# YangHai-1218/RADet

Measured on AMD Instinct MI355X. Metric: images/sec train-step, r50_ycbv_pbr 640x480 bs=4/GPU, higher is better.
Workload: dtype f32

## Files before the change

include/radet_hip.h:

```cpp
#ifndef RADET_HIP_H
#define RADET_HIP_H
#include <stdint.h>

#ifdef __cplusplus
extern "C" {
#endif


typedef struct RadetConvDesc {
    const float* w;
    const float* bias;
    const float* bn_gamma;
    const float* bn_beta;
    const float* bn_mean;
    const float* bn_var;
    float* wf;
    float* wft;
    float* bias_f;
    const float* dwf_slabs;
    const float* dbias_partials;
    float* dw;
    float* dbias;
    float* dgamma;
    float* dbeta;
    int cout, cin, kh, kw;
    int nsplit;
    float eps;
    int wft_ld;
    int wft_off;
    int w16;
    float* w_amax;
    float* wfq;
    float* w_l1;
    float* bias_amax;
    float* w_l1t;
} RadetConvDesc;

#define RADET_AMAX_WORDS 64
typedef struct RadetScales {
    const void* x_amax;
    const void* w_amax;
    void* y_amax;
    const void* x1_amax;
    const void* w1_amax;
    void* y1_amax;
    void* yq;
    void* yq_amax;
    const void* x_true_amax;
    const void* w_l1;
    const void* bias_amax;
    const void* addend_amax;
} RadetScales;

int radet_gather_table_rows(int M);
int radet_build_gather_table(int* table, int B, int KH, int KW, int so, int sr, int off, int div, const int* seg_desc,
                             int nseg, void* stream);
enum {
    RADET_TILE_ID_MASK = 0xFF,
    RADET_TILE_SYMBOL = 0x100,
    RADET_TILE_BK32 = 0x200,
    RADET_TILE_MATH_BF16 = 0x400,
    RADET_TILE_STORE_BF16 = 0x800,
    RADET_TILE_SPLITK = 0x1000,
    RADET_TILE_SPLITK_MASK = 0xF000,
    RADET_TILE_OUT_F32 = 0x10000,
    RADET_TILE_STAGES3 = 0x20000,
    RADET_TILE_STAGES4 = 0x40000,
    RADET_TILE_ROWPAIRS = 0x80000,
    RADET_TILE_STREAMK = 0x100000,
    RADET_TILE_STREAMK_MASK = 0x700000,
    RADET_TILE_X3 = 0x1000000,
    RADET_TILE_P3 = 0x2000000,
    RADET_TILE_H2 = 0x8000000,
    RADET_TILE_MASKQ = 0x10000000
};
int radet_conv2d_igemm(const float* x, const float* w, const float* bias, const float* addend, const float* mask,
                       float* y, const int* gather_table, int M, int Cin, int Cout, int KH, int KW, int relu,
                       int tile_override, float* splitk_ws, size_t splitk_ws_floats, void* stream);
int radet_conv2d_igemm_s(const float* x, const float* w, const float* bias, const float* addend, const float* mask,
                         float* y, const int* gather_table, int M, int Cin, int Cout, int KH, int KW, int relu,
                         int tile_override, float* splitk_ws, size_t splitk_ws_floats, void* stream, const RadetScales* sc);
int radet_conv2d_igemm_pair_s(const float* x0, const float* w0, const float* bias0, const float* addend0,
                              const float* mask0, float* y0, const float* x1, const float* w1, const float* bias1,
                              const float* addend1, const float* mask1, float* y1, const int* gather_table, int M,
                              int Cin, int Cout, int KH, int KW, int relu, int tile_override, float* splitk_ws,
                              size_t splitk_ws_floats, void* stream, const RadetScales* sc);
int radet_conv2d_igemm_taps_s(const float* x, const float* w, const float* addend, const float* mask, float* y,
                              const int* gather_table, const int* out_rows, const int* tap_ids_host, int ntaps, int kt_w,
                              int M, int Cin, int Cout, int tile_override, float* splitk_ws, size_t splitk_ws_floats,
                              void* stream, const RadetScales* sc);
int radet_conv2d_igemm_classes_s(const float* x, const float* w, const float* addend, const float* mask, float* y,
                                 const int* gather_table, const int* out_rows, const int* tap_ids_host,
                                 const int* cls_ntaps, const int* cls_start, int ncls, int kt_w, int M, int Cin, int Cout,
                                 int tile_override, float* splitk_ws, size_t splitk_ws_floats, void* stream,
                                 const RadetScales* sc);
int radet_conv2d_igemm_pair(const float* x0, const float* w0, const float* bias0, const float* addend0,
                            const float* mask0, float* y0, const float* x1, const float* w1, const float* bias1,
                            const float* addend1, const float* mask1, float* y1, const int* gather_table, int M, int Cin,
                            int Cout, int KH, int KW, int relu, int tile_override, float* splitk_ws,
                            size_t splitk_ws_floats, void* stream);
int radet_conv2d_igemm_taps(const float* x, const float* w, const float* addend, const float* mask, float* y,
                            const int* gather_table, const int* out_rows, const int* tap_ids_host, int ntaps, int kt_w,
                            int M, int Cin, int Cout, int tile_override, float* splitk_ws, size_t splitk_ws_floats,
                            void* stream);
int radet_conv2d_igemm_classes(const float* x, const float* w, const float* addend, const float* mask, float* y,
                               const int* gather_table, const int* out_rows, const int* tap_ids_host, const int* cls_ntaps,
                               const int* cls_start, int ncls, int kt_w, int M, int Cin, int Cout, int tile_override,
                               float* splitk_ws, size_t splitk_ws_floats, void* stream);
int radet_pred3x3_patch(const float* x, int Cin, const int* tiles_dev, int ntiles, const float* w0, const float* bias0,
                        float* y0, int c0, const float* w1, const float* bias1, float* y1, int c1, void* stream);
enum {
    RADET_WGRAD_MATH_BF16 = 0x1,
    RADET_WGRAD_STORE_BF16 = 0x2,
    RADET_WGRAD_TILE = 0x10,
    RADET_WGRAD_TILE_MASK = 0x30,
    RADET_WGRAD_ONE_TAP = 0x40,
    RADET_WGRAD_PX32 = 0x80,
    RADET_WGRAD_X3 = 0x100,
    RADET_WGRAD_P3 = 0x200,
    RADET_WGRAD_KDIV4 = 0x400,
    RADET_WGRAD_KDIV2 = 0x800,
    RADET_WGRAD_H2 = 0x1000,
    RADET_WGRAD_DEEP = 0x2000,
    RADET_WGRAD_WINDOWS = 0x4000
};
int radet_conv2d_wgrad_splits(int M, int Cin, int Cout, int KH, int KW);
int radet_conv2d_wgrad(const float* dy, const float* x, float* slabs, float* dbias_partials, const int* gather_table,
                       int M, int Cin, int Cout, int ld_dy, int KH, int KW, int S, int flags, void* stream);
int radet_conv2d_wgrad_s(const float* dy, const float* x, float* slabs, float* dbias_partials, const int* gather_table,
                         int M, int Cin, int Cout, int ld_dy, int KH, int KW, int S, int flags, void* stream,
                         const RadetScales* sc);
typedef struct RadetWgradJob {
    const float* dy;
    const float* x;
    float* slabs;
    float* dbias_partials;
    const int* gather_table;
    int M, Cin, Cout, ld_dy, KH, KW, S;
} RadetWgradJob;
int radet_conv2d_wgrad_group(const RadetWgradJob* jobs, int njobs, int flags, void* stream);
int radet_fold_weights(const RadetConvDesc* table_dev, int nconv, void* stream);
int radet_unfold_grads(const RadetConvDesc* table_dev, int nconv, int max_cout, void* stream);
int radet_stem_conv_bn_relu(const float* img_nchw, const float* wf_ohwi, const float* bias, float* y_nhwc, int B,
                            int H, int W, void* stream);
int radet_maxpool3x3s2(const float* x, float* y, int B, int H, int W, int C, void* stream);
int radet_maxpool3x3s2_bwd_relu(const float* s, const float* dpool, float* ds, int B, int H, int W, int C, void* stream);
int radet_stem_wgrad_splits(int B, int H, int W);
int radet_stem_wgrad(const float* img_nchw, const float* ds, float* slabs, float* dbias_partials, int B, int H, int W, int S,
                     void* stream);

int radet_gn_workspace_floats(int B, const int* seg_desc, int nseg);
int radet_gn_relu_fwd(const float* z, const float* gamma, const float* beta, float* y, float* stats ,
                      float* partial_ws, int B, int C, int groups, float eps, int relu, const int* seg_desc, int nseg,
                      void* stream);
int radet_gn_relu_bwd(const float* dy, const float* z, const float* stats, const float* gamma, const float* beta,
                      float* dz, float* dgamma, float* dbeta, float* partial_ws, int B, int C, int groups, int relu,
                      const int* seg_desc, int nseg, void* stream);

int radet_upsample_add(float* dst, const float* src, int B, int Ho, int Wo, int Hi, int Wi, int C, void* stream);
int radet_upsample_add_bwd(float* dsrc, const float* ddst, int B, int Ho, int Wo, int Hi, int Wi, int C, void* stream);
int radet_relu_bwd(const float* dy, const float* addend, const float* act, float* dx, size_t n, void* stream);
int radet_stem_conv_bn_relu_h(const float* img_nchw, const float* wf_ohwi, const float* bias, void* y_nhwc, int B, int H,
                              int W, void* stream);
int radet_maxpool3x3s2_h(const void* x, void* y, int B, int H, int W, int C, void* stream);
int radet_gn_relu_fwd_pair(const float* z0, const float* gamma0, const float* beta0, float* y0, float* stats0,
                           float* partial_ws0, const float* z1, const float* gamma1, const float* beta1, float* y1,
                           float* stats1, float* partial_ws1, int B, int C, int groups, float eps, int relu,
                           const int* seg_desc, int nseg, void* stream);
int radet_gn_relu_fwd_pair_h(const void* z0, const float* gamma0, const float* beta0, void* y0, float* stats0,
                             float* partial_ws0, const void* z1, const float* gamma1, const float* beta1, void* y1,
                             float* stats1, float* partial_ws1, int B, int C, int groups, float eps, int relu,
                             const int* seg_desc, int nseg, void* stream);
int radet_gn_relu_fwd_h(const void* z, const float* gamma, const float* beta, void* y, float* stats, float* partial_ws,
                        int B, int C, int groups, float eps, int relu, const int* seg_desc, int nseg, void* stream);
int radet_gn_relu_bwd_h(const void* dy, const void* z, const float* stats, const float* gamma, const float* beta, void* dz,
                        float* dgamma, float* dbeta, float* partial_ws, int B, int C, int groups, int relu,
                        const int* seg_desc, int nseg, void* stream);
int radet_upsample_add_h(void* dst, const void* src, int B, int Ho, int Wo, int Hi, int Wi, int C, void* stream);
int radet_upsample_add_bwd_h(void* dsrc, const void* ddst, int B, int Ho, int Wo, int Hi, int Wi, int C, void* stream);
int radet_relu_bwd_h(const void* dy, const void* addend, const void* act, void* dx, size_t n, void* stream);
int radet_convert_rows(const void* src, void* dst, size_t rows, int ncols, int src_ld, int src_off, int dst_ld,
                       int dst_off, int to_bf16, void* stream);
int radet_split_planes(const float* src, void* dst_planes, size_t rows, int C, int src_ld, void* stream);
int radet_merge_planes(const void* src_planes, float* dst, size_t rows, int C, int dst_ld, void* stream);
int radet_split_pairs(const float* src, void* dst_pairs, size_t rows, int C, int src_ld, const void* src_amax, void* dst_amax,
                      void* stream);
int radet_merge_pairs(const void* src_pairs, float* dst, size_t rows, int C, int dst_ld, const void* amax, void* stream);
int radet_gn_relu_fwd_q(const float* z, const float* gamma, const float* beta, float* y, void* yq, float* stats,
                        float* partial_ws, int B, int C, int groups, float eps, int relu, const int* seg_desc, int nseg,
                        void* stream, void* y_amax, void* yq_amax, void* zhat_amax);
int radet_gn_relu_fwd_pair_q(const float* z0, const float* gamma0, const float* beta0, float* y0, void* yq0, float* stats0,
                             float* partial_ws0, void* y_amax0, void* yq_amax0, void* zhat_amax0, const float* z1,
                             const float* gamma1, const float* beta1, float* y1, void* yq1, float* stats1,
                             float* partial_ws1, void* y_amax1, void* yq_amax1, void* zhat_amax1, int B, int C, int groups,
                             float eps, int relu, const int* seg_desc, int nseg, void* stream);
int radet_gn_relu_bwd_q(const float* dy, const float* z, const float* stats, const float* gamma, const float* beta, float* dz,
                        void* dzq, float* dgamma, float* dbeta, float* partial_ws, int B, int C, int groups, int relu,
                        const int* seg_desc, int nseg, void* stream, const void* dy_amax, const void* zhat_amax,
                        void* dzq_amax);
int radet_maxpool3x3s2_a(const float* x, float* y, int B, int H, int W, int C, void* y_amax, void* stream);
int radet_maxpool3x3s2_q(const float* x, float* y, int B, int H, int W, int C, void* y_amax, void* yq, void* yq_amax,
                         const void* x_amax, void* stream);
int radet_stem_conv_bn_relu_a(const float* img_nchw, const float* wf_ohwi, const float* bias, float* y_nhwc, int B, int H, int W,
                              void* y_amax, void* stream);
int radet_upsample_add_a(float* dst, const float* src, int B, int Ho, int Wo, int Hi, int Wi, int C, void* dst_amax,
                         void* stream);
int radet_upsample_add_bwd_a(float* dsrc, const float* ddst, int B, int Ho, int Wo, int Hi, int Wi, int C, void* dsrc_amax,
                             void* stream);
int radet_relu_bwd_a(const float* dy, const float* addend, const float* act, float* dx, size_t n, void* dx_amax, void* stream);
int radet_absmax(const float* x, size_t n, void* amax, void* stream);
int radet_amax_slot_words(void);
int radet_gn_relu_fwd_p(const float* z, const float* gamma, const float* beta, float* y, void* yp, float* stats,
                        float* partial_ws, int B, int C, int groups, float eps, int relu, const int* seg_desc, int nseg,
                        void* stream);
int radet_gn_relu_fwd_pair_p(const float* z0, const float* gamma0, const float* beta0, float* y0, void* yp0, float* stats0,
                             float* partial_ws0, const float* z1, const float* gamma1, const float* beta1, float* y1,
                             void* yp1, float* stats1, float* partial_ws1, int B, int C, int groups, float eps, int relu,
                             const int* seg_desc, int nseg, void* stream);
int radet_gn_relu_bwd_p(const float* dy, const float* z, const float* stats, const float* gamma, const float* beta,
                        float* dz, void* dzp, float* dgamma, float* dbeta, float* partial_ws, int B, int C, int groups,
                        int relu, const int* seg_desc, int nseg, void* stream);
int radet_nchw_to_nhwc(const float* x, float* y, int B, int C, int H, int W, void* stream);
int radet_nhwc_to_nchw(const float* x, float* y, int B, int C, int H, int W, void* stream);

#define RADET_HEAD_LOSS_POSTACT 1
#define RADET_HEAD_LOSS_KIND_SHIFT 1
#define RADET_HEAD_LOSS_KIND_MASK (7 << RADET_HEAD_LOSS_KIND_SHIFT)
#define RADET_BOX_LOSS_GIOU 0
#define RADET_BOX_LOSS_IOU 1
#define RADET_BOX_LOSS_IOU_LINEAR 2
#define RADET_BOX_LOSS_DIOU 3
#define RADET_BOX_LOSS_CIOU 4
#define RADET_BOX_LOSS_KINDS 5
int radet_head_loss_ws_ints(int R);
int radet_head_loss(const float* cls, const float* reg_u, const float* iou, const float* scales,
                    const float* gt_boxes, const int64_t* gt_labels, const int* gt_off, const int64_t* p2g,
                    const float* pw, const int* level_desc, int nlvl, int B, int num_classes, float alpha,
                    float gamma, float loss_bbox_weight, float giou_eps, const float* grad_scale, float* losses,
                    float* dcls, int dcls_ld, float* dreg_u, int dreg_ld, float* diou, int diou_ld, float* dscales,
                    int64_t* labels_out, float* bbox_targets_out, int flags, int* ws, void* stream);
int radet_scale_relu(const float* reg_u, const float* scales, float* out, const int* level_desc, int nlvl, int B,
                     void* stream);

size_t radet_decode_ws_bytes(int B, int nlvl, int nms_pre);
int radet_decode_candidates(const float* cls, const float* reg_u, const float* iou, const float* scales,
                            const int* level_desc, int nlvl, int B, int num_classes, float score_thr, int nms_pre,
                            const float* img_hw , const float* scale_factor ,
                            float* cand_boxes, float* cand_scores, float* cand_ctr, int64_t* cand_labels,
                            int* cand_count, void* ws, void* stream);

size_t radet_nms_ws_bytes(int B, int cap);
int radet_nms(const float* boxes, const float* cluster_scores, const float* vote_scores, const int64_t* labels,
              const int* counts, int B, int cap, int mode, float iou_thr, int iou_enable, float sigma, int max_out,
              float* out_boxes, float* out_scores, int64_t* out_labels, int* out_count, int64_t* aux0, int64_t* aux1,
              void* ws, void* stream);

size_t radet_assign_ws_bytes(int B, int N);
int radet_assign_points(const float* gt_boxes, const int* gt_off, const uint8_t* masks, int H, int W,
                        const uint32_t* rng_words, int U, const int* level_desc, const float* regress_ranges ,
                        int nlvl, int B, int positive_num, int flags, float neg_threshold, int64_t* p2g, float* pw, int* used,
                        void* ws, void* stream);

int radet_assign_points_f(const float* gt_boxes, const int* gt_off, const float* distance_maps, int H, int W,
                          const uint32_t* rng_words, int U, const int* level_desc, const float* regress_ranges ,
                          int nlvl, int B, int positive_num, int flags, float neg_threshold, int64_t* p2g, float* pw, int* used,
                          void* ws, void* stream);

size_t radet_mbd_ws_bytes(size_t total_px);
int radet_mbd(const uint8_t* images, const int* img_desc_dev, int nimg, const int* seeds_x, const int* seeds_y, float alpha,
              int niter, int base_size, double* dmap, size_t total_px, void* ws, void* stream);
int radet_gdt(const float* cost, const int* img_desc_dev, int nimg, const int* seeds_x, const int* seeds_y, float* dist,
              void* ws_labels , void* stream);

int radet_resize_linear_u8(const uint8_t* src, const int* src_desc, uint8_t* dst, const int* dst_desc, const int* view_desc,
                           int ncrop, int max_dst_px, int channels, void* stream);
int radet_resize_linear_f(const void* src, const int* src_desc, void* dst, const int* dst_desc, int ncrop, int max_dst_px,
                          int is_f64, void* stream);
#define RADET_VIEW_INTS 12
int radet_gaussian_blur9_u8(const uint8_t* src, const int* desc, uint8_t* dst, float* tmp, const float* kernel5, int ncrop,
                            int max_px, void* stream);
int radet_sobel_edge(const uint8_t* src, const int* desc, float* edge, uint8_t* gray_ws, uint32_t* max_ws, int ncrop,
                     int max_px, void* stream);

int radet_mask_max(const uint8_t* masks, uint32_t* maxes , int G, size_t hw, void* stream);
int radet_mask_transform(const uint8_t* src, uint8_t* dst, const uint32_t* norm_max, const int* view_desc, int G, int Hs, int Ws,
                         int Hr, int Wr, int Hd, int Wd, int flip, int pad_val, void* stream);

#define RLE_MASK_INTS 5
#define RLE_PART_INTS 2
int radet_rle_masks(const uint32_t* run_ends, int n_ends, const int* part_desc, int n_parts, const int* mask_desc,
                    const int* view_desc, int G, uint8_t* dst, uint8_t* dst_plain, int Hr, int Wr, int Hd, int Wd, int pad_val,
                    void* stream);

#define JPEG_ROW_INTS 8
#define JPEG_DESC_INTS 20
#define JPEG_HUFF_BYTES 1424
int radet_jpeg_index(const uint8_t* file, int scan_lo, int scan_hi, int ncomp, const int* comp_blocks, const void* huff,
                     int n_mcus, int restart_interval, int seg_mcus, int* rows, int max_rows);
int radet_jpeg_decode(const uint8_t* files, const int* desc, int nimg, const int* wgs, int n_wg, const void* huff,
                      const uint16_t* quant, const int* rows, int n_rows, int16_t* coef, uint8_t* planes, uint8_t* dst,
                      int* err, int max_blocks, int max_px, int stages, void* stream);

#define AUG_PARAM_INTS 16
#define AUG_MAX_W 8192
int radet_augment_merge_hblur(const uint8_t* src, const uint8_t* bg, const int* params, uint8_t* dst, int nimg, int max_h,
                              int max_w, void* stream);
int radet_augment_vblur(const uint8_t* src, const int* params, uint8_t* dst, int nimg, int max_h, int max_w, void* stream);
int radet_augment_sharp(const uint8_t* src, const int* params, uint8_t* dst, unsigned long long* lsum, int nimg, int max_px,
                        void* stream);
int radet_augment_finish(const uint8_t* src, const unsigned long long* lsum, const int* params, float* out, int nimg, int Hp,
                         int Wp, float m0, float m1, float m2, float s0, float s1, float s2, void* stream);

#define AUG2_PARAM_INTS 16
int radet_augment_hsv_noise(const uint8_t* src, const int* params2, uint8_t* dst, int nimg, int max_px, void* stream);
int radet_augment_box(const uint8_t* src, const int* params2, uint8_t* dst, size_t nbytes, int nimg, int max_h, int max_w,
                      void* stream);

#define CROP_DESC_INTS 12
#define PASTE_DESC_INTS 10
int radet_crop_canvases(const uint8_t* src, size_t src_bytes, const unsigned long long* lsum, const int* params, int nimg,
                        const int* desc, int ncanvas, int max_px, uint8_t* dst, size_t total_px, void* stream);
int radet_paste_maps(const void* maps, size_t map_px, int is_f64, const int* desc, int nbox, int H, int W, float* out,
                     void* stream);

#define WARP_DESC_INTS 20
#define WARP_DESC_SRC 0
#define WARP_DESC_DST 1
#define WARP_DESC_H 2
#define WARP_DESC_W 3
#define WARP_DESC_CHANNELS 4
#define WARP_DESC_FILL 5
#define WARP_DESC_FLAGS 6
#define WARP_DESC_MATRIX 8
#define WARP_SKIP 1
int radet_warp_affine_u8(const uint8_t* src, size_t src_px, uint8_t* dst, size_t dst_px, const int* desc, int nimg, int max_px,
                         int channels, void* stream);

#define CUTOUT_DESC_INTS 8
#define CUTOUT_DESC_OFF 0
#define CUTOUT_DESC_H 1
#define CUTOUT_DESC_W 2
#define CUTOUT_DESC_FILL 3
#define CUTOUT_DESC_FIRST 4
#define CUTOUT_DESC_COUNT 5
#define CUTOUT_DESC_FLAGS 6
#define CUTOUT_SKIP 1
#define CUTOUT_FLIP 2
#define CUTOUT_TO_RGB 4
int radet_cutout_u8(uint8_t* img, size_t img_px, const int* desc, int nimg, const int* holes, int nholes, int max_holes,
                    int max_area, int channels, void* stream);
int radet_cutout_f32(float* out, int nbatch, int Hp, int Wp, const int* desc, int nimg, const int* holes, int nholes, int max_holes,
                     int max_area, float m0, float m1, float m2, float s0, float s1, float s2, void* stream);

#define PREP_DESC_INTS 8
#define PREP_TO_RGB 1
int radet_preprocess_frames(const int* desc, int nimg, int Hp, int Wp, float m0, float m1, float m2, float s0, float s1,
                            float s2, float* out, void* stream);

int radet_bbox_overlaps(const float* bboxes1, const float* bboxes2, float* out, int batch, int M, int N, int mode,
                        int aligned, float eps, void* stream);
int radet_tblr_encode(const float* priors, const float* gts, float* out, int n, const float* normalizer4,
                      int normalize_by_wh, void* stream);
int radet_tblr_decode(const float* priors, const float* tblr, float* out, int n, const float* normalizer4,
                      int normalize_by_wh, float max_h, float max_w, int clip, void* stream);
int radet_loss_partials(size_t n_elem);
int radet_loss_finalize(const float* partials, int npartials, const float* avg_factor, float scale, float* out,
                        void* stream);
int radet_sigmoid_focal_loss(const float* logits, const int64_t* target, const float* weight, int weight_cols, size_t N,
                             int C, float gamma, float alpha, float* loss_elem, float elem_scale, float* partials,
                             void* stream);
int radet_sigmoid_focal_loss_bwd(const float* logits, const int64_t* target, const float* weight, int weight_cols, size_t N,
                                 int C, float gamma, float alpha, const float* grad_elem, const float* grad_scalar,
                                 const float* avg_factor, float scale, float* dlogits, void* stream);
int radet_bce_logits_loss(const float* logits, const float* target, const float* weight, int weight_cols, size_t N, int C,
                          float* loss_elem, float elem_scale, float* partials, void* stream);
int radet_bce_logits_loss_bwd(const float* logits, const float* target, const float* weight, int weight_cols, size_t N,
                              int C, const float* grad_elem, const float* grad_scalar, const float* avg_factor, float scale,
                              float* dlogits, void* stream);
int radet_giou_loss(const float* pred, const float* target, const float* weight, size_t N, float eps, float* loss_elem,
                    float elem_scale, float* partials, void* stream);
int radet_giou_loss_bwd(const float* pred, const float* target, const float* weight, size_t N, float eps,
                        const float* grad_elem, const float* grad_scalar, const float* avg_factor, float scale, float* dpred,
                        void* stream);
int radet_box_loss(int kind, const float* pred, const float* target, const float* weight, size_t N, float eps, float hp1,
                   float* loss_elem, float elem_scale, float* partials, void* stream);
int radet_box_loss_bwd(int kind, const float* pred, const float* target, const float* weight, size_t N, float eps, float hp1,
                       const float* grad_elem, const float* grad_scalar, const float* avg_factor, float scale, float* dpred,
                       void* stream);
int radet_threshold_compact(const float* scores, size_t n, float thr, int64_t* idx, int* count, void* stream);

int radet_grid_anchors(float* out, const int* level_desc, int nlvl, int octave_base_scale, void* stream);

int radet_sqnorm_partials(const float* g, size_t n, float* partials, int npartials, void* stream);
int radet_adamw_step(float* p, const float* g, float* m, float* v, size_t n, float lr, float beta1, float beta2,
                     float eps, float weight_decay, int step, float max_norm, float grad_div,
                     const float* partials, int npartials, float* grad_norm_out, void* stream);
#define RADET_OPT_MAX_RUNS 1024
typedef struct { uint32_t begin, end; float lr_mult, decay_mult; } RadetOptRun;
// ... 42 lines not shown
```

radet_amd/_lib.py:

```python
import ctypes as C
import os

_HERE = os.path.dirname(os.path.abspath(__file__))
LIB_PATH = os.path.join(_HERE, os.environ.get("RADET_LIB", "libradet_hip.so"))

_p = C.c_void_p
_i = C.c_int
_f = C.c_float
_sz = C.c_size_t


class RadetConvDesc(C.Structure):
    _fields_ = [("w", _p), ("bias", _p), ("bn_gamma", _p), ("bn_beta", _p), ("bn_mean", _p), ("bn_var", _p),
                ("wf", _p), ("wft", _p), ("bias_f", _p), ("dwf_slabs", _p), ("dbias_partials", _p),
                ("dw", _p), ("dbias", _p), ("dgamma", _p), ("dbeta", _p),
                ("cout", _i), ("cin", _i), ("kh", _i), ("kw", _i), ("nsplit", _i), ("eps", _f),
                ("wft_ld", _i), ("wft_off", _i), ("w16", _i), ("w_amax", _p), ("wfq", _p), ("w_l1", _p), ("bias_amax", _p),
                ("w_l1t", _p)]


class RadetScales(C.Structure):
    _fields_ = [("x_amax", _p), ("w_amax", _p), ("y_amax", _p), ("x1_amax", _p), ("w1_amax", _p), ("y1_amax", _p),
                ("yq", _p), ("yq_amax", _p), ("x_true_amax", _p), ("w_l1", _p), ("bias_amax", _p), ("addend_amax", _p)]


class RadetWgradJob(C.Structure):
    _fields_ = [("dy", _p), ("x", _p), ("slabs", _p), ("dbias_partials", _p), ("gather_table", _p),
                ("M", _i), ("Cin", _i), ("Cout", _i), ("ld_dy", _i), ("KH", _i), ("KW", _i), ("S", _i)]


class RadetTapeOp(C.Structure):
    _fields_ = [("kind", C.c_int32), ("fn", C.c_int32), ("stream", _p), ("event", _p), ("args", C.c_uint64 * 32)]


SIGNATURES = {
    "radet_gather_table_rows": (_i, [_i]),
    "radet_build_gather_table": (_i, [_p, _i, _i, _i, _i, _i, _i, _i, _p, _i, _p]),
    "radet_conv2d_igemm": (_i, [_p, _p, _p, _p, _p, _p, _p, _i, _i, _i, _i, _i, _i, _i, _p, _sz, _p]),
    "radet_conv2d_igemm_pair": (_i, [_p] * 13 + [_i, _i, _i, _i, _i, _i, _i, _p, _sz, _p]),
    "radet_conv2d_igemm_taps": (_i, [_p, _p, _p, _p, _p, _p, _p, _p, _i, _i, _i, _i, _i, _i, _p, _sz, _p]),
    "radet_conv2d_igemm_classes": (_i, [_p, _p, _p, _p, _p, _p, _p, _p, _p, _p, _i, _i, _i, _i, _i, _i, _p, _sz, _p]),
    "radet_conv2d_igemm_s": (_i, [_p, _p, _p, _p, _p, _p, _p, _i, _i, _i, _i, _i, _i, _i, _p, _sz, _p, _p]),
    "radet_conv2d_igemm_pair_s": (_i, [_p] * 13 + [_i, _i, _i, _i, _i, _i, _i, _p, _sz, _p, _p]),
    "radet_conv2d_igemm_taps_s": (_i, [_p, _p, _p, _p, _p, _p, _p, _p, _i, _i, _i, _i, _i, _i, _p, _sz, _p, _p]),
    "radet_conv2d_igemm_classes_s": (_i, [_p, _p, _p, _p, _p, _p, _p, _p, _p, _p, _i, _i, _i, _i, _i, _i, _p, _sz, _p, _p]),
    "radet_conv2d_wgrad_s": (_i, [_p, _p, _p, _p, _p, _i, _i, _i, _i, _i, _i, _i, _i, _p, _p]),
    "radet_split_pairs": (_i, [_p, _p, _sz, _i, _i, _p, _p, _p]),
    "radet_merge_pairs": (_i, [_p, _p, _sz, _i, _i, _p, _p]),
    "radet_gn_relu_fwd_q": (_i, [_p, _p, _p, _p, _p, _p, _p, _i, _i, _i, _f, _i, _p, _i, _p, _p, _p, _p]),
    "radet_gn_relu_fwd_pair_q": (_i, [_p] * 20 + [_i, _i, _i, _f, _i, _p, _i, _p]),
    "radet_gn_relu_bwd_q": (_i, [_p, _p, _p, _p, _p, _p, _p, _p, _p, _p, _i, _i, _i, _i, _p, _i, _p, _p, _p, _p]),
    "radet_maxpool3x3s2_a": (_i, [_p, _p, _i, _i, _i, _i, _p, _p]),
    "radet_maxpool3x3s2_q": (_i, [_p, _p, _i, _i, _i, _i, _p, _p, _p, _p, _p]),
    "radet_stem_conv_bn_relu_a": (_i, [_p, _p, _p, _p, _i, _i, _i, _p, _p]),
    "radet_upsample_add_a": (_i, [_p, _p, _i, _i, _i, _i, _i, _i, _p, _p]),
    "radet_upsample_add_bwd_a": (_i, [_p, _p, _i, _i, _i, _i, _i, _i, _p, _p]),
    "radet_relu_bwd_a": (_i, [_p, _p, _p, _p, _sz, _p, _p]),
    "radet_absmax": (_i, [_p, _sz, _p, _p]),
    "radet_amax_slot_words": (_i, []),
    "radet_pred3x3_patch": (_i, [_p, _i, _p, _i, _p, _p, _p, _i, _p, _p, _p, _i, _p]),
    "radet_conv2d_wgrad_splits": (_i, [_i, _i, _i, _i, _i]),
    "radet_conv2d_wgrad": (_i, [_p, _p, _p, _p, _p, _i, _i, _i, _i, _i, _i, _i, _i, _p]),
    "radet_conv2d_wgrad_group": (_i, [_p, _i, _i, _p]),
    "radet_fold_weights": (_i, [_p, _i, _p]),
    "radet_unfold_grads": (_i, [_p, _i, _i, _p]),
    "radet_stem_conv_bn_relu": (_i, [_p, _p, _p, _p, _i, _i, _i, _p]),
    "radet_maxpool3x3s2": (_i, [_p, _p, _i, _i, _i, _i, _p]),
    "radet_maxpool3x3s2_bwd_relu": (_i, [_p, _p, _p, _i, _i, _i, _i, _p]),
    "radet_stem_wgrad_splits": (_i, [_i, _i, _i]),
    "radet_stem_wgrad": (_i, [_p, _p, _p, _p, _i, _i, _i, _i, _p]),
    "radet_gn_workspace_floats": (_i, [_i, _p, _i]),
    "radet_gn_relu_fwd": (_i, [_p, _p, _p, _p, _p, _p, _i, _i, _i, _f, _i, _p, _i, _p]),
    "radet_gn_relu_fwd_pair": (_i, [_p] * 12 + [_i, _i, _i, _f, _i, _p, _i, _p]),
    "radet_gn_relu_fwd_pair_h": (_i, [_p] * 12 + [_i, _i, _i, _f, _i, _p, _i, _p]),
    "radet_gn_relu_bwd": (_i, [_p, _p, _p, _p, _p, _p, _p, _p, _p, _i, _i, _i, _i, _p, _i, _p]),
    "radet_upsample_add": (_i, [_p, _p, _i, _i, _i, _i, _i, _i, _p]),
    "radet_upsample_add_bwd": (_i, [_p, _p, _i, _i, _i, _i, _i, _i, _p]),
    "radet_relu_bwd": (_i, [_p, _p, _p, _p, _sz, _p]),
    "radet_nchw_to_nhwc": (_i, [_p, _p, _i, _i, _i, _i, _p]),
    "radet_nhwc_to_nchw": (_i, [_p, _p, _i, _i, _i, _i, _p]),
    "radet_head_loss_ws_ints": (_i, [_i]),
    "radet_head_loss": (_i, [_p, _p, _p, _p, _p, _p, _p, _p, _p, _p, _i, _i, _i, _f, _f, _f, _f, _p, _p, _p, _i, _p,
                             _i, _p, _i, _p, _p, _p, _i, _p, _p]),
    "radet_scale_relu": (_i, [_p, _p, _p, _p, _i, _i, _p]),
    "radet_decode_ws_bytes": (_sz, [_i, _i, _i]),
    "radet_decode_candidates": (_i, [_p, _p, _p, _p, _p, _i, _i, _i, _f, _i, _p, _p, _p, _p, _p, _p, _p, _p, _p]),
    "radet_nms_ws_bytes": (_sz, [_i, _i]),
    "radet_nms": (_i, [_p, _p, _p, _p, _p, _i, _i, _i, _f, _i, _f, _i, _p, _p, _p, _p, _p, _p, _p, _p]),
    "radet_assign_ws_bytes": (_sz, [_i, _i]),
    "radet_assign_points": (_i, [_p, _p, _p, _i, _i, _p, _i, _p, _p, _i, _i, _i, _i, _f, _p, _p, _p, _p, _p]),
    "radet_assign_points_f": (_i, [_p, _p, _p, _i, _i, _p, _i, _p, _p, _i, _i, _i, _i, _f, _p, _p, _p, _p, _p]),
    "radet_resize_linear_u8": (_i, [_p, _p, _p, _p, _p, _i, _i, _i, _p]),
    "radet_resize_linear_f": (_i, [_p, _p, _p, _p, _i, _i, _i, _p]),
    "radet_warp_affine_u8": (_i, [_p, _sz, _p, _sz, _p, _i, _i, _i, _p]),
    "radet_cutout_u8": (_i, [_p, _sz, _p, _i, _p, _i, _i, _i, _i, _p]),
    "radet_cutout_f32": (_i, [_p, _i, _i, _i, _p, _i, _p, _i, _i, _i, _f, _f, _f, _f, _f, _f, _p]),
    "radet_gaussian_blur9_u8": (_i, [_p, _p, _p, _p, _p, _i, _i, _p]),
    "radet_sobel_edge": (_i, [_p, _p, _p, _p, _p, _i, _i, _p]),
    "radet_stem_conv_bn_relu_h": (_i, [_p, _p, _p, _p, _i, _i, _i, _p]),
    "radet_maxpool3x3s2_h": (_i, [_p, _p, _i, _i, _i, _i, _p]),
    "radet_gn_relu_fwd_h": (_i, [_p, _p, _p, _p, _p, _p, _i, _i, _i, _f, _i, _p, _i, _p]),
    "radet_gn_relu_bwd_h": (_i, [_p, _p, _p, _p, _p, _p, _p, _p, _p, _i, _i, _i, _i, _p, _i, _p]),
    "radet_upsample_add_h": (_i, [_p, _p, _i, _i, _i, _i, _i, _i, _p]),
    "radet_upsample_add_bwd_h": (_i, [_p, _p, _i, _i, _i, _i, _i, _i, _p]),
    "radet_relu_bwd_h": (_i, [_p, _p, _p, _p, _sz, _p]),
    "radet_convert_rows": (_i, [_p, _p, _sz, _i, _i, _i, _i, _i, _i, _p]),
    "radet_split_planes": (_i, [_p, _p, _sz, _i, _i, _p]),
    "radet_merge_planes": (_i, [_p, _p, _sz, _i, _i, _p]),
    "radet_gn_relu_fwd_p": (_i, [_p, _p, _p, _p, _p, _p, _p, _i, _i, _i, _f, _i, _p, _i, _p]),
    "radet_gn_relu_fwd_pair_p": (_i, [_p] * 14 + [_i, _i, _i, _f, _i, _p, _i, _p]),
    "radet_gn_relu_bwd_p": (_i, [_p, _p, _p, _p, _p, _p, _p, _p, _p, _p, _i, _i, _i, _i, _p, _i, _p]),
    "radet_mbd_ws_bytes": (_sz, [_sz]),
    "radet_mbd": (_i, [_p, _p, _i, _p, _p, _f, _i, _i, _p, _sz, _p, _p]),
    "radet_gdt": (_i, [_p, _p, _i, _p, _p, _p, _p, _p]),
    "radet_mask_max": (_i, [_p, _p, _i, _sz, _p]),
    "radet_mask_transform": (_i, [_p, _p, _p, _p, _i, _i, _i, _i, _i, _i, _i, _i, _i, _p]),
    "radet_rle_masks": (_i, [_p, _i, _p, _i, _p, _p, _i, _p, _p, _i, _i, _i, _i, _i, _p]),
    "radet_jpeg_index": (_i, [_p, _i, _i, _i, _p, _p, _i, _i, _i, _p, _i]),
    "radet_jpeg_decode": (_i, [_p, _p, _i, _p, _i, _p, _p, _p, _i, _p, _p, _p, _p, _i, _i, _i, _p]),
    "radet_augment_merge_hblur": (_i, [_p, _p, _p, _p, _i, _i, _i, _p]),
    "radet_augment_vblur": (_i, [_p, _p, _p, _i, _i, _i, _p]),
    "radet_augment_sharp": (_i, [_p, _p, _p, _p, _i, _i, _p]),
    "radet_augment_finish": (_i, [_p, _p, _p, _p, _i, _i, _i, _f, _f, _f, _f, _f, _f, _p]),
    "radet_augment_hsv_noise": (_i, [_p, _p, _p, _i, _i, _p]),
    "radet_augment_box": (_i, [_p, _p, _p, _sz, _i, _i, _i, _p]),
    "radet_crop_canvases": (_i, [_p, _sz, _p, _p, _i, _p, _i, _i, _p, _sz, _p]),
    "radet_paste_maps": (_i, [_p, _sz, _i, _p, _i, _i, _i, _p, _p]),
    "radet_preprocess_frames": (_i, [_p, _i, _i, _i, _f, _f, _f, _f, _f, _f, _p, _p]),
    "radet_grid_anchors": (_i, [_p, _p, _i, _i, _p]),
    "radet_bbox_overlaps": (_i, [_p, _p, _p, _i, _i, _i, _i, _i, _f, _p]),
    "radet_tblr_encode": (_i, [_p, _p, _p, _i, _p, _i, _p]),
    "radet_tblr_decode": (_i, [_p, _p, _p, _i, _p, _i, _f, _f, _i, _p]),
    "radet_loss_partials": (_i, [_sz]),
    "radet_loss_finalize": (_i, [_p, _i, _p, _f, _p, _p]),
    "radet_sigmoid_focal_loss": (_i, [_p, _p, _p, _i, _sz, _i, _f, _f, _p, _f, _p, _p]),
    "radet_sigmoid_focal_loss_bwd": (_i, [_p, _p, _p, _i, _sz, _i, _f, _f, _p, _p, _p, _f, _p, _p]),
    "radet_bce_logits_loss": (_i, [_p, _p, _p, _i, _sz, _i, _p, _f, _p, _p]),
    "radet_bce_logits_loss_bwd": (_i, [_p, _p, _p, _i, _sz, _i, _p, _p, _p, _f, _p, _p]),
    "radet_giou_loss": (_i, [_p, _p, _p, _sz, _f, _p, _f, _p, _p]),
    "radet_giou_loss_bwd": (_i, [_p, _p, _p, _sz, _f, _p, _p, _p, _f, _p, _p]),
    "radet_box_loss": (_i, [_i, _p, _p, _p, _sz, _f, _f, _p, _f, _p, _p]),
    "radet_box_loss_bwd": (_i, [_i, _p, _p, _p, _sz, _f, _f, _p, _p, _p, _f, _p, _p]),
    "radet_threshold_compact": (_i, [_p, _sz, _f, _p, _p, _p]),
    "radet_sqnorm_partials": (_i, [_p, _sz, _p, _i, _p]),
    "radet_adamw_step": (_i, [_p, _p, _p, _p, _sz, _f, _f, _f, _f, _f, _i, _f, _f, _p, _i, _p, _p]),
    "radet_adamw_step_runs": (_i, [_p, _p, _p, _p, _sz, _f, _f, _f, _f, _f, _i, _f, _f, _p, _i, _p, _p, _i, _p]),
    "radet_sgd_step": (_i, [_p, _p, _p, _sz, _f, _f, _f, _f, _i, _i, _f, _f, _p, _i, _p, _p, _i, _p]),
    "radet_grad_accumulate": (_i, [_p, _p, _sz, _i, _p]),
    "radet_coco_match": (_i, [_p, _p, _p, _p, _p, _p, _i, _i, _p, _i, _p, _i, _p, _p, _p, _p, _p]),
    "radet_coco_accumulate": (_i, [_p, _p, _p, _p, _p, _p, _p, _p, _i, _i, _i, _i, _i, _p, _p, _p, _p]),
    "radet_tape_fn_index": (_i, [C.c_char_p]),
    "radet_tape_replay": (_i, [_p, _i, _i, _p]),
    "radet_fill_zero": (_i, [_p, _sz, _p]),
    "radet_copy_d2d": (_i, [_p, _p, _sz, _p]),
    "radet_stream_create_cumask": (_i, [_p, _i, _p]),
    "radet_copy_segments": (_i, [_p, _i, _i, _p]),
}

_lib = None


class RadetHipError(RuntimeError):
    pass


def load():
    global _lib
    if _lib is not None:
        return _lib
    if not os.path.exists(LIB_PATH):
        raise RadetHipError(
            f"{LIB_PATH} is missing: the HIP extension is not built. Run `make -C radet_amd/csrc` "
            "(or __graft_entry__.build()). radet_amd has no CPU / PyTorch fallback.")
    lib = C.CDLL(LIB_PATH)
    for name, (res, args) in SIGNATURES.items():
        try:
            fn = getattr(lib, name)
        except AttributeError as e:
            raise RadetHipError(f"libradet_hip.so does not export {name}") from e
        fn.restype = res
        fn.argtypes = args
    _lib = lib
    return lib


def check(rc, name):
    if rc != 0:
        raise RadetHipError(f"{name} failed with code {rc} (-1 bad argument, -2 launch failure)")


_FN = {}


def call(name, *args):
    fn = _FN.get(name)
    if fn is None:
        if name not in SIGNATURES:
            raise RadetHipError(f"{name} has no entry in radet_amd._lib.SIGNATURES")
        fn = _FN[name] = getattr(load(), name)
    rc = fn(*args)
    if rc != 0:
        raise RadetHipError(f"{name} failed with code {rc} (-1 bad argument, -2 launch failure)")
    if TAPE is not None:
        TAPE.record_call(name, args)


TAPE = None
```

radet_amd/csrc/tape_thunks.c:

```c
#include <stdint.h>
#include <stddef.h>
#include <string.h>
#include "radet_hip.h"

static float f32(uint64_t w) { uint32_t u = (uint32_t)w; float f; memcpy(&f, &u, 4); return f; }

static int t_radet_absmax(const uint64_t* a) { return radet_absmax((void*)(uintptr_t)a[0], (size_t)a[1], (void*)(uintptr_t)a[2], (void*)(uintptr_t)a[3]); }
static int t_radet_adamw_step(const uint64_t* a) { return radet_adamw_step((void*)(uintptr_t)a[0], (void*)(uintptr_t)a[1], (void*)(uintptr_t)a[2], (void*)(uintptr_t)a[3], (size_t)a[4], f32(a[5]), f32(a[6]), f32(a[7]), f32(a[8]), f32(a[9]), (int)(int64_t)a[10], f32(a[11]), f32(a[12]), (void*)(uintptr_t)a[13], (int)(int64_t)a[14], (void*)(uintptr_t)a[15], (void*)(uintptr_t)a[16]); }
static int t_radet_adamw_step_runs(const uint64_t* a) { return radet_adamw_step_runs((void*)(uintptr_t)a[0], (void*)(uintptr_t)a[1], (void*)(uintptr_t)a[2], (void*)(uintptr_t)a[3], (size_t)a[4], f32(a[5]), f32(a[6]), f32(a[7]), f32(a[8]), f32(a[9]), (int)(int64_t)a[10], f32(a[11]), f32(a[12]), (void*)(uintptr_t)a[13], (int)(int64_t)a[14], (void*)(uintptr_t)a[15], (void*)(uintptr_t)a[16], (int)(int64_t)a[17], (void*)(uintptr_t)a[18]); }
static int t_radet_amax_slot_words(const uint64_t* a) { (void)a; return radet_amax_slot_words(); }
static int t_radet_assign_points(const uint64_t* a) { return radet_assign_points((void*)(uintptr_t)a[0], (void*)(uintptr_t)a[1], (void*)(uintptr_t)a[2], (int)(int64_t)a[3], (int)(int64_t)a[4], (void*)(uintptr_t)a[5], (int)(int64_t)a[6], (void*)(uintptr_t)a[7], (void*)(uintptr_t)a[8], (int)(int64_t)a[9], (int)(int64_t)a[10], (int)(int64_t)a[11], (int)(int64_t)a[12], f32(a[13]), (void*)(uintptr_t)a[14], (void*)(uintptr_t)a[15], (void*)(uintptr_t)a[16], (void*)(uintptr_t)a[17], (void*)(uintptr_t)a[18]); }
static int t_radet_assign_points_f(const uint64_t* a) { return radet_assign_points_f((void*)(uintptr_t)a[0], (void*)(uintptr_t)a[1], (void*)(uintptr_t)a[2], (int)(int64_t)a[3], (int)(int64_t)a[4], (void*)(uintptr_t)a[5], (int)(int64_t)a[6], (void*)(uintptr_t)a[7], (void*)(uintptr_t)a[8], (int)(int64_t)a[9], (int)(int64_t)a[10], (int)(int64_t)a[11], (int)(int64_t)a[12], f32(a[13]), (void*)(uintptr_t)a[14], (void*)(uintptr_t)a[15], (void*)(uintptr_t)a[16], (void*)(uintptr_t)a[17], (void*)(uintptr_t)a[18]); }
static int t_radet_augment_box(const uint64_t* a) { return radet_augment_box((void*)(uintptr_t)a[0], (void*)(uintptr_t)a[1], (void*)(uintptr_t)a[2], (size_t)a[3], (int)(int64_t)a[4], (int)(int64_t)a[5], (int)(int64_t)a[6], (void*)(uintptr_t)a[7]); }
static int t_radet_augment_finish(const uint64_t* a) { return radet_augment_finish((void*)(uintptr_t)a[0], (void*)(uintptr_t)a[1], (void*)(uintptr_t)a[2], (void*)(uintptr_t)a[3], (int)(int64_t)a[4], (int)(int64_t)a[5], (int)(int64_t)a[6], f32(a[7]), f32(a[8]), f32(a[9]), f32(a[10]), f32(a[11]), f32(a[12]), (void*)(uintptr_t)a[13]); }
static int t_radet_augment_hsv_noise(const uint64_t* a) { return radet_augment_hsv_noise((void*)(uintptr_t)a[0], (void*)(uintptr_t)a[1], (void*)(uintptr_t)a[2], (int)(int64_t)a[3], (int)(int64_t)a[4], (void*)(uintptr_t)a[5]); }
static int t_radet_augment_merge_hblur(const uint64_t* a) { return radet_augment_merge_hblur((void*)(uintptr_t)a[0], (void*)(uintptr_t)a[1], (void*)(uintptr_t)a[2], (void*)(uintptr_t)a[3], (int)(int64_t)a[4], (int)(int64_t)a[5], (int)(int64_t)a[6], (void*)(uintptr_t)a[7]); }
static int t_radet_augment_sharp(const uint64_t* a) { return radet_augment_sharp((void*)(uintptr_t)a[0], (void*)(uintptr_t)a[1], (void*)(uintptr_t)a[2], (void*)(uintptr_t)a[3], (int)(int64_t)a[4], (int)(int64_t)a[5], (void*)(uintptr_t)a[6]); }
static int t_radet_augment_vblur(const uint64_t* a) { return radet_augment_vblur((void*)(uintptr_t)a[0], (void*)(uintptr_t)a[1], (void*)(uintptr_t)a[2], (int)(int64_t)a[3], (int)(int64_t)a[4], (int)(int64_t)a[5], (void*)(uintptr_t)a[6]); }
static int t_radet_bbox_overlaps(const uint64_t* a) { return radet_bbox_overlaps((void*)(uintptr_t)a[0], (void*)(uintptr_t)a[1], (void*)(uintptr_t)a[2], (int)(int64_t)a[3], (int)(int64_t)a[4], (int)(int64_t)a[5], (int)(int64_t)a[6], (int)(int64_t)a[7], f32(a[8]), (void*)(uintptr_t)a[9]); }
static int t_radet_bce_logits_loss(const uint64_t* a) { return radet_bce_logits_loss((void*)(uintptr_t)a[0], (void*)(uintptr_t)a[1], (void*)(uintptr_t)a[2], (int)(int64_t)a[3], (size_t)a[4], (int)(int64_t)a[5], (void*)(uintptr_t)a[6], f32(a[7]), (void*)(uintptr_t)a[8], (void*)(uintptr_t)a[9]); }
static int t_radet_bce_logits_loss_bwd(const uint64_t* a) { return radet_bce_logits_loss_bwd((void*)(uintptr_t)a[0], (void*)(uintptr_t)a[1], (void*)(uintptr_t)a[2], (int)(int64_t)a[3], (size_t)a[4], (int)(int64_t)a[5], (void*)(uintptr_t)a[6], (void*)(uintptr_t)a[7], (void*)(uintptr_t)a[8], f32(a[9]), (void*)(uintptr_t)a[10], (void*)(uintptr_t)a[11]); }
static int t_radet_box_loss(const uint64_t* a) { return radet_box_loss((int)(int64_t)a[0], (void*)(uintptr_t)a[1], (void*)(uintptr_t)a[2], (void*)(uintptr_t)a[3], (size_t)a[4], f32(a[5]), f32(a[6]), (void*)(uintptr_t)a[7], f32(a[8]), (void*)(uintptr_t)a[9], (void*)(uintptr_t)a[10]); }
static int t_radet_box_loss_bwd(const uint64_t* a) { return radet_box_loss_bwd((int)(int64_t)a[0], (void*)(uintptr_t)a[1], (void*)(uintptr_t)a[2], (void*)(uintptr_t)a[3], (size_t)a[4], f32(a[5]), f32(a[6]), (void*)(uintptr_t)a[7], (void*)(uintptr_t)a[8], (void*)(uintptr_t)a[9], f32(a[10]), (void*)(uintptr_t)a[11], (void*)(uintptr_t)a[12]); }
static int t_radet_build_gather_table(const uint64_t* a) { return radet_build_gather_table((void*)(uintptr_t)a[0], (int)(int64_t)a[1], (int)(int64_t)a[2], (int)(int64_t)a[3], (int)(int64_t)a[4], (int)(int64_t)a[5], (int)(int64_t)a[6], (int)(int64_t)a[7], (void*)(uintptr_t)a[8], (int)(int64_t)a[9], (void*)(uintptr_t)a[10]); }
static int t_radet_coco_accumulate(const uint64_t* a) { return radet_coco_accumulate((void*)(uintptr_t)a[0], (void*)(uintptr_t)a[1], (void*)(uintptr_t)a[2], (void*)(uintptr_t)a[3], (void*)(uintptr_t)a[4], (void*)(uintptr_t)a[5], (void*)(uintptr_t)a[6], (void*)(uintptr_t)a[7], (int)(int64_t)a[8], (int)(int64_t)a[9], (int)(int64_t)a[10], (int)(int64_t)a[11], (int)(int64_t)a[12], (void*)(uintptr_t)a[13], (void*)(uintptr_t)a[14], (void*)(uintptr_t)a[15], (void*)(uintptr_t)a[16]); }
static int t_radet_coco_match(const uint64_t* a) { return radet_coco_match((void*)(uintptr_t)a[0], (void*)(uintptr_t)a[1], (void*)(uintptr_t)a[2], (void*)(uintptr_t)a[3], (void*)(uintptr_t)a[4], (void*)(uintptr_t)a[5], (int)(int64_t)a[6], (int)(int64_t)a[7], (void*)(uintptr_t)a[8], (int)(int64_t)a[9], (void*)(uintptr_t)a[10], (int)(int64_t)a[11], (void*)(uintptr_t)a[12], (void*)(uintptr_t)a[13], (void*)(uintptr_t)a[14], (void*)(uintptr_t)a[15], (void*)(uintptr_t)a[16]); }
static int t_radet_conv2d_igemm(const uint64_t* a) { return radet_conv2d_igemm((void*)(uintptr_t)a[0], (void*)(uintptr_t)a[1], (void*)(uintptr_t)a[2], (void*)(uintptr_t)a[3], (void*)(uintptr_t)a[4], (void*)(uintptr_t)a[5], (void*)(uintptr_t)a[6], (int)(int64_t)a[7], (int)(int64_t)a[8], (int)(int64_t)a[9], (int)(int64_t)a[10], (int)(int64_t)a[11], (int)(int64_t)a[12], (int)(int64_t)a[13], (void*)(uintptr_t)a[14], (size_t)a[15], (void*)(uintptr_t)a[16]); }
static int t_radet_conv2d_igemm_classes(const uint64_t* a) { return radet_conv2d_igemm_classes((void*)(uintptr_t)a[0], (void*)(uintptr_t)a[1], (void*)(uintptr_t)a[2], (void*)(uintptr_t)a[3], (void*)(uintptr_t)a[4], (void*)(uintptr_t)a[5], (void*)(uintptr_t)a[6], (void*)(uintptr_t)a[7], (void*)(uintptr_t)a[8], (void*)(uintptr_t)a[9], (int)(int64_t)a[10], (int)(int64_t)a[11], (int)(int64_t)a[12], (int)(int64_t)a[13], (int)(int64_t)a[14], (int)(int64_t)a[15], (void*)(uintptr_t)a[16], (size_t)a[17], (void*)(uintptr_t)a[18]); }
static int t_radet_conv2d_igemm_classes_s(const uint64_t* a) { return radet_conv2d_igemm_classes_s((void*)(uintptr_t)a[0], (void*)(uintptr_t)a[1], (void*)(uintptr_t)a[2], (void*)(uintptr_t)a[3], (void*)(uintptr_t)a[4], (void*)(uintptr_t)a[5], (void*)(uintptr_t)a[6], (void*)(uintptr_t)a[7], (void*)(uintptr_t)a[8], (void*)(uintptr_t)a[9], (int)(int64_t)a[10], (int)(int64_t)a[11], (int)(int64_t)a[12], (int)(int64_t)a[13], (int)(int64_t)a[14], (int)(int64_t)a[15], (void*)(uintptr_t)a[16], (size_t)a[17], (void*)(uintptr_t)a[18], (void*)(uintptr_t)a[19]); }
static int t_radet_conv2d_igemm_pair(const uint64_t* a) { return radet_conv2d_igemm_pair((void*)(uintptr_t)a[0], (void*)(uintptr_t)a[1], (void*)(uintptr_t)a[2], (void*)(uintptr_t)a[3], (void*)(uintptr_t)a[4], (void*)(uintptr_t)a[5], (void*)(uintptr_t)a[6], (void*)(uintptr_t)a[7], (void*)(uintptr_t)a[8], (void*)(uintptr_t)a[9], (void*)(uintptr_t)a[10], (void*)(uintptr_t)a[11], (void*)(uintptr_t)a[12], (int)(int64_t)a[13], (int)(int64_t)a[14], (int)(int64_t)a[15], (int)(int64_t)a[16], (int)(int64_t)a[17], (int)(int64_t)a[18], (int)(int64_t)a[19], (void*)(uintptr_t)a[20], (size_t)a[21], (void*)(uintptr_t)a[22]); }
static int t_radet_conv2d_igemm_pair_s(const uint64_t* a) { return radet_conv2d_igemm_pair_s((void*)(uintptr_t)a[0], (void*)(uintptr_t)a[1], (void*)(uintptr_t)a[2], (void*)(uintptr_t)a[3], (void*)(uintptr_t)a[4], (void*)(uintptr_t)a[5], (void*)(uintptr_t)a[6], (void*)(uintptr_t)a[7], (void*)(uintptr_t)a[8], (void*)(uintptr_t)a[9], (void*)(uintptr_t)a[10], (void*)(uintptr_t)a[11], (void*)(uintptr_t)a[12], (int)(int64_t)a[13], (int)(int64_t)a[14], (int)(int64_t)a[15], (int)(int64_t)a[16], (int)(int64_t)a[17], (int)(int64_t)a[18], (int)(int64_t)a[19], (void*)(uintptr_t)a[20], (size_t)a[21], (void*)(uintptr_t)a[22], (void*)(uintptr_t)a[23]); }
static int t_radet_conv2d_igemm_s(const uint64_t* a) { return radet_conv2d_igemm_s((void*)(uintptr_t)a[0], (void*)(uintptr_t)a[1], (void*)(uintptr_t)a[2], (void*)(uintptr_t)a[3], (void*)(uintptr_t)a[4], (void*)(uintptr_t)a[5], (void*)(uintptr_t)a[6], (int)(int64_t)a[7], (int)(int64_t)a[8], (int)(int64_t)a[9], (int)(int64_t)a[10], (int)(int64_t)a[11], (int)(int64_t)a[12], (int)(int64_t)a[13], (void*)(uintptr_t)a[14], (size_t)a[15], (void*)(uintptr_t)a[16], (void*)(uintptr_t)a[17]); }
static int t_radet_conv2d_igemm_taps(const uint64_t* a) { return radet_conv2d_igemm_taps((void*)(uintptr_t)a[0], (void*)(uintptr_t)a[1], (void*)(uintptr_t)a[2], (void*)(uintptr_t)a[3], (void*)(uintptr_t)a[4], (void*)(uintptr_t)a[5], (void*)(uintptr_t)a[6], (void*)(uintptr_t)a[7], (int)(int64_t)a[8], (int)(int64_t)a[9], (int)(int64_t)a[10], (int)(int64_t)a[11], (int)(int64_t)a[12], (int)(int64_t)a[13], (void*)(uintptr_t)a[14], (size_t)a[15], (void*)(uintptr_t)a[16]); }
static int t_radet_conv2d_igemm_taps_s(const uint64_t* a) { return radet_conv2d_igemm_taps_s((void*)(uintptr_t)a[0], (void*)(uintptr_t)a[1], (void*)(uintptr_t)a[2], (void*)(uintptr_t)a[3], (void*)(uintptr_t)a[4], (void*)(uintptr_t)a[5], (void*)(uintptr_t)a[6], (void*)(uintptr_t)a[7], (int)(int64_t)a[8], (int)(int64_t)a[9], (int)(int64_t)a[10], (int)(int64_t)a[11], (int)(int64_t)a[12], (int)(int64_t)a[13], (void*)(uintptr_t)a[14], (size_t)a[15], (void*)(uintptr_t)a[16], (void*)(uintptr_t)a[17]); }
static int t_radet_conv2d_wgrad(const uint64_t* a) { return radet_conv2d_wgrad((void*)(uintptr_t)a[0], (void*)(uintptr_t)a[1], (void*)(uintptr_t)a[2], (void*)(uintptr_t)a[3], (void*)(uintptr_t)a[4], (int)(int64_t)a[5], (int)(int64_t)a[6], (int)(int64_t)a[7], (int)(int64_t)a[8], (int)(int64_t)a[9], (int)(int64_t)a[10], (int)(int64_t)a[11], (int)(int64_t)a[12], (void*)(uintptr_t)a[13]); }
static int t_radet_conv2d_wgrad_group(const uint64_t* a) { return radet_conv2d_wgrad_group((void*)(uintptr_t)a[0], (int)(int64_t)a[1], (int)(int64_t)a[2], (void*)(uintptr_t)a[3]); }
static int t_radet_conv2d_wgrad_s(const uint64_t* a) { return radet_conv2d_wgrad_s((void*)(uintptr_t)a[0], (void*)(uintptr_t)a[1], (void*)(uintptr_t)a[2], (void*)(uintptr_t)a[3], (void*)(uintptr_t)a[4], (int)(int64_t)a[5], (int)(int64_t)a[6], (int)(int64_t)a[7], (int)(int64_t)a[8], (int)(int64_t)a[9], (int)(int64_t)a[10], (int)(int64_t)a[11], (int)(int64_t)a[12], (void*)(uintptr_t)a[13], (void*)(uintptr_t)a[14]); }
static int t_radet_conv2d_wgrad_splits(const uint64_t* a) { return radet_conv2d_wgrad_splits((int)(int64_t)a[0], (int)(int64_t)a[1], (int)(int64_t)a[2], (int)(int64_t)a[3], (int)(int64_t)a[4]); }
static int t_radet_convert_rows(const uint64_t* a) { return radet_convert_rows((void*)(uintptr_t)a[0], (void*)(uintptr_t)a[1], (size_t)a[2], (int)(int64_t)a[3], (int)(int64_t)a[4], (int)(int64_t)a[5], (int)(int64_t)a[6], (int)(int64_t)a[7], (int)(int64_t)a[8], (void*)(uintptr_t)a[9]); }
static int t_radet_copy_d2d(const uint64_t* a) { return radet_copy_d2d((void*)(uintptr_t)a[0], (void*)(uintptr_t)a[1], (size_t)a[2], (void*)(uintptr_t)a[3]); }
static int t_radet_copy_segments(const uint64_t* a) { return radet_copy_segments((void*)(uintptr_t)a[0], (int)(int64_t)a[1], (int)(int64_t)a[2], (void*)(uintptr_t)a[3]); }
static int t_radet_crop_canvases(const uint64_t* a) { return radet_crop_canvases((void*)(uintptr_t)a[0], (size_t)a[1], (void*)(uintptr_t)a[2], (void*)(uintptr_t)a[3], (int)(int64_t)a[4], (void*)(uintptr_t)a[5], (int)(int64_t)a[6], (int)(int64_t)a[7], (void*)(uintptr_t)a[8], (size_t)a[9], (void*)(uintptr_t)a[10]); }
static int t_radet_cutout_f32(const uint64_t* a) { return radet_cutout_f32((void*)(uintptr_t)a[0], (int)(int64_t)a[1], (int)(int64_t)a[2], (int)(int64_t)a[3], (void*)(uintptr_t)a[4], (int)(int64_t)a[5], (void*)(uintptr_t)a[6], (int)(int64_t)a[7], (int)(int64_t)a[8], (int)(int64_t)a[9], f32(a[10]), f32(a[11]), f32(a[12]), f32(a[13]), f32(a[14]), f32(a[15]), (void*)(uintptr_t)a[16]); }
static int t_radet_cutout_u8(const uint64_t* a) { return radet_cutout_u8((void*)(uintptr_t)a[0], (size_t)a[1], (void*)(uintptr_t)a[2], (int)(int64_t)a[3], (void*)(uintptr_t)a[4], (int)(int64_t)a[5], (int)(int64_t)a[6], (int)(int64_t)a[7], (int)(int64_t)a[8], (void*)(uintptr_t)a[9]); }
static int t_radet_decode_candidates(const uint64_t* a) { return radet_decode_candidates((void*)(uintptr_t)a[0], (void*)(uintptr_t)a[1], (void*)(uintptr_t)a[2], (void*)(uintptr_t)a[3], (void*)(uintptr_t)a[4], (int)(int64_t)a[5], (int)(int64_t)a[6], (int)(int64_t)a[7], f32(a[8]), (int)(int64_t)a[9], (void*)(uintptr_t)a[10], (void*)(uintptr_t)a[11], (void*)(uintptr_t)a[12], (void*)(uintptr_t)a[13], (void*)(uintptr_t)a[14], (void*)(uintptr_t)a[15], (void*)(uintptr_t)a[16], (void*)(uintptr_t)a[17], (void*)(uintptr_t)a[18]); }
static int t_radet_fill_zero(const uint64_t* a) { return radet_fill_zero((void*)(uintptr_t)a[0], (size_t)a[1], (void*)(uintptr_t)a[2]); }
static int t_radet_fold_weights(const uint64_t* a) { return radet_fold_weights((void*)(uintptr_t)a[0], (int)(int64_t)a[1], (void*)(uintptr_t)a[2]); }
static int t_radet_gather_table_rows(const uint64_t* a) { return radet_gather_table_rows((int)(int64_t)a[0]); }
static int t_radet_gaussian_blur9_u8(const uint64_t* a) { return radet_gaussian_blur9_u8((void*)(uintptr_t)a[0], (void*)(uintptr_t)a[1], (void*)(uintptr_t)a[2], (void*)(uintptr_t)a[3], (void*)(uintptr_t)a[4], (int)(int64_t)a[5], (int)(int64_t)a[6], (void*)(uintptr_t)a[7]); }
static int t_radet_gdt(const uint64_t* a) { return radet_gdt((void*)(uintptr_t)a[0], (void*)(uintptr_t)a[1], (int)(int64_t)a[2], (void*)(uintptr_t)a[3], (void*)(uintptr_t)a[4], (void*)(uintptr_t)a[5], (void*)(uintptr_t)a[6], (void*)(uintptr_t)a[7]); }
static int t_radet_giou_loss(const uint64_t* a) { return radet_giou_loss((void*)(uintptr_t)a[0], (void*)(uintptr_t)a[1], (void*)(uintptr_t)a[2], (size_t)a[3], f32(a[4]), (void*)(uintptr_t)a[5], f32(a[6]), (void*)(uintptr_t)a[7], (void*)(uintptr_t)a[8]); }
static int t_radet_giou_loss_bwd(const uint64_t* a) { return radet_giou_loss_bwd((void*)(uintptr_t)a[0], (void*)(uintptr_t)a[1], (void*)(uintptr_t)a[2], (size_t)a[3], f32(a[4]), (void*)(uintptr_t)a[5], (void*)(uintptr_t)a[6], (void*)(uintptr_t)a[7], f32(a[8]), (void*)(uintptr_t)a[9], (void*)(uintptr_t)a[10]); }
static int t_radet_gn_relu_bwd(const uint64_t* a) { return radet_gn_relu_bwd((void*)(uintptr_t)a[0], (void*)(uintptr_t)a[1], (void*)(uintptr_t)a[2], (void*)(uintptr_t)a[3], (void*)(uintptr_t)a[4], (void*)(uintptr_t)a[5], (void*)(uintptr_t)a[6], (void*)(uintptr_t)a[7], (void*)(uintptr_t)a[8], (int)(int64_t)a[9], (int)(int64_t)a[10], (int)(int64_t)a[11], (int)(int64_t)a[12], (void*)(uintptr_t)a[13], (int)(int64_t)a[14], (void*)(uintptr_t)a[15]); }
static int t_radet_gn_relu_bwd_h(const uint64_t* a) { return radet_gn_relu_bwd_h((void*)(uintptr_t)a[0], (void*)(uintptr_t)a[1], (void*)(uintptr_t)a[2], (void*)(uintptr_t)a[3], (void*)(uintptr_t)a[4], (void*)(uintptr_t)a[5], (void*)(uintptr_t)a[6], (void*)(uintptr_t)a[7], (void*)(uintptr_t)a[8], (int)(int64_t)a[9], (int)(int64_t)a[10], (int)(int64_t)a[11], (int)(int64_t)a[12], (void*)(uintptr_t)a[13], (int)(int64_t)a[14], (void*)(uintptr_t)a[15]); }
static int t_radet_gn_relu_bwd_p(const uint64_t* a) { return radet_gn_relu_bwd_p((void*)(uintptr_t)a[0], (void*)(uintptr_t)a[1], (void*)(uintptr_t)a[2], (void*)(uintptr_t)a[3], (void*)(uintptr_t)a[4], (void*)(uintptr_t)a[5], (void*)(uintptr_t)a[6], (void*)(uintptr_t)a[7], (void*)(uintptr_t)a[8], (void*)(uintptr_t)a[9], (int)(int64_t)a[10], (int)(int64_t)a[11], (int)(int64_t)a[12], (int)(int64_t)a[13], (void*)(uintptr_t)a[14], (int)(int64_t)a[15], (void*)(uintptr_t)a[16]); }
static int t_radet_gn_relu_bwd_q(const uint64_t* a) { return radet_gn_relu_bwd_q((void*)(uintptr_t)a[0], (void*)(uintptr_t)a[1], (void*)(uintptr_t)a[2], (void*)(uintptr_t)a[3], (void*)(uintptr_t)a[4], (void*)(uintptr_t)a[5], (void*)(uintptr_t)a[6], (void*)(uintptr_t)a[7], (void*)(uintptr_t)a[8], (void*)(uintptr_t)a[9], (int)(int64_t)a[10], (int)(int64_t)a[11], (int)(int64_t)a[12], (int)(int64_t)a[13], (void*)(uintptr_t)a[14], (int)(int64_t)a[15], (void*)(uintptr_t)a[16], (void*)(uintptr_t)a[17], (void*)(uintptr_t)a[18], (void*)(uintptr_t)a[19]); }
static int t_radet_gn_relu_fwd(const uint64_t* a) { return radet_gn_relu_fwd((void*)(uintptr_t)a[0], (void*)(uintptr_t)a[1], (void*)(uintptr_t)a[2], (void*)(uintptr_t)a[3], (void*)(uintptr_t)a[4], (void*)(uintptr_t)a[5], (int)(int64_t)a[6], (int)(int64_t)a[7], (int)(int64_t)a[8], f32(a[9]), (int)(int64_t)a[10], (void*)(uintptr_t)a[11], (int)(int64_t)a[12], (void*)(uintptr_t)a[13]); }
static int t_radet_gn_relu_fwd_h(const uint64_t* a) { return radet_gn_relu_fwd_h((void*)(uintptr_t)a[0], (void*)(uintptr_t)a[1], (void*)(uintptr_t)a[2], (void*)(uintptr_t)a[3], (void*)(uintptr_t)a[4], (void*)(uintptr_t)a[5], (int)(int64_t)a[6], (int)(int64_t)a[7], (int)(int64_t)a[8], f32(a[9]), (int)(int64_t)a[10], (void*)(uintptr_t)a[11], (int)(int64_t)a[12], (void*)(uintptr_t)a[13]); }
static int t_radet_gn_relu_fwd_p(const uint64_t* a) { return radet_gn_relu_fwd_p((void*)(uintptr_t)a[0], (void*)(uintptr_t)a[1], (void*)(uintptr_t)a[2], (void*)(uintptr_t)a[3], (void*)(uintptr_t)a[4], (void*)(uintptr_t)a[5], (void*)(uintptr_t)a[6], (int)(int64_t)a[7], (int)(int64_t)a[8], (int)(int64_t)a[9], f32(a[10]), (int)(int64_t)a[11], (void*)(uintptr_t)a[12], (int)(int64_t)a[13], (void*)(uintptr_t)a[14]); }
static int t_radet_gn_relu_fwd_pair(const uint64_t* a) { return radet_gn_relu_fwd_pair((void*)(uintptr_t)a[0], (void*)(uintptr_t)a[1], (void*)(uintptr_t)a[2], (void*)(uintptr_t)a[3], (void*)(uintptr_t)a[4], (void*)(uintptr_t)a[5], (void*)(uintptr_t)a[6], (void*)(uintptr_t)a[7], (void*)(uintptr_t)a[8], (void*)(uintptr_t)a[9], (void*)(uintptr_t)a[10], (void*)(uintptr_t)a[11], (int)(int64_t)a[12], (int)(int64_t)a[13], (int)(int64_t)a[14], f32(a[15]), (int)(int64_t)a[16], (void*)(uintptr_t)a[17], (int)(int64_t)a[18], (void*)(uintptr_t)a[19]); }
static int t_radet_gn_relu_fwd_pair_h(const uint64_t* a) { return radet_gn_relu_fwd_pair_h((void*)(uintptr_t)a[0], (void*)(uintptr_t)a[1], (void*)(uintptr_t)a[2], (void*)(uintptr_t)a[3], (void*)(uintptr_t)a[4], (void*)(uintptr_t)a[5], (void*)(uintptr_t)a[6], (void*)(uintptr_t)a[7], (void*)(uintptr_t)a[8], (void*)(uintptr_t)a[9], (void*)(uintptr_t)a[10], (void*)(uintptr_t)a[11], (int)(int64_t)a[12], (int)(int64_t)a[13], (int)(int64_t)a[14], f32(a[15]), (int)(int64_t)a[16], (void*)(uintptr_t)a[17], (int)(int64_t)a[18], (void*)(uintptr_t)a[19]); }
static int t_radet_gn_relu_fwd_pair_p(const uint64_t* a) { return radet_gn_relu_fwd_pair_p((void*)(uintptr_t)a[0], (void*)(uintptr_t)a[1], (void*)(uintptr_t)a[2], (void*)(uintptr_t)a[3], (void*)(uintptr_t)a[4], (void*)(uintptr_t)a[5], (void*)(uintptr_t)a[6], (void*)(uintptr_t)a[7], (void*)(uintptr_t)a[8], (void*)(uintptr_t)a[9], (void*)(uintptr_t)a[10], (void*)(uintptr_t)a[11], (void*)(uintptr_t)a[12], (void*)(uintptr_t)a[13], (int)(int64_t)a[14], (int)(int64_t)a[15], (int)(int64_t)a[16], f32(a[17]), (int)(int64_t)a[18], (void*)(uintptr_t)a[19], (int)(int64_t)a[20], (void*)(uintptr_t)a[21]); }
static int t_radet_gn_relu_fwd_pair_q(const uint64_t* a) { return radet_gn_relu_fwd_pair_q((void*)(uintptr_t)a[0], (void*)(uintptr_t)a[1], (void*)(uintptr_t)a[2], (void*)(uintptr_t)a[3], (void*)(uintptr_t)a[4], (void*)(uintptr_t)a[5], (void*)(uintptr_t)a[6], (void*)(uintptr_t)a[7], (void*)(uintptr_t)a[8], (void*)(uintptr_t)a[9], (void*)(uintptr_t)a[10], (void*)(uintptr_t)a[11], (void*)(uintptr_t)a[12], (void*)(uintptr_t)a[13], (void*)(uintptr_t)a[14], (void*)(uintptr_t)a[15], (void*)(uintptr_t)a[16], (void*)(uintptr_t)a[17], (void*)(uintptr_t)a[18], (void*)(uintptr_t)a[19], (int)(int64_t)a[20], (int)(int64_t)a[21], (int)(int64_t)a[22], f32(a[23]), (int)(int64_t)a[24], (void*)(uintptr_t)a[25], (int)(int64_t)a[26], (void*)(uintptr_t)a[27]); }
static int t_radet_gn_relu_fwd_q(const uint64_t* a) { return radet_gn_relu_fwd_q((void*)(uintptr_t)a[0], (void*)(uintptr_t)a[1], (void*)(uintptr_t)a[2], (void*)(uintptr_t)a[3], (void*)(uintptr_t)a[4], (void*)(uintptr_t)a[5], (void*)(uintptr_t)a[6], (int)(int64_t)a[7], (int)(int64_t)a[8], (int)(int64_t)a[9], f32(a[10]), (int)(int64_t)a[11], (void*)(uintptr_t)a[12], (int)(int64_t)a[13], (void*)(uintptr_t)a[14], (void*)(uintptr_t)a[15], (void*)(uintptr_t)a[16], (void*)(uintptr_t)a[17]); }
static int t_radet_gn_workspace_floats(const uint64_t* a) { return radet_gn_workspace_floats((int)(int64_t)a[0], (void*)(uintptr_t)a[1], (int)(int64_t)a[2]); }
static int t_radet_grad_accumulate(const uint64_t* a) { return radet_grad_accumulate((void*)(uintptr_t)a[0], (void*)(uintptr_t)a[1], (size_t)a[2], (int)(int64_t)a[3], (void*)(uintptr_t)a[4]); }
static int t_radet_grid_anchors(const uint64_t* a) { return radet_grid_anchors((void*)(uintptr_t)a[0], (void*)(uintptr_t)a[1], (int)(int64_t)a[2], (int)(int64_t)a[3], (void*)(uintptr_t)a[4]); }
static int t_radet_head_loss(const uint64_t* a) { return radet_head_loss((void*)(uintptr_t)a[0], (void*)(uintptr_t)a[1], (void*)(uintptr_t)a[2], (void*)(uintptr_t)a[3], (void*)(uintptr_t)a[4], (void*)(uintptr_t)a[5], (void*)(uintptr_t)a[6], (void*)(uintptr_t)a[7], (void*)(uintptr_t)a[8], (void*)(uintptr_t)a[9], (int)(int64_t)a[10], (int)(int64_t)a[11], (int)(int64_t)a[12], f32(a[13]), f32(a[14]), f32(a[15]), f32(a[16]), (void*)(uintptr_t)a[17], (void*)(uintptr_t)a[18], (void*)(uintptr_t)a[19], (int)(int64_t)a[20], (void*)(uintptr_t)a[21], (int)(int64_t)a[22], (void*)(uintptr_t)a[23], (int)(int64_t)a[24], (void*)(uintptr_t)a[25], (void*)(uintptr_t)a[26], (void*)(uintptr_t)a[27], (int)(int64_t)a[28], (void*)(uintptr_t)a[29], (void*)(uintptr_t)a[30]); }
static int t_radet_head_loss_ws_ints(const uint64_t* a) { return radet_head_loss_ws_ints((int)(int64_t)a[0]); }
static int t_radet_jpeg_decode(const uint64_t* a) { return radet_jpeg_decode((void*)(uintptr_t)a[0], (void*)(uintptr_t)a[1], (int)(int64_t)a[2], (void*)(uintptr_t)a[3], (int)(int64_t)a[4], (void*)(uintptr_t)a[5], (void*)(uintptr_t)a[6], (void*)(uintptr_t)a[7], (int)(int64_t)a[8], (void*)(uintptr_t)a[9], (void*)(uintptr_t)a[10], (void*)(uintptr_t)a[11], (void*)(uintptr_t)a[12], (int)(int64_t)a[13], (int)(int64_t)a[14], (int)(int64_t)a[15], (void*)(uintptr_t)a[16]); }
static int t_radet_jpeg_index(const uint64_t* a) { return radet_jpeg_index((void*)(uintptr_t)a[0], (int)(int64_t)a[1], (int)(int64_t)a[2], (int)(int64_t)a[3], (void*)(uintptr_t)a[4], (void*)(uintptr_t)a[5], (int)(int64_t)a[6], (int)(int64_t)a[7], (int)(int64_t)a[8], (void*)(uintptr_t)a[9], (int)(int64_t)a[10]); }
static int t_radet_loss_finalize(const uint64_t* a) { return radet_loss_finalize((void*)(uintptr_t)a[0], (int)(int64_t)a[1], (void*)(uintptr_t)a[2], f32(a[3]), (void*)(uintptr_t)a[4], (void*)(uintptr_t)a[5]); }
static int t_radet_loss_partials(const uint64_t* a) { return radet_loss_partials((size_t)a[0]); }
static int t_radet_mask_max(const uint64_t* a) { return radet_mask_max((void*)(uintptr_t)a[0], (void*)(uintptr_t)a[1], (int)(int64_t)a[2], (size_t)a[3], (void*)(uintptr_t)a[4]); }
static int t_radet_mask_transform(const uint64_t* a) { return radet_mask_transform((void*)(uintptr_t)a[0], (void*)(uintptr_t)a[1], (void*)(uintptr_t)a[2], (void*)(uintptr_t)a[3], (int)(int64_t)a[4], (int)(int64_t)a[5], (int)(int64_t)a[6], (int)(int64_t)a[7], (int)(int64_t)a[8], (int)(int64_t)a[9], (int)(int64_t)a[10], (int)(int64_t)a[11], (int)(int64_t)a[12], (void*)(uintptr_t)a[13]); }
static int t_radet_maxpool3x3s2(const uint64_t* a) { return radet_maxpool3x3s2((void*)(uintptr_t)a[0], (void*)(uintptr_t)a[1], (int)(int64_t)a[2], (int)(int64_t)a[3], (int)(int64_t)a[4], (int)(int64_t)a[5], (void*)(uintptr_t)a[6]); }
static int t_radet_maxpool3x3s2_a(const uint64_t* a) { return radet_maxpool3x3s2_a((void*)(uintptr_t)a[0], (void*)(uintptr_t)a[1], (int)(int64_t)a[2], (int)(int64_t)a[3], (int)(int64_t)a[4], (int)(int64_t)a[5], (void*)(uintptr_t)a[6], (void*)(uintptr_t)a[7]); }
static int t_radet_maxpool3x3s2_bwd_relu(const uint64_t* a) { return radet_maxpool3x3s2_bwd_relu((void*)(uintptr_t)a[0], (void*)(uintptr_t)a[1], (void*)(uintptr_t)a[2], (int)(int64_t)a[3], (int)(int64_t)a[4], (int)(int64_t)a[5], (int)(int64_t)a[6], (void*)(uintptr_t)a[7]); }
static int t_radet_maxpool3x3s2_h(const uint64_t* a) { return radet_maxpool3x3s2_h((void*)(uintptr_t)a[0], (void*)(uintptr_t)a[1], (int)(int64_t)a[2], (int)(int64_t)a[3], (int)(int64_t)a[4], (int)(int64_t)a[5], (void*)(uintptr_t)a[6]); }
static int t_radet_maxpool3x3s2_q(const uint64_t* a) { return radet_maxpool3x3s2_q((void*)(uintptr_t)a[0], (void*)(uintptr_t)a[1], (int)(int64_t)a[2], (int)(int64_t)a[3], (int)(int64_t)a[4], (int)(int64_t)a[5], (void*)(uintptr_t)a[6], (void*)(uintptr_t)a[7], (void*)(uintptr_t)a[8], (void*)(uintptr_t)a[9], (void*)(uintptr_t)a[10]); }
static int t_radet_mbd(const uint64_t* a) { return radet_mbd((void*)(uintptr_t)a[0], (void*)(uintptr_t)a[1], (int)(int64_t)a[2], (void*)(uintptr_t)a[3], (void*)(uintptr_t)a[4], f32(a[5]), (int)(int64_t)a[6], (int)(int64_t)a[7], (void*)(uintptr_t)a[8], (size_t)a[9], (void*)(uintptr_t)a[10], (void*)(uintptr_t)a[11]); }
static int t_radet_merge_pairs(const uint64_t* a) { return radet_merge_pairs((void*)(uintptr_t)a[0], (void*)(uintptr_t)a[1], (size_t)a[2], (int)(int64_t)a[3], (int)(int64_t)a[4], (void*)(uintptr_t)a[5], (void*)(uintptr_t)a[6]); }
static int t_radet_merge_planes(const uint64_t* a) { return radet_merge_planes((void*)(uintptr_t)a[0], (void*)(uintptr_t)a[1], (size_t)a[2], (int)(int64_t)a[3], (int)(int64_t)a[4], (void*)(uintptr_t)a[5]); }
static int t_radet_nchw_to_nhwc(const uint64_t* a) { return radet_nchw_to_nhwc((void*)(uintptr_t)a[0], (void*)(uintptr_t)a[1], (int)(int64_t)a[2], (int)(int64_t)a[3], (int)(int64_t)a[4], (int)(int64_t)a[5], (void*)(uintptr_t)a[6]); }
static int t_radet_nhwc_to_nchw(const uint64_t* a) { return radet_nhwc_to_nchw((void*)(uintptr_t)a[0], (void*)(uintptr_t)a[1], (int)(int64_t)a[2], (int)(int64_t)a[3], (int)(int64_t)a[4], (int)(int64_t)a[5], (void*)(uintptr_t)a[6]); }
static int t_radet_nms(const uint64_t* a) { return radet_nms((void*)(uintptr_t)a[0], (void*)(uintptr_t)a[1], (void*)(uintptr_t)a[2], (void*)(uintptr_t)a[3], (void*)(uintptr_t)a[4], (int)(int64_t)a[5], (int)(int64_t)a[6], (int)(int64_t)a[7], f32(a[8]), (int)(int64_t)a[9], f32(a[10]), (int)(int64_t)a[11], (void*)(uintptr_t)a[12], (void*)(uintptr_t)a[13], (void*)(uintptr_t)a[14], (void*)(uintptr_t)a[15], (void*)(uintptr_t)a[16], (void*)(uintptr_t)a[17], (void*)(uintptr_t)a[18], (void*)(uintptr_t)a[19]); }
static int t_radet_paste_maps(const uint64_t* a) { return radet_paste_maps((void*)(uintptr_t)a[0], (size_t)a[1], (int)(int64_t)a[2], (void*)(uintptr_t)a[3], (int)(int64_t)a[4], (int)(int64_t)a[5], (int)(int64_t)a[6], (void*)(uintptr_t)a[7], (void*)(uintptr_t)a[8]); }
static int t_radet_pred3x3_patch(const uint64_t* a) { return radet_pred3x3_patch((void*)(uintptr_t)a[0], (int)(int64_t)a[1], (void*)(uintptr_t)a[2], (int)(int64_t)a[3], (void*)(uintptr_t)a[4], (void*)(uintptr_t)a[5], (void*)(uintptr_t)a[6], (int)(int64_t)a[7], (void*)(uintptr_t)a[8], (void*)(uintptr_t)a[9], (void*)(uintptr_t)a[10], (int)(int64_t)a[11], (void*)(uintptr_t)a[12]); }
static int t_radet_preprocess_frames(const uint64_t* a) { return radet_preprocess_frames((void*)(uintptr_t)a[0], (int)(int64_t)a[1], (int)(int64_t)a[2], (int)(int64_t)a[3], f32(a[4]), f32(a[5]), f32(a[6]), f32(a[7]), f32(a[8]), f32(a[9]), (void*)(uintptr_t)a[10], (void*)(uintptr_t)a[11]); }
static int t_radet_relu_bwd(const uint64_t* a) { return radet_relu_bwd((void*)(uintptr_t)a[0], (void*)(uintptr_t)a[1], (void*)(uintptr_t)a[2], (void*)(uintptr_t)a[3], (size_t)a[4], (void*)(uintptr_t)a[5]); }
static int t_radet_relu_bwd_a(const uint64_t* a) { return radet_relu_bwd_a((void*)(uintptr_t)a[0], (void*)(uintptr_t)a[1], (void*)(uintptr_t)a[2], (void*)(uintptr_t)a[3], (size_t)a[4], (void*)(uintptr_t)a[5], (void*)(uintptr_t)a[6]); }
static int t_radet_relu_bwd_h(const uint64_t* a) { return radet_relu_bwd_h((void*)(uintptr_t)a[0], (void*)(uintptr_t)a[1], (void*)(uintptr_t)a[2], (void*)(uintptr_t)a[3], (size_t)a[4], (void*)(uintptr_t)a[5]); }
static int t_radet_resize_linear_f(const uint64_t* a) { return radet_resize_linear_f((void*)(uintptr_t)a[0], (void*)(uintptr_t)a[1], (void*)(uintptr_t)a[2], (void*)(uintptr_t)a[3], (int)(int64_t)a[4], (int)(int64_t)a[5], (int)(int64_t)a[6], (void*)(uintptr_t)a[7]); }
static int t_radet_resize_linear_u8(const uint64_t* a) { return radet_resize_linear_u8((void*)(uintptr_t)a[0], (void*)(uintptr_t)a[1], (void*)(uintptr_t)a[2], (void*)(uintptr_t)a[3], (void*)(uintptr_t)a[4], (int)(int64_t)a[5], (int)(int64_t)a[6], (int)(int64_t)a[7], (void*)(uintptr_t)a[8]); }
static int t_radet_rle_masks(const uint64_t* a) { return radet_rle_masks((void*)(uintptr_t)a[0], (int)(int64_t)a[1], (void*)(uintptr_t)a[2], (int)(int64_t)a[3], (void*)(uintptr_t)a[4], (void*)(uintptr_t)a[5], (int)(int64_t)a[6], (void*)(uintptr_t)a[7], (void*)(uintptr_t)a[8], (int)(int64_t)a[9], (int)(int64_t)a[10], (int)(int64_t)a[11], (int)(int64_t)a[12], (int)(int64_t)a[13], (void*)(uintptr_t)a[14]); }
static int t_radet_scale_relu(const uint64_t* a) { return radet_scale_relu((void*)(uintptr_t)a[0], (void*)(uintptr_t)a[1], (void*)(uintptr_t)a[2], (void*)(uintptr_t)a[3], (int)(int64_t)a[4], (int)(int64_t)a[5], (void*)(uintptr_t)a[6]); }
static int t_radet_sgd_step(const uint64_t* a) { return radet_sgd_step((void*)(uintptr_t)a[0], (void*)(uintptr_t)a[1], (void*)(uintptr_t)a[2], (size_t)a[3], f32(a[4]), f32(a[5]), f32(a[6]), f32(a[7]), (int)(int64_t)a[8], (int)(int64_t)a[9], f32(a[10]), f32(a[11]), (void*)(uintptr_t)a[12], (int)(int64_t)a[13], (void*)(uintptr_t)a[14], (void*)(uintptr_t)a[15], (int)(int64_t)a[16], (void*)(uintptr_t)a[17]); }
static int t_radet_sigmoid_focal_loss(const uint64_t* a) { return radet_sigmoid_focal_loss((void*)(uintptr_t)a[0], (void*)(uintptr_t)a[1], (void*)(uintptr_t)a[2], (int)(int64_t)a[3], (size_t)a[4], (int)(int64_t)a[5], f32(a[6]), f32(a[7]), (void*)(uintptr_t)a[8], f32(a[9]), (void*)(uintptr_t)a[10], (void*)(uintptr_t)a[11]); }
static int t_radet_sigmoid_focal_loss_bwd(const uint64_t* a) { return radet_sigmoid_focal_loss_bwd((void*)(uintptr_t)a[0], (void*)(uintptr_t)a[1], (void*)(uintptr_t)a[2], (int)(int64_t)a[3], (size_t)a[4], (int)(int64_t)a[5], f32(a[6]), f32(a[7]), (void*)(uintptr_t)a[8], (void*)(uintptr_t)a[9], (void*)(uintptr_t)a[10], f32(a[11]), (void*)(uintptr_t)a[12], (void*)(uintptr_t)a[13]); }
static int t_radet_sobel_edge(const uint64_t* a) { return radet_sobel_edge((void*)(uintptr_t)a[0], (void*)(uintptr_t)a[1], (void*)(uintptr_t)a[2], (void*)(uintptr_t)a[3], (void*)(uintptr_t)a[4], (int)(int64_t)a[5], (int)(int64_t)a[6], (void*)(uintptr_t)a[7]); }
static int t_radet_split_pairs(const uint64_t* a) { return radet_split_pairs((void*)(uintptr_t)a[0], (void*)(uintptr_t)a[1], (size_t)a[2], (int)(int64_t)a[3], (int)(int64_t)a[4], (void*)(uintptr_t)a[5], (void*)(uintptr_t)a[6], (void*)(uintptr_t)a[7]); }
static int t_radet_split_planes(const uint64_t* a) { return radet_split_planes((void*)(uintptr_t)a[0], (void*)(uintptr_t)a[1], (size_t)a[2], (int)(int64_t)a[3], (int)(int64_t)a[4], (void*)(uintptr_t)a[5]); }
static int t_radet_sqnorm_partials(const uint64_t* a) { return radet_sqnorm_partials((void*)(uintptr_t)a[0], (size_t)a[1], (void*)(uintptr_t)a[2], (int)(int64_t)a[3], (void*)(uintptr_t)a[4]); }
static int t_radet_stem_conv_bn_relu(const uint64_t* a) { return radet_stem_conv_bn_relu((void*)(uintptr_t)a[0], (void*)(uintptr_t)a[1], (void*)(uintptr_t)a[2], (void*)(uintptr_t)a[3], (int)(int64_t)a[4], (int)(int64_t)a[5], (int)(int64_t)a[6], (void*)(uintptr_t)a[7]); }
static int t_radet_stem_conv_bn_relu_a(const uint64_t* a) { return radet_stem_conv_bn_relu_a((void*)(uintptr_t)a[0], (void*)(uintptr_t)a[1], (void*)(uintptr_t)a[2], (void*)(uintptr_t)a[3], (int)(int64_t)a[4], (int)(int64_t)a[5], (int)(int64_t)a[6], (void*)(uintptr_t)a[7], (void*)(uintptr_t)a[8]); }
static int t_radet_stem_conv_bn_relu_h(const uint64_t* a) { return radet_stem_conv_bn_relu_h((void*)(uintptr_t)a[0], (void*)(uintptr_t)a[1], (void*)(uintptr_t)a[2], (void*)(uintptr_t)a[3], (int)(int64_t)a[4], (int)(int64_t)a[5], (int)(int64_t)a[6], (void*)(uintptr_t)a[7]); }
static int t_radet_stem_wgrad(const uint64_t* a) { return radet_stem_wgrad((void*)(uintptr_t)a[0], (void*)(uintptr_t)a[1], (void*)(uintptr_t)a[2], (void*)(uintptr_t)a[3], (int)(int64_t)a[4], (int)(int64_t)a[5], (int)(int64_t)a[6], (int)(int64_t)a[7], (void*)(uintptr_t)a[8]); }
static int t_radet_stem_wgrad_splits(const uint64_t* a) { return radet_stem_wgrad_splits((int)(int64_t)a[0], (int)(int64_t)a[1], (int)(int64_t)a[2]); }
static int t_radet_stream_create_cumask(const uint64_t* a) { return radet_stream_create_cumask((void*)(uintptr_t)a[0], (int)(int64_t)a[1], (void*)(uintptr_t)a[2]); }
static int t_radet_tblr_decode(const uint64_t* a) { return radet_tblr_decode((void*)(uintptr_t)a[0], (void*)(uintptr_t)a[1], (void*)(uintptr_t)a[2], (int)(int64_t)a[3], (void*)(uintptr_t)a[4], (int)(int64_t)a[5], f32(a[6]), f32(a[7]), (int)(int64_t)a[8], (void*)(uintptr_t)a[9]); }
static int t_radet_tblr_encode(const uint64_t* a) { return radet_tblr_encode((void*)(uintptr_t)a[0], (void*)(uintptr_t)a[1], (void*)(uintptr_t)a[2], (int)(int64_t)a[3], (void*)(uintptr_t)a[4], (int)(int64_t)a[5], (void*)(uintptr_t)a[6]); }
static int t_radet_threshold_compact(const uint64_t* a) { return radet_threshold_compact((void*)(uintptr_t)a[0], (size_t)a[1], f32(a[2]), (void*)(uintptr_t)a[3], (void*)(uintptr_t)a[4], (void*)(uintptr_t)a[5]); }
static int t_radet_unfold_grads(const uint64_t* a) { return radet_unfold_grads((void*)(uintptr_t)a[0], (int)(int64_t)a[1], (int)(int64_t)a[2], (void*)(uintptr_t)a[3]); }
static int t_radet_upsample_add(const uint64_t* a) { return radet_upsample_add((void*)(uintptr_t)a[0], (void*)(uintptr_t)a[1], (int)(int64_t)a[2], (int)(int64_t)a[3], (int)(int64_t)a[4], (int)(int64_t)a[5], (int)(int64_t)a[6], (int)(int64_t)a[7], (void*)(uintptr_t)a[8]); }
static int t_radet_upsample_add_a(const uint64_t* a) { return radet_upsample_add_a((void*)(uintptr_t)a[0], (void*)(uintptr_t)a[1], (int)(int64_t)a[2], (int)(int64_t)a[3], (int)(int64_t)a[4], (int)(int64_t)a[5], (int)(int64_t)a[6], (int)(int64_t)a[7], (void*)(uintptr_t)a[8], (void*)(uintptr_t)a[9]); }
static int t_radet_upsample_add_bwd(const uint64_t* a) { return radet_upsample_add_bwd((void*)(uintptr_t)a[0], (void*)(uintptr_t)a[1], (int)(int64_t)a[2], (int)(int64_t)a[3], (int)(int64_t)a[4], (int)(int64_t)a[5], (int)(int64_t)a[6], (int)(int64_t)a[7], (void*)(uintptr_t)a[8]); }
static int t_radet_upsample_add_bwd_a(const uint64_t* a) { return radet_upsample_add_bwd_a((void*)(uintptr_t)a[0], (void*)(uintptr_t)a[1], (int)(int64_t)a[2], (int)(int64_t)a[3], (int)(int64_t)a[4], (int)(int64_t)a[5], (int)(int64_t)a[6], (int)(int64_t)a[7], (void*)(uintptr_t)a[8], (void*)(uintptr_t)a[9]); }
static int t_radet_upsample_add_bwd_h(const uint64_t* a) { return radet_upsample_add_bwd_h((void*)(uintptr_t)a[0], (void*)(uintptr_t)a[1], (int)(int64_t)a[2], (int)(int64_t)a[3], (int)(int64_t)a[4], (int)(int64_t)a[5], (int)(int64_t)a[6], (int)(int64_t)a[7], (void*)(uintptr_t)a[8]); }
static int t_radet_upsample_add_h(const uint64_t* a) { return radet_upsample_add_h((void*)(uintptr_t)a[0], (void*)(uintptr_t)a[1], (int)(int64_t)a[2], (int)(int64_t)a[3], (int)(int64_t)a[4], (int)(int64_t)a[5], (int)(int64_t)a[6], (int)(int64_t)a[7], (void*)(uintptr_t)a[8]); }
static int t_radet_warp_affine_u8(const uint64_t* a) { return radet_warp_affine_u8((void*)(uintptr_t)a[0], (size_t)a[1], (void*)(uintptr_t)a[2], (size_t)a[3], (void*)(uintptr_t)a[4], (int)(int64_t)a[5], (int)(int64_t)a[6], (int)(int64_t)a[7], (void*)(uintptr_t)a[8]); }

typedef int (*radet_thunk_fn)(const uint64_t*);
const struct RadetTapeThunk { const char* name; radet_thunk_fn fn; int nargs; } radet_tape_thunks[] = {
    {"radet_absmax", t_radet_absmax, 4},
    {"radet_adamw_step", t_radet_adamw_step, 17},
    {"radet_adamw_step_runs", t_radet_adamw_step_runs, 19},
    {"radet_amax_slot_words", t_radet_amax_slot_words, 0},
    {"radet_assign_points", t_radet_assign_points, 19},
    {"radet_assign_points_f", t_radet_assign_points_f, 19},
    {"radet_augment_box", t_radet_augment_box, 8},
    {"radet_augment_finish", t_radet_augment_finish, 14},
    {"radet_augment_hsv_noise", t_radet_augment_hsv_noise, 6},
    {"radet_augment_merge_hblur", t_radet_augment_merge_hblur, 8},
    {"radet_augment_sharp", t_radet_augment_sharp, 7},
    {"radet_augment_vblur", t_radet_augment_vblur, 7},
    {"radet_bbox_overlaps", t_radet_bbox_overlaps, 10},
    {"radet_bce_logits_loss", t_radet_bce_logits_loss, 10},
    {"radet_bce_logits_loss_bwd", t_radet_bce_logits_loss_bwd, 12},
    {"radet_box_loss", t_radet_box_loss, 11},
    {"radet_box_loss_bwd", t_radet_box_loss_bwd, 13},
    {"radet_build_gather_table", t_radet_build_gather_table, 11},
    {"radet_coco_accumulate", t_radet_coco_accumulate, 17},
    {"radet_coco_match", t_radet_coco_match, 17},
    {"radet_conv2d_igemm", t_radet_conv2d_igemm, 17},
    {"radet_conv2d_igemm_classes", t_radet_conv2d_igemm_classes, 19},
    {"radet_conv2d_igemm_classes_s", t_radet_conv2d_igemm_classes_s, 20},
    {"radet_conv2d_igemm_pair", t_radet_conv2d_igemm_pair, 23},
    {"radet_conv2d_igemm_pair_s", t_radet_conv2d_igemm_pair_s, 24},
    {"radet_conv2d_igemm_s", t_radet_conv2d_igemm_s, 18},
    {"radet_conv2d_igemm_taps", t_radet_conv2d_igemm_taps, 17},
    {"radet_conv2d_igemm_taps_s", t_radet_conv2d_igemm_taps_s, 18},
    {"radet_conv2d_wgrad", t_radet_conv2d_wgrad, 14},
    {"radet_conv2d_wgrad_group", t_radet_conv2d_wgrad_group, 4},
    {"radet_conv2d_wgrad_s", t_radet_conv2d_wgrad_s, 15},
    {"radet_conv2d_wgrad_splits", t_radet_conv2d_wgrad_splits, 5},
    {"radet_convert_rows", t_radet_convert_rows, 10},
    {"radet_copy_d2d", t_radet_copy_d2d, 4},
    {"radet_copy_segments", t_radet_copy_segments, 4},
    {"radet_crop_canvases", t_radet_crop_canvases, 11},
    {"radet_cutout_f32", t_radet_cutout_f32, 17},
    {"radet_cutout_u8", t_radet_cutout_u8, 10},
    {"radet_decode_candidates", t_radet_decode_candidates, 19},
    {"radet_fill_zero", t_radet_fill_zero, 3},
    {"radet_fold_weights", t_radet_fold_weights, 3},
    {"radet_gather_table_rows", t_radet_gather_table_rows, 1},
    {"radet_gaussian_blur9_u8", t_radet_gaussian_blur9_u8, 8},
    {"radet_gdt", t_radet_gdt, 8},
    {"radet_giou_loss", t_radet_giou_loss, 9},
    {"radet_giou_loss_bwd", t_radet_giou_loss_bwd, 11},
    {"radet_gn_relu_bwd", t_radet_gn_relu_bwd, 16},
    {"radet_gn_relu_bwd_h", t_radet_gn_relu_bwd_h, 16},
    {"radet_gn_relu_bwd_p", t_radet_gn_relu_bwd_p, 17},
    {"radet_gn_relu_bwd_q", t_radet_gn_relu_bwd_q, 20},
    {"radet_gn_relu_fwd", t_radet_gn_relu_fwd, 14},
    {"radet_gn_relu_fwd_h", t_radet_gn_relu_fwd_h, 14},
    {"radet_gn_relu_fwd_p", t_radet_gn_relu_fwd_p, 15},
    {"radet_gn_relu_fwd_pair", t_radet_gn_relu_fwd_pair, 20},
    {"radet_gn_relu_fwd_pair_h", t_radet_gn_relu_fwd_pair_h, 20},
    {"radet_gn_relu_fwd_pair_p", t_radet_gn_relu_fwd_pair_p, 22},
    {"radet_gn_relu_fwd_pair_q", t_radet_gn_relu_fwd_pair_q, 28},
    {"radet_gn_relu_fwd_q", t_radet_gn_relu_fwd_q, 18},
    {"radet_gn_workspace_floats", t_radet_gn_workspace_floats, 3},
    {"radet_grad_accumulate", t_radet_grad_accumulate, 5},
    {"radet_grid_anchors", t_radet_grid_anchors, 5},
    {"radet_head_loss", t_radet_head_loss, 31},
    {"radet_head_loss_ws_ints", t_radet_head_loss_ws_ints, 1},
    {"radet_jpeg_decode", t_radet_jpeg_decode, 17},
    {"radet_jpeg_index", t_radet_jpeg_index, 11},
    {"radet_loss_finalize", t_radet_loss_finalize, 6},
    {"radet_loss_partials", t_radet_loss_partials, 1},
    {"radet_mask_max", t_radet_mask_max, 5},
    {"radet_mask_transform", t_radet_mask_transform, 14},
    {"radet_maxpool3x3s2", t_radet_maxpool3x3s2, 7},
    {"radet_maxpool3x3s2_a", t_radet_maxpool3x3s2_a, 8},
    {"radet_maxpool3x3s2_bwd_relu", t_radet_maxpool3x3s2_bwd_relu, 8},
    {"radet_maxpool3x3s2_h", t_radet_maxpool3x3s2_h, 7},
    {"radet_maxpool3x3s2_q", t_radet_maxpool3x3s2_q, 11},
    {"radet_mbd", t_radet_mbd, 12},
    {"radet_merge_pairs", t_radet_merge_pairs, 7},
    {"radet_merge_planes", t_radet_merge_planes, 6},
    {"radet_nchw_to_nhwc", t_radet_nchw_to_nhwc, 7},
    {"radet_nhwc_to_nchw", t_radet_nhwc_to_nchw, 7},
    {"radet_nms", t_radet_nms, 20},
    {"radet_paste_maps", t_radet_paste_maps, 9},
    {"radet_pred3x3_patch", t_radet_pred3x3_patch, 13},
    {"radet_preprocess_frames", t_radet_preprocess_frames, 12},
    {"radet_relu_bwd", t_radet_relu_bwd, 6},
    {"radet_relu_bwd_a", t_radet_relu_bwd_a, 7},
    {"radet_relu_bwd_h", t_radet_relu_bwd_h, 6},
    {"radet_resize_linear_f", t_radet_resize_linear_f, 8},
    {"radet_resize_linear_u8", t_radet_resize_linear_u8, 9},
    {"radet_rle_masks", t_radet_rle_masks, 15},
    {"radet_scale_relu", t_radet_scale_relu, 7},
    {"radet_sgd_step", t_radet_sgd_step, 18},
    {"radet_sigmoid_focal_loss", t_radet_sigmoid_focal_loss, 12},
    {"radet_sigmoid_focal_loss_bwd", t_radet_sigmoid_focal_loss_bwd, 14},
    {"radet_sobel_edge", t_radet_sobel_edge, 8},
    {"radet_split_pairs", t_radet_split_pairs, 8},
    {"radet_split_planes", t_radet_split_planes, 6},
    {"radet_sqnorm_partials", t_radet_sqnorm_partials, 5},
    {"radet_stem_conv_bn_relu", t_radet_stem_conv_bn_relu, 8},
    {"radet_stem_conv_bn_relu_a", t_radet_stem_conv_bn_relu_a, 9},
    {"radet_stem_conv_bn_relu_h", t_radet_stem_conv_bn_relu_h, 8},
    {"radet_stem_wgrad", t_radet_stem_wgrad, 9},
    {"radet_stem_wgrad_splits", t_radet_stem_wgrad_splits, 3},
    {"radet_stream_create_cumask", t_radet_stream_create_cumask, 3},
    {"radet_tblr_decode", t_radet_tblr_decode, 10},
    {"radet_tblr_encode", t_radet_tblr_encode, 7},
    {"radet_threshold_compact", t_radet_threshold_compact, 6},
    {"radet_unfold_grads", t_radet_unfold_grads, 4},
    {"radet_upsample_add", t_radet_upsample_add, 9},
    {"radet_upsample_add_a", t_radet_upsample_add_a, 10},
    {"radet_upsample_add_bwd", t_radet_upsample_add_bwd, 9},
    {"radet_upsample_add_bwd_a", t_radet_upsample_add_bwd_a, 10},
    {"radet_upsample_add_bwd_h", t_radet_upsample_add_bwd_h, 9},
    {"radet_upsample_add_h", t_radet_upsample_add_h, 9},
    {"radet_warp_affine_u8", t_radet_warp_affine_u8, 9},
};
const int radet_tape_nthunks = 114;
```

radet_amd/engine.py:

```python
import contextlib
import ctypes as C
import os

import torch

from . import _lib
from . import kernels as K
from .kernels import ConvGeom, Levels

ARCH = {50: (3, 4, 6, 3), 101: (3, 4, 23, 3)}


def conv_out_hw(h, w, k, s, p):
    return (h + 2 * p - k) // s + 1, (w + 2 * p - k) // s + 1


class _StemSplits:

    def __init__(self, nsplit):
        self.nsplit = nsplit


class Conv:

    def __init__(self, name, cin, cout, k, stride, pad, bn=None, bias=False, trainable=True, dgrad=True):
        self.name, self.cin, self.cout, self.k, self.stride, self.pad = name, cin, cout, k, stride, pad
        self.bn, self.bias, self.trainable, self.need_dgrad = bn, bias, trainable, dgrad
        self.wft_ld, self.wft_off, self.wft_shared = 0, 0, None
        self.grouped = False
        self.geom = None
        self.wf = self.wft = self.bias_f = self.slabs = self.dbias_partials = None

    @property
    def wsize(self):
        return self.cout * self.cin * self.k * self.k


class Engine:
    def __init__(self, params, grads, depth=50, num_classes=21, frozen_stages=1, strides=(8, 16, 32, 64, 128),
                 stacked_convs=4, feat=256, math=None, watch=None):
        math = math or os.environ.get("RADET_MATH", "fp32")
        assert math in ("fp32", "fp32-mfma", "bf16", "bf16-storage"), math
        self.watch = watch or {}
        self._watched = {}
        self.math = 1 if math == "bf16" else 0
        self.h16 = math == "bf16-storage"
        x3mode = os.environ.get("RADET_X3", "h2")
        self.x3 = math == "fp32" and x3mode != "0"
        self.h2 = self.x3 and x3mode not in ("bf16", "b3")
        self.pairs = self.h2 and os.environ.get("RADET_PAIRS", "0") == "1"
        self.po = self.h2 and not self.pairs and os.environ.get("RADET_PAIRS_ONLY", "0") == "1"
        self.po_max_planes = int(os.environ.get("RADET_PAIRS_ONLY_MAX", "512"))
        self.pairs_from = int(os.environ.get("RADET_PAIRS_FROM", "2"))
        if self.x3 and "RADET_TOWER_MODE" not in os.environ:
            self.tower_mode = "pairbwd"
        self.p3 = self.x3 and self.tower_mode == "pairbwd" and feat % 32 == 0 and os.environ.get("RADET_P3", "1") != "0"
        self.math_name = math
        self.act_dtype = torch.bfloat16 if self.h16 else torch.float32
        self.p, self.g = params, grads
        self.depth, self.num_classes, self.frozen_stages = depth, num_classes, frozen_stages
        self.strides, self.stacked_convs, self.feat = tuple(strides), stacked_convs, feat
        self.dev = next(iter(params.values())).device
        self.convs = []
        self._build_layers()
        self._alloc_folded()
        self.geo_key = None
        self.table = None

    TOWER_TAG = K.SYMBOL | K.BK32 | 3
    TOWER_TAG_FWD = K.SYMBOL | K.BK32 | 2

    tower_stages = K.STAGES3 if os.environ.get("RADET_TOWER_STAGES3", "0") == "1" else 0
    tower_tile = int(os.environ.get("RADET_TOWER_TILE", "6"))
    if os.environ.get("RADET_TOWER_ROWPAIRS", "0") == "1":
        tower_tile |= K.ROWPAIRS

    def _ttile(self, c, bwd=False, tag=True, pair=True):
        fp32 = not self.math and not self.h16
        if self.p3:
            return (6 if pair else 5) | (K.SYMBOL if tag else 0) | self.tower_stages
        if fp32 and self.x3:
            t = K.BK32 | 1
        elif bwd:
            t = (self.TOWER_TAG & ~K.SYMBOL) if fp32 else (self.tower_bwd_tile_h16 or c.geom.bwd_tile)
        else:
            t = (self.TOWER_TAG_FWD & ~K.SYMBOL) | (K.STAGES3 if fp32 else 0)
            if not fp32 and self.tower_fwd_tile_h16:
                t = self.tower_fwd_tile_h16
        return t | (K.SYMBOL if tag else 0)
    tower_fwd_tile_h16 = int(os.environ.get("RADET_TOWER_FWD_TILE", "0"), 0)
    tower_bwd_tile_h16 = int(os.environ.get("RADET_TOWER_BWD_TILE", str(K.BK32 | 1)), 0)
    tower_events = None
    _pfx_ready = None

    def _tower_launch(self, fn, *args, **kw):
        ev = self.tower_events
        if ev is None:
            return fn(*args, **kw)
        s, e = torch.cuda.Event(enable_timing=True), torch.cuda.Event(enable_timing=True)
        s.record()
        fn(*args, **kw)
        e.record()
        ev.append((s, e))

    def tower_gemm_flops(self):
        return 2.0 * self.R * self.feat * 9 * self.feat

    def _add(self, conv):
        self.convs.append(conv)
        return conv

    def _build_layers(self):
        fs = self.frozen_stages
        if fs < 0 and self.h16:
            raise NotImplementedError("ResNet(frozen_stages=-1) (trainable stem) with bf16 storage is not implemented on MI355X: "
                                      "every RADet config freezes the stem (frozen_stages >= 0; the BOP configs use 1)")
        self.stem = self._add(Conv("backbone.conv1", 3, 64, 7, 2, 3, bn="backbone.bn1", trainable=fs < 0, dgrad=False))
        self.stages = []
        inpl = 64
        for li, nb in enumerate(ARCH[self.depth]):
            planes = 64 * 2 ** li
            train = (li + 1) > fs
            blocks = []
            for b in range(nb):
                pfx = f"backbone.layer{li + 1}.{b}"
                stride = 2 if (b == 0 and li > 0) else 1
                in_dgrad = train and not (b == 0 and li <= fs)
                blk = dict(
                    c1=self._add(Conv(pfx + ".conv1", inpl, planes, 1, 1, 0, bn=pfx + ".bn1", trainable=train, dgrad=in_dgrad)),
                    c2=self._add(Conv(pfx + ".conv2", planes, planes, 3, stride, 1, bn=pfx + ".bn2", trainable=train, dgrad=train)),
                    c3=self._add(Conv(pfx + ".conv3", planes, planes * 4, 1, 1, 0, bn=pfx + ".bn3", trainable=train, dgrad=train)),
                    ds=None, stride=stride, train=train,
                    po=self.po and stride == 1 and planes % 32 == 0 and planes <= self.po_max_planes)
                if b == 0:
                    blk["ds"] = self._add(Conv(pfx + ".downsample.0", inpl, planes * 4, 1, stride, 0, bn=pfx + ".downsample.1",
                                               trainable=train, dgrad=in_dgrad))
                inpl = planes * 4
                blocks.append(blk)
            self.stages.append(blocks)
        f = self.feat
        self.lat = [self._add(Conv(f"neck.lateral_convs.{i}.conv", c, f, 1, 1, 0, bias=True)) for i, c in enumerate((512, 1024, 2048))]
        self.fpn = [self._add(Conv(f"neck.fpn_convs.{i}.conv", f, f, 3, 1 if i < 3 else 2, 1, bias=True)) for i in range(5)]
        self.cls_tower = [self._add(Conv(f"bbox_head.cls_convs.{i}.conv", f, f, 3, 1, 1)) for i in range(self.stacked_convs)]
        self.reg_tower = [self._add(Conv(f"bbox_head.reg_convs.{i}.conv", f, f, 3, 1, 1)) for i in range(self.stacked_convs)]
        self.pred_cls = self._add(Conv("bbox_head.atss_cls", f, self.num_classes, 3, 1, 1, bias=True))
        self.pred_reg = self._add(Conv("bbox_head.atss_reg", f, 4, 3, 1, 1, bias=True))
        self.pred_iou = self._add(Conv("bbox_head.atss_centerness", f, 1, 3, 1, 1, bias=True))
        kq = 32 if self.h16 else 16
        self.cls_pad = ((self.num_classes + kq - 1) // kq) * kq
        self.ri_pad = kq
        self.iou_col = 8 if self.h16 else 4
        self.pred_cls.wft_ld, self.pred_cls.wft_off = self.cls_pad, 0
        self.pred_reg.wft_ld, self.pred_reg.wft_off = self.ri_pad, 0
        self.pred_iou.wft_ld, self.pred_iou.wft_off = self.ri_pad, self.iou_col
        self.pred_iou.wft_shared = self.pred_reg

    def _alloc_folded(self):
        dev = self.dev
        n_wf = sum(c.wsize for c in self.convs)
        n_b = sum(c.cout for c in self.convs)
        self.wf_arena = torch.zeros(n_wf, device=dev, dtype=self.act_dtype)
        self.stem_wf = torch.zeros(self.convs[0].wsize, device=dev)
        self.bias_arena = torch.zeros(n_b, device=dev)
        n_wft = 0
        for c in self.convs:
            if c.need_dgrad and c.wft_shared is None:
                ld = c.wft_ld or c.cout
                n_wft += c.cin * c.k * c.k * ld
        self.wft_arena = torch.zeros(n_wft, device=dev, dtype=self.act_dtype)
        self.w_amax = K.new_amax(dev, len(self.convs))
        self.w_l1 = K.new_amax(dev, len(self.convs)) if (self.pairs or self.po) else None
        self.b_amax = K.new_amax(dev, len(self.convs)) if (self.pairs or self.po) else None
        self.w_l1t = K.new_amax(dev, len(self.convs)) if self.po else None
        self._w_amax_keys = []
        o_w = o_b = o_t = 0
        towers = (self.cls_tower + self.reg_tower) if self.p3 else []
        po_c1 = [blk["c1"] for st in self.stages for blk in st if blk["po"]]
        po_c2 = [blk["c2"] for st in self.stages for blk in st if blk["po"]]
        po_c3 = [blk["c3"] for st in self.stages for blk in st if blk["po"] and blk["train"]]
        towers = towers + po_c2
        pkind = "h2" if self.h2 else "b3"
        for ci, c in enumerate(self.convs):
            c.w_amax = self.w_amax[ci]
            c.wfq = None
            c.wmeta = (self.w_l1[ci], self.b_amax[ci] if (c.bn or c.bias) else None) if (self.pairs or c in po_c1) else None
            c.wmeta_t = (self.w_l1t[ci], None) if c in po_c3 else None
            c.w16 = (3 if self.h2 else 2) if c in towers else (1 if (self.h16 and c is not self.convs[0]) else 0)
            c.wf = self.wf_arena[o_w:o_w + c.wsize] if c is not self.convs[0] else self.stem_wf
            o_w += c.wsize
            c.bias_f = self.bias_arena[o_b:o_b + c.cout]
            o_b += c.cout
            if c.need_dgrad:
                if c.wft_shared is not None:
                    c.wft = c.wft_shared.wft
                else:
                    n = c.cin * c.k * c.k * (c.wft_ld or c.cout)
                    c.wft = self.wft_arena[o_t:o_t + n]
                    o_t += n
            if c.w16 >= 2:
                c.wf = K.Planes(c.cout * c.k * c.k, c.cin, device=dev, kind=pkind, amax=c.w_amax)
                c.wft = K.Planes(c.cin * c.k * c.k, c.cout, device=dev, kind=pkind, amax=c.w_amax) if c.need_dgrad else None
            elif self.h2 and c is not self.convs[0]:
                if self.pairs and c.name.startswith(("backbone.layer", "neck.lateral")) and c.cin % 32 == 0 and \
                        (not c.name.startswith("backbone.layer") or int(c.name[14]) >= self.pairs_from):
                    c.wfq = K.Planes(c.cout * c.k * c.k, c.cin, device=dev, kind="h2", amax=c.w_amax)
                self._w_amax_keys.append(K.register_amax(c.wf, c.w_amax))
                if c.need_dgrad and c.wft_shared is None:
                    self._w_amax_keys.append(K.register_amax(c.wft, c.w_amax))

    max_plans = int(os.environ.get("RADET_MAX_PLANS", "4"))
    _PLAN_ATTRS = ("B", "H", "W", "stem_hw", "pool_hw", "buf", "plv", "R", "gn_ws", "gn_ws2", "ldesc", "nlvl", "loss_ws",
                   "losses", "dscales", "slab_arena", "bp_arena", "table", "_table_keepalive", "max_cout", "_pending_wgrad",
                   "amax_act", "amax_aux", "_amax_keys", "amax_pfx", "_pfx_shapes", "_pfx_sets", "_pfx_active", "_pfx_ready",
                   "plan_id")

    def _snapshot(self):
        return dict(attrs={k: getattr(self, k) for k in self._PLAN_ATTRS},
                    convs=[(c.geom, c.slabs, c.dbias_partials, c.grouped) for c in self.convs],
                    blocks=[[(blk.get("lin"), blk.get("lout")) for blk in blocks] for blocks in self.stages])

    def _restore(self, plan):
        for k, v in plan["attrs"].items():
            setattr(self, k, v)
        for c, (g, sl, bp, gr) in zip(self.convs, plan["convs"]):
            c.geom, c.slabs, c.dbias_partials, c.grouped = g, sl, bp, gr
        for blocks, saved in zip(self.stages, plan["blocks"]):
            for blk, (lin, lout) in zip(blocks, saved):
                blk["lin"], blk["lout"] = lin, lout

    def prepare(self, B, H, W):
        key = (B, H, W)
        if self.geo_key == key:
            return
        if not hasattr(self, "_plans"):
            import collections
            self._plans = collections.OrderedDict()
        if self.geo_key is not None:
            self._plans[self.geo_key] = self._snapshot()
            requested = self._plans.pop(key, None)
            while len(self._plans) >= max(self.max_plans, 1):
                torch.cuda.synchronize()
                _, old = self._plans.popitem(last=False)
                K.unregister_amax(old["attrs"].get("_amax_keys") or [])
            if requested is not None:
                self._plans[key] = requested
        self.geo_key = key
        if key in self._plans:
            self._restore(self._plans.pop(key))
            return
        self.plans_built = getattr(self, "plans_built", 0) + 1
        self.plan_id = self.plans_built
        dev = self.dev
        self.B, self.H, self.W = B, H, W
        h1, w1 = conv_out_hw(H, W, 7, 2, 3)
        h2, w2 = conv_out_hw(h1, w1, 3, 2, 1)
        self.stem_hw, self.pool_hw = (h1, w1), (h2, w2)
        self.buf = {}
        self.amax_act = K.new_amax(dev, 768)
        self.amax_aux = K.new_amax(dev, 32)
        self._amax_keys = []
        n_slot = [0, 0]

        def slot(aux=False):
            i = n_slot[aux]
            n_slot[aux] += 1
            return (self.amax_aux if aux else self.amax_act)[i]

        self.amax_pfx = [K.new_amax(dev, 128), None]
        self._pfx_shapes = {}
        self._pfx_sets = [{}, None]
        self._pfx_active, self._pfx_ready = 0, None
        n_pfx = [0]

        def new(name, rows, ch, dtype=None, prefix=False, twin=False, only=False):
            if only:
                q = K.Planes(rows, ch, device=dev, kind="h2")
                if prefix:
                    assert n_pfx[0] < self.amax_pfx[0].shape[0], "frozen prefix: more buffers than amax slots"
                    q.true_amax = self.amax_pfx[0][n_pfx[0]]
                    n_pfx[0] += 1
                    self._pfx_shapes[name] = (rows, ch, "pairs-only", False)
                    self._pfx_sets[0][name] = q
                else:
                    q.true_amax = slot()
                self.buf[name] = q
                return q
            t = torch.empty(rows, ch, device=dev, dtype=dtype or self.act_dtype)
            self.buf[name] = t
            if prefix:
                self._pfx_shapes[name] = (rows, ch, t.dtype, twin and self.pairs)
                self._pfx_sets[0][name] = t
            sl_ = None
            if self.h2 and t.dtype == torch.float32:
                if prefix:
                    assert n_pfx[0] < self.amax_pfx[0].shape[0], "frozen prefix: more buffers than amax slots"
                    sl_ = self.amax_pfx[0][n_pfx[0]]
                    n_pfx[0] += 1
                else:
                    sl_ = slot()
                self._amax_keys.append(K.register_amax(t, sl_, by_storage=True))
            if twin and self.pairs and ch % 32 == 0:
                q = K.Planes(rows, ch, device=dev, kind="h2")
                q.true_amax = sl_
                self.buf[name + "@q"] = q
                if prefix:
                    self._pfx_sets[0][name + "@q"] = q
            return t

        frozen_prefix = not self.stem.trainable
        new("stem", B * h1 * w1, 64, prefix=frozen_prefix)
        new("pool", B * h2 * w2, 64, prefix=frozen_prefix, twin=self.pairs_from <= 1)
        if self.stem.trainable:
            new("d_pool", B * h2 * w2, 64)
            new("d_stem", B * h1 * w1, 64)
            self.stem.geom = _StemSplits(K.stem_wgrad_splits(B, H, W))
        lv = Levels([(h2, w2)], B)
        for li, blocks in enumerate(self.stages):
            for b, blk in enumerate(blocks):
                pfx = f"l{li + 1}.{b}"
                blk["lin"] = lv
                fz = frozen_prefix and not blk["train"] and all(not bb["train"] for st in self.stages[:li] for bb in st)
                blk["c1"].geom = ConvGeom(lv, blk["c1"].cin, blk["c1"].cout, 1, 1, 0)
                blk["c2"].geom = ConvGeom(lv, blk["c2"].cin, blk["c2"].cout, 3, blk["stride"], 1)
                lo = blk["c2"].geom.lout
                blk["c3"].geom = ConvGeom(lo, blk["c3"].cin, blk["c3"].cout, 1, 1, 0)
                if blk["ds"] is not None:
                    blk["ds"].geom = ConvGeom(lv, blk["ds"].cin, blk["ds"].cout, 1, blk["stride"], 0)
                    new(pfx + ".idt", lo.rows, blk["ds"].cout, prefix=fz)
                blk["lout"] = lo
                tw = li + 1 >= self.pairs_from
                new(pfx + ".o1", lv.rows, blk["c1"].cout, prefix=fz, twin=tw, only=blk["po"])
                new(pfx + ".o2", lo.rows, blk["c2"].cout, prefix=fz, twin=tw)
                new(pfx + ".out", lo.rows, blk["c3"].cout, prefix=fz, twin=tw or (li + 2 == self.pairs_from and b == len(blocks) - 1))
                if blk["train"]:
                    new(pfx + ".d_o1", lv.rows, blk["c1"].cout)
                    new(pfx + ".d_o2", lo.rows, blk["c2"].cout, only=blk["po"])
                    new(pfx + ".d_pre", lo.rows, blk["c3"].cout)
                lv = lo
        c_lv = [self.stages[i][-1]["lout"] for i in (1, 2, 3)]
        f = self.feat
        for i in range(3):
            self.lat[i].geom = ConvGeom(c_lv[i], self.lat[i].cin, f, 1, 1, 0)
            new(f"lat{i}", c_lv[i].rows, f)
            new(f"d_lat{i}", c_lv[i].rows, f)
            new(f"d_c{i}", c_lv[i].rows, self.lat[i].cin)
        hw = [c_lv[i].hw[0] for i in range(3)]
        hw.append(conv_out_hw(*hw[-1], 3, 2, 1))
        hw.append(conv_out_hw(*hw[-1], 3, 2, 1))
        self.plv = Levels(hw, B)
        if self.x3:
            K._pred_tiles(self.plv)
        for i in range(3):
            self.fpn[i].geom = ConvGeom(c_lv[i], f, f, 3, 1, 1)
        self.fpn[3].geom = ConvGeom(self.plv.sub(2), f, f, 3, 2, 1)
        self.fpn[4].geom = ConvGeom(self.plv.sub(3), f, f, 3, 2, 1)
        R = self.plv.rows
        self.R = R
        new("P", R, f)
        new("dP", R, f)
        for lvl in (2, 3):
            r0, r1 = self.plv.level_rows(lvl)
            new(f"dP_tmp{lvl}", r1 - r0, f)
        pkind = "h2" if self.h2 else "b3"
        if self.p3:
            self.buf["Pp"] = K.Planes(R, f, device=dev, kind=pkind)
        for t in ("cls", "reg"):
            for i in range(self.stacked_convs):
                new(f"{t}.z{i}", R, f)
                if self.p3 and i < self.stacked_convs - 1:
                    self.buf[f"{t}.y{i}"] = K.Planes(R, f, device=dev, kind=pkind)
                else:
                    new(f"{t}.y{i}", R, f)
                if self.h2:
                    self.buf[f"{t}.zhat{i}"] = slot(aux=True)
                self.buf[f"{t}.stats{i}"] = torch.empty(len(hw) * B * 64, device=dev)
            new(f"{t}.dy", R, f)
            for nm in (f"{t}.dz0", f"{t}.dz1"):
                if self.p3:
                    self.buf[nm] = K.Planes(R, f, device=dev, kind=pkind)
                else:
                    new(nm, R, f)
            self.buf[f"{t}.dz"] = self.buf[f"{t}.dz0"]
        for c in self.cls_tower + self.reg_tower:
            c.geom = ConvGeom(self.plv, f, f, 3, 1, 1)
            if self.p3 and self.h2:
                c.geom.nsplit = max(1, min(64, 256 // (-(-f // 128) * (f // 32)), (R + 127) // 128))
        for c in (self.pred_cls, self.pred_reg, self.pred_iou):
            c.geom = ConvGeom(self.plv, f, c.cout, 3, 1, 1)
        new("cls", R, self.num_classes, torch.float32)
        new("reg_u", R, 4, torch.float32)
        new("iou", R, 1, torch.float32)
        self.buf["dcls"] = torch.zeros(R, self.cls_pad, device=dev)
        self.buf["dregiou"] = torch.zeros(R, 16, device=dev)
        if self.h2:
            for nm in ("dcls", "dregiou"):
                self._amax_keys.append(K.register_amax(self.buf[nm], slot(), by_storage=True))
        if self.h16:
            self.buf["dcls16"] = torch.zeros(R, self.cls_pad, device=dev, dtype=torch.bfloat16)
            self.buf["dregiou16"] = torch.zeros(R, self.ri_pad, device=dev, dtype=torch.bfloat16)
        self.gn_ws = torch.empty(K.gn_ws_floats(self.plv), device=dev)
        self.gn_ws2 = torch.empty(K.gn_ws_floats(self.plv), device=dev)
        self.ldesc, self.nlvl = K.level_desc(self.plv, self.strides)
        self.loss_ws = torch.zeros(K.head_loss_ws_ints(R), dtype=torch.int32, device=dev)
        self.losses = torch.zeros(3, device=dev)
        self.dscales = torch.zeros(len(hw), device=dev)
        for c in self.convs:
            if c.geom is not None:
                c.geom.math = self.math
                c.geom.h16 = self.h16
                c.geom.x3 = self.x3
                c.geom.h2 = self.h2
                c.geom.pairs = c.wfq is not None or (self.po and c.w16 == 3 and c.name.startswith("backbone."))
        tune = os.environ.get("RADET_AUTOTUNE", "1") != "0"
        self._plan_wgrad_groups()
        if tune:
            K.load_tune_cache()
            for c in self.convs:
                if c.trainable and c.geom is not None and c.cout > 64 and c.cin > 64 and not c.grouped \
                        and c not in self.cls_tower and c not in self.reg_tower:
                    K.autotune_wgrad(c.geom)
        for c in self.convs:
            if c.geom is not None and hasattr(c.geom, "wgrad_pair_flags") and c not in self.cls_tower + self.reg_tower:
                c.geom.wgrad_pair_flags = K.WG_ONE_TAP | (c.geom.wgrad_flags & K.WG_TILE_MASK)
        n_slab = sum(c.geom.nsplit * c.wsize for c in self.convs if c.trainable)
        n_bp = sum(c.geom.nsplit * c.cout for c in self.convs if c.trainable)
        self.slab_arena = torch.empty(n_slab, device=dev)
        self.bp_arena = torch.zeros(n_bp, device=dev)
        o_s = o_b = 0
        for c in self.convs:
            if c.trainable:
                n = c.geom.nsplit * c.wsize
                c.slabs = self.slab_arena[o_s:o_s + n]
                o_s += n
                n = c.geom.nsplit * c.cout
                c.dbias_partials = self.bp_arena[o_b:o_b + n]
                o_b += n
        self._build_table()
        if tune:
            towers = self.cls_tower + self.reg_tower
            for c in self.convs:
                if c is not self.stem and c.geom is not None and (self.math or c not in towers):
                    K.autotune(c.geom, need_dgrad=c.need_dgrad)
            K.save_tune_cache()

    wgrad_group = os.environ.get("RADET_WGRAD_GROUP", "0") == "1"
    wgrad_group_tile = int(os.environ.get("RADET_WGRAD_GROUP_TILE", "128"))
    wgrad_group_slots = int(os.environ.get("RADET_WGRAD_GROUP_SLOTS", "512"))
    wgrad_flush_blocks = int(os.environ.get("RADET_WGRAD_FLUSH_BLOCKS", "0"))

    def _plan_wgrad_groups(self):
        for c in self.convs:
            c.grouped = False
        self._pending_wgrad = []
        if not self.wgrad_group or self.h16:
            return
        t = self.wgrad_group_tile
        fb = self.wgrad_flush_blocks
        groups = []
        for blocks in self.stages:
            rev = list(reversed(blocks))
            step = fb if fb > 0 else len(rev)
            for i in range(0, len(rev), step):
                groups.append([c for blk in rev[i:i + step] for c in (blk["c1"], blk["c2"], blk["c3"], blk["ds"])
                               if c is not None and c.trainable])
        groups.append(list(self.lat) + list(self.fpn))
        for grp in groups:
            grp = [c for c in grp if c.cout % t == 0 and c.cin % t == 0]
            if not grp:
                continue
            for c, s in zip(grp, K.group_splits([c.geom for c in grp], tile=t, slots=self.wgrad_group_slots)):
                c.grouped = True
                c.geom.nsplit = s

    def flush_wgrads(self):
        jobs, self._pending_wgrad = self._pending_wgrad, []
        if not jobs:
            return
        if not self.use_streams:
            K.conv_wgrad_group(jobs, tile=self.wgrad_group_tile, math=self.math)
            return
        side = self._side()
        self._fork(side)
        with torch.cuda.stream(side):
            K.conv_wgrad_group(jobs, tile=self.wgrad_group_tile, math=self.math)

    def _build_table(self):
        n = len(self.convs)
        arr = (_lib.RadetConvDesc * n)()

        def ptr(t):
            return None if t is None else C.c_void_p(t.data_ptr())

        for d, c in zip(arr, self.convs):
            p, g = self.p, self.g
            d.w = ptr(p[c.name + ".weight"])
            d.bias = ptr(p.get(c.name + ".bias")) if c.bias else None
            if c.bn:
                d.bn_gamma, d.bn_beta = ptr(p[c.bn + ".weight"]), ptr(p[c.bn + ".bias"])
                d.bn_mean, d.bn_var = ptr(p[c.bn + ".running_mean"]), ptr(p[c.bn + ".running_var"])
            d.wf, d.wft, d.bias_f = ptr(c.wf), ptr(c.wft) if c.need_dgrad else None, ptr(c.bias_f)
            d.cout, d.cin, d.kh, d.kw = c.cout, c.cin, c.k, c.k
            d.eps = 1e-5
            d.wft_ld, d.wft_off = c.wft_ld, c.wft_off
            d.w16 = c.w16
            d.w_amax = ptr(c.w_amax) if self.h2 else None
            if self.pairs and c is not self.convs[0]:
                d.wfq = ptr(c.wfq)
                d.w_l1, d.bias_amax = ptr(c.wmeta[0]), ptr(self.b_amax[self.convs.index(c)])
            if self.po and c.wmeta is not None:
                d.w_l1, d.bias_amax = ptr(c.wmeta[0]), ptr(self.b_amax[self.convs.index(c)])
            if c.wmeta_t is not None:
                d.w_l1t = ptr(c.wmeta_t[0])
            d.nsplit = c.geom.nsplit if c.geom is not None else 1
            if c.trainable and c.geom is not None:
                d.dwf_slabs, d.dbias_partials = ptr(c.slabs), ptr(c.dbias_partials)
                d.dw = ptr(g[c.name + ".weight"])
                if c.bias:
                    d.dbias = ptr(g[c.name + ".bias"])
                if c.bn:
                    d.dgamma, d.dbeta = ptr(g[c.bn + ".weight"]), ptr(g[c.bn + ".bias"])
        raw = bytes(arr)
        self.table = torch.frombuffer(bytearray(raw), dtype=torch.uint8).to(self.dev)
        self._table_keepalive = arr
        self.max_cout = max(c.cout for c in self.convs)

    _fold_event = None

    def fold(self):
        n = len(self.convs)
        nf = 0
        while nf < n and not self.convs[nf].trainable:
            nf += 1
        vf, vt = self._part_version(0, nf), self._part_version(nf, n) + (self._param_epoch,)
        do_f = nf > 0 and vf != self._folded[0]
        do_t = nf < n and vt != self._folded[1]
        if do_f:
            self._pfx_ready = None
            for plan in getattr(self, "_plans", {}).values():
                plan["attrs"]["_pfx_ready"] = None
        tail = self.table[nf * C.sizeof(_lib.RadetConvDesc):]
        if do_t and self.use_streams and nf > 0 and os.environ.get("RADET_FOLD_SIDE", "1") != "0":
            side = self._side()
            self._fork(side)
            with torch.cuda.stream(side):
                K.fold_weights(tail, n - nf)
                ev = self._event()
                K.ev_record(ev)
            self._fold_event = ev
            if do_f:
                K.fold_weights(self.table, nf)
        elif do_f and do_t:
            K.fold_weights(self.table, n)
        elif do_f:
            K.fold_weights(self.table, nf)
        elif do_t:
            K.fold_weights(tail, n - nf)
        self._folded = (vf, vt)
        self._last_fold = (do_f, do_t)

    def _frozen_conv_count(self):
        nf = 0
        while nf < len(self.convs) and not self.convs[nf].trainable:
            nf += 1
        return nf

    _last_fold = (None, None)
    _folded = (None, None)
    _param_epoch = 0
    _watched = None

    def _part_version(self, lo, hi):
        if os.environ.get("RADET_FOLD_EVERY_CALL"):
            return (object(),)
        key = (lo, hi)
        watched = self._watched.get(key)
        if watched is None:
            watched = []
            for c in self.convs[lo:hi]:
                names = [c.name + ".weight"] + ([c.name + ".bias"] if c.bias else [])
                if c.bn:
                    names += [c.bn + sfx for sfx in (".weight", ".bias", ".running_mean", ".running_var")]
                for k in names:
                    if k in self.p:
                        watched += list(self.watch.get(k, (self.p[k],)))
            self._watched[key] = watched
        return (tuple(t._version for t in watched), tuple(t.data_ptr() for t in watched), self.h16, self.math)

    def params_changed(self):
        self._param_epoch += 1

    def invalidate_fold(self):
        self._folded = (None, None)

    def _await_fold(self):
        if self._fold_event is not None:
            K.ev_wait(self._fold_event)
            self._fold_event = None

    def unfold(self):
        K.unfold_grads(self.table, len(self.convs), self.max_cout)

    def _block_forward(self, blk, pfx, x, b, xq=None):
        blk["x"] = x
        o1, o2, out = b[pfx + ".o1"], b[pfx + ".o2"], b[pfx + ".out"]
        c1, c2, c3, ds = blk["c1"], blk["c2"], blk["c3"], blk["ds"]
        if xq is not None and c1.wfq is not None and c2.wfq is not None and c3.wfq is not None and (ds is None or ds.wfq is not None):
            o1q, o2q, outq = b[pfx + ".o1@q"], b[pfx + ".o2@q"], b.get(pfx + ".out@q")
            K.conv_fwd(c1.geom, xq, c1.wfq, c1.bias_f, o1, relu=True, tile=c1.geom.fwd_tile_q, yq=o1q, wmeta=c1.wmeta)
            K.conv_fwd(c2.geom, o1q, c2.wfq, c2.bias_f, o2, relu=True, tile=c2.geom.fwd_tile_q, yq=o2q, wmeta=c2.wmeta)
            if ds is not None:
                idt = b[pfx + ".idt"]
                K.conv_fwd(ds.geom, xq, ds.wfq, ds.bias_f, idt, tile=ds.geom.fwd_tile_q)
            else:
                idt = x
            K.conv_fwd(c3.geom, o2q, c3.wfq, c3.bias_f, out, addend=idt, relu=True, tile=c3.geom.fwd_tile_q, yq=outq,
                       wmeta=c3.wmeta)
            return out
        if blk["po"]:
            K.conv_fwd(c1.geom, x, c1.wf, c1.bias_f, None, relu=True, yq=o1, wmeta=c1.wmeta)
            K.conv_fwd(c2.geom, o1, c2.wf, c2.bias_f, o2, relu=True, tile=c2.geom.fwd_tile_q)
        else:
            K.conv_fwd(blk["c1"].geom, x, blk["c1"].wf, blk["c1"].bias_f, o1, relu=True)
            K.conv_fwd(blk["c2"].geom, o1, blk["c2"].wf, blk["c2"].bias_f, o2, relu=True)
        if blk["ds"] is not None:
            idt = b[pfx + ".idt"]
            K.conv_fwd(blk["ds"].geom, x, blk["ds"].wf, blk["ds"].bias_f, idt)
        else:
            idt = x
        outq = b.get(pfx + ".out@q")
        K.conv_fwd(blk["c3"].geom, o2, blk["c3"].wf, blk["c3"].bias_f, out, addend=idt, relu=True, yq=outq,
                   wmeta=c3.wmeta if outq is not None else None)
        return out

    def _n_frozen_stages(self):
        n = 0
        while n < len(self.stages) and not self.stages[n][0]["train"]:
            n += 1
        return n

    def _prefix_forward(self, img, which):
        B, H, W = self.B, self.H, self.W
        b = self._pfx_sets[which]
        if self.h2:
            K.fill_zero(self.amax_pfx[which])
        K.STAGE = "stem"
        K.stem(img, self.stem.wf, self.stem.bias_f, b["stem"], B, H, W)
        K.maxpool(b["stem"], b["pool"], B, self.stem_hw[0], self.stem_hw[1], 64, yq=b.get("pool@q"))
        x, xq = b["pool"], b.get("pool@q")
        for li in range(self._n_frozen_stages()):
            K.STAGE = f"layer{li + 1}"
            for bi, blk in enumerate(self.stages[li]):
                x = self._block_forward(blk, f"l{li + 1}.{bi}", x, b, xq)
                xq = b.get(f"l{li + 1}.{bi}.out@q")
        return b

    @staticmethod
    def _img_key(img, geo):
        return (img.data_ptr(), img._version, tuple(img.shape), geo)

    def prefetch_prefix(self, next_img):
        if self.stem.trainable or not self.use_streams or next_img is None or self.geo_key is None:
            return False
        if tuple(next_img.shape) != (self.B, 3, self.H, self.W) or not next_img.is_contiguous():
            return False
        other = 1 - self._pfx_active
        if self._pfx_sets[other] is None:
            self._pfx_sets[other] = {}
            if self.h2:
                self.amax_pfx[other] = K.new_amax(self.dev, 128)
            for i, (name, (rows, ch, dt, twin)) in enumerate(self._pfx_shapes.items()):
                if dt == "pairs-only":
                    q = K.Planes(rows, ch, device=self.dev, kind="h2")
                    q.true_amax = self.amax_pfx[other][i]
                    self._pfx_sets[other][name] = q
                    continue
                t = torch.empty(rows, ch, device=self.dev, dtype=dt)
                self._pfx_sets[other][name] = t
                if self.h2 and dt == torch.float32:
                    self._amax_keys.append(K.register_amax(t, self.amax_pfx[other][i], by_storage=True))
                if twin:
                    q = K.Planes(rows, ch, device=self.dev, kind="h2")
                    q.true_amax = self.amax_pfx[other][i]
                    self._pfx_sets[other][name + "@q"] = q
        cs = self._chain_stream()
        self._fork(cs)
        stage = K.STAGE
        if self._pfx_event is None:
            self._pfx_event = torch.cuda.Event()
        ev = self._pfx_event
        with torch.cuda.stream(cs):
            self._prefix_forward(next_img, other)
            K.ev_record(ev)
        K.STAGE = stage
        self._pfx_ready = (self._img_key(next_img, self.geo_key), other, ev, next_img)
        return True

    _pfx_event = None

    def backbone_forward(self, img):
        b = self.buf
        self._img = img if self.stem.trainable else None
        if self.h2:
            K.fill_zero(self.amax_act)
        nf = self._n_frozen_stages() if not self.stem.trainable else 0
        rdy, self._pfx_ready = self._pfx_ready, None
        if not self.stem.trainable and rdy is not None and rdy[3] is img and rdy[0] == self._img_key(img, self.geo_key):
            K.ev_wait(rdy[2])
            self._pfx_active = rdy[1]
            pb = self._pfx_sets[self._pfx_active]
        elif not self.stem.trainable:
            pb = self._prefix_forward(img, self._pfx_active)
        else:
            K.STAGE = "stem"
            K.stem(img, self.stem.wf, self.stem.bias_f, b["stem"], self.B, self.H, self.W)
            K.maxpool(b["stem"], b["pool"], self.B, self.stem_hw[0], self.stem_hw[1], 64, yq=b.get("pool@q"))
            pb = b
        if not self.stem.trainable:
            b.update(pb)
        last = "pool" if nf == 0 else f"l{nf}.{len(self.stages[nf - 1]) - 1}.out"
        x, xq = pb[last], pb.get(last + "@q")
        outs = [pb[f"l{li + 1}.{len(self.stages[li]) - 1}.out"] for li in range(nf)]
        for li in range(nf, len(self.stages)):
            blocks = self.stages[li]
            K.STAGE = f"layer{li + 1}"
            if blocks[0]["train"]:
                self._await_fold()
            for bi, blk in enumerate(blocks):
                x = self._block_forward(blk, f"l{li + 1}.{bi}", x, b, xq)
                xq = b.get(f"l{li + 1}.{bi}.out@q")
            outs.append(x)
        return outs


    def neck_forward(self, feats):
        K.STAGE = "neck"
        self._await_fold()
        b, B = self.buf, self.B
        c = feats[1:]
        for i in range(3):
            cq = b.get(f"l{i + 2}.{len(self.stages[i + 1]) - 1}.out@q")
            if cq is not None and self.lat[i].wfq is not None:
                K.conv_fwd(self.lat[i].geom, cq, self.lat[i].wfq, self.lat[i].bias_f, b[f"lat{i}"], tile=self.lat[i].geom.fwd_tile_q)
            else:
                K.conv_fwd(self.lat[i].geom, c[i], self.lat[i].wf, self.lat[i].bias_f, b[f"lat{i}"])
        hw = self.plv.hw
        for i in (2, 1):
            K.upsample_add(b[f"lat{i - 1}"], b[f"lat{i}"], B, hw[i - 1][0], hw[i - 1][1], hw[i][0], hw[i][1], self.feat)
        P = b["P"]
        for i in range(3):
            r0, r1 = self.plv.level_rows(i)
            K.conv_fwd(self.fpn[i].geom, b[f"lat{i}"], self.fpn[i].wf, self.fpn[i].bias_f, P[r0:r1])
        for i in (3, 4):
            s0, s1 = self.plv.level_rows(i - 1)
            r0, r1 = self.plv.level_rows(i)
            K.conv_fwd(self.fpn[i].geom, P[s0:s1], self.fpn[i].wf, self.fpn[i].bias_f, P[r0:r1])
        return P

    use_streams = True

    _SHARED_STREAMS = {}

    def _shared_stream(self, role):
        key = (torch.device(self.dev).index if torch.device(self.dev).index is not None else torch.cuda.current_device(), role)
        st = Engine._SHARED_STREAMS.get(key)
        if st is None:
            mask = os.environ.get("RADET_WGRAD_CU_MASK")
            if mask and role in ("side", "side2"):
                words = (C.c_uint32 * 8)(*([int(mask, 0) & 0xFFFFFFFF] * 8))
                out = C.c_void_p()
                with torch.cuda.device(self.dev):
                    _lib.check(_lib.load().radet_stream_create_cumask(words, 8, C.byref(out)), "radet_stream_create_cumask")
                st = torch.cuda.ExternalStream(out.value, device=self.dev)
            else:
                st = torch.cuda.Stream(device=self.dev)
            Engine._SHARED_STREAMS[key] = st
        return st

    def caller_stream(self):
        key = (torch.device(self.dev).index if torch.device(self.dev).index is not None else torch.cuda.current_device(), "caller")
        st = Engine._SHARED_STREAMS.get(key)
        if st is None:
            touch = [self._side(), self._side2(), self._chain_stream()]
            touch += [torch.cuda.Stream(device=self.dev) for _ in range(2)]
            Engine._SHARED_STREAMS[key + ("placeholders",)] = touch[3:]
            st = Engine._SHARED_STREAMS[key] = torch.cuda.Stream(device=self.dev)
            for t in touch + [st]:
                with torch.cuda.stream(t):
                    torch.zeros(1, device=self.dev)
            torch.cuda.synchronize(self.dev)
        return st

    def _side(self):
        if getattr(self, "_side_stream", None) is None:
            self._side_stream = self._shared_stream("side")
            self._events = [torch.cuda.Event() for _ in range(2048)]
            self._ev_i = 0
        return self._side_stream

    def _chain_stream(self):
        if getattr(self, "_chain", None) is None:
            self._side()
            self._chain = self._shared_stream("chain")
        return self._chain

    def _event(self):
        self._ev_i = (self._ev_i + 1) % len(self._events)
        return self._events[self._ev_i]

    def _fork(self, side):
        ev = self._event()
        K.ev_record(ev)
        K.ev_wait(ev, side)

    def _join(self, side):
        ev = self._event()
        K.ev_record(ev, side)
        K.ev_wait(ev)

    wgrad_pairs = os.environ.get("RADET_WGRAD_PAIRS", "0") == "1"

    def _wgrad_pairs_ok(self, geom, dy, x):
        return (self.h2 and self.wgrad_pairs and not K._isp(dy) and geom.cin % 32 == 0 and geom.cout % 32 == 0
                and dy.dtype == torch.float32 and dy.dim() == 2 and dy.shape[1] == geom.cout and x.shape[1] == geom.cin)

    def _wgrad_via_pairs(self, geom, dy, x, slabs, dbias_partials):
        key = torch.cuda.current_stream().cuda_stream
        sc = self._pair_scratch.get(key)
        need = max(dy.numel(), x.numel())
        if sc is None or sc[0].numel() < 2 * need:
            n = max(2 * need, 2 * self._pair_scratch_elems())
            sc = self._pair_scratch[key] = (torch.empty(n, dtype=torch.float16, device=self.dev),
                                            torch.empty(n, dtype=torch.float16, device=self.dev), K.new_amax(self.dev, 2))
        dyq = K.Planes(dy.shape[0], geom.cout, t=sc[0][:2 * dy.numel()].view(dy.shape[0], 2 * geom.cout), kind="h2", amax=sc[2][0])
        xq = K.Planes(x.shape[0], geom.cin, t=sc[1][:2 * x.numel()].view(x.shape[0], 2 * geom.cin), kind="h2", amax=sc[2][1])
        K.split_planes(dy, dyq)
        K.split_planes(x, xq)
        K.conv_wgrad(geom, dyq, xq, slabs, dbias_partials)

    def _pair_scratch_elems(self):
        return max((max(c.geom.lout.rows * c.cout, c.geom.lin.rows * c.cin) for c in self.convs
                    if c.trainable and c.geom is not None and hasattr(c.geom, "lout")), default=0)

    _pair_scratch = None

    def _wgrad_async(self, geom, dy, x, slabs, dbias_partials=None, conv=None):
        if conv is not None and conv.grouped:
            self._pending_wgrad.append(dict(g=geom, dy=dy, x=x, slabs=slabs, dbias=dbias_partials))
            return None
        if self._pair_scratch is None:
            self._pair_scratch = {}
        wg = self._wgrad_via_pairs if self._wgrad_pairs_ok(geom, dy, x) else K.conv_wgrad
        if not self.use_streams:
            wg(geom, dy, x, slabs, dbias_partials)
            return None
        side = self._side()
        if self.wgrad_streams > 1:
            self._wg_i = getattr(self, "_wg_i", 0) + 1
            if self._wg_i & 1:
                side = self._side2()
                self._side2_dirty = True
        self._fork(side)
        with torch.cuda.stream(side):
            wg(geom, dy, x, slabs, dbias_partials)
            ev = self._event()
            K.ev_record(ev)
        return ev

    wgrad_streams = int(os.environ.get("RADET_WGRAD_STREAMS", "2"))
    _side2_dirty = False

    def _side2(self):
        if getattr(self, "_side2_stream", None) is None:
            self._side()
            self._side2_stream = self._shared_stream("side2")
        return self._side2_stream

    def side_collect(self):
        if self._side2_dirty:
            ev = self._event()
            K.ev_record(ev, self._side2_stream)
            K.ev_wait(ev, self._side())
            self._side2_dirty = False

    def join_side(self):
        if self.use_streams and getattr(self, "_side_stream", None) is not None:
            self.side_collect()
            self._join(self._side_stream)

    def _gn_fwd(self, z, gamma, beta, y, stats, ws):
        if self.h2 and not K._isp(y):
            K.gn_relu_fwd_q(self.plv, z, gamma, beta, y, None, stats, ws)
        else:
            K.gn_relu_fwd(self.plv, z, gamma, beta, y, stats, ws)

    def _gn_bwd(self, dy, z, stats, gamma, beta, dz, dgamma, dbeta, ws):
        K.gn_relu_bwd(self.plv, dy, z, stats, gamma, beta, dz, dgamma, dbeta, ws)
        if self.h2 and not K._isp(dz) and dz.dtype == torch.float32:
            sl = K.amax_slot(dz)
            if sl is not None:
                K.absmax(dz, sl)

    def _tower_fwd_layer(self, t, tower, i, x, ws):
        b, p = self.buf, self.p
        c = tower[i]
        z, y = b[f"{t}.z{i}"], b[f"{t}.y{i}"]
        self._tower_launch(K.conv_fwd, c.geom, x, c.wf, None, z, tile=self._ttile(c))
        gn = f"bbox_head.{t}_convs.{i}.gn"
        self._gn_fwd(z, p[gn + ".weight"], p[gn + ".bias"], y, b[f"{t}.stats{i}"], ws)
        return y

    tower_fwd_streams = os.environ.get("RADET_TOWER_FWD_STREAMS", "1") != "0"

    def _tower_fwd_layer_p(self, t, tower, i, x, ws):
        b, p = self.buf, self.p
        c = tower[i]
        z, y = b[f"{t}.z{i}"], b[f"{t}.y{i}"]
        self._tower_launch(K.conv_fwd, c.geom, x, c.wf, None, z, tile=self.tower_tile | K.SYMBOL | K.splitk(1) | self.tower_stages)
        gn = f"bbox_head.{t}_convs.{i}.gn"
        pl = K._isp(y)
        if self.h2:
            K.gn_relu_fwd_q(self.plv, z, p[gn + ".weight"], p[gn + ".bias"], None if pl else y, y if pl else None,
                            b[f"{t}.stats{i}"], ws, zhat_amax=b[f"{t}.zhat{i}"])
            return y
        K.gn_relu_fwd_p(self.plv, z, p[gn + ".weight"], p[gn + ".bias"], None if pl else y, y if pl else None,
                        b[f"{t}.stats{i}"], ws)
        return y

    tower_mode = os.environ.get("RADET_TOWER_MODE", "hybrid")

    def _tower_pair_fwd(self, i, xc, xr):
        b, p = self.buf, self.p
        cc, cr = self.cls_tower[i], self.reg_tower[i]
        zc, yc, zr, yr = b[f"cls.z{i}"], b[f"cls.y{i}"], b[f"reg.z{i}"], b[f"reg.y{i}"]
        self._tower_launch(K.conv_fwd_pair, cc.geom, dict(x=xc, w=cc.wf, y=zc), dict(x=xr, w=cr.wf, y=zr),
                           tile=self._ttile(cc))
        gc, gr = f"bbox_head.cls_convs.{i}.gn", f"bbox_head.reg_convs.{i}.gn"
        if self.p3:
            pl = K._isp(yc)
            if self.h2:
                K.gn_relu_fwd_pair_q(self.plv, (zc, p[gc + ".weight"], p[gc + ".bias"], None if pl else yc, yc if pl else None,
                                                b[f"cls.stats{i}"], self.gn_ws, b[f"cls.zhat{i}"]),
                                     (zr, p[gr + ".weight"], p[gr + ".bias"], None if pl else yr, yr if pl else None,
                                      b[f"reg.stats{i}"], self.gn_ws2, b[f"reg.zhat{i}"]))
                return yc, yr
            K.gn_relu_fwd_pair_p(self.plv, (zc, p[gc + ".weight"], p[gc + ".bias"], None if pl else yc, yc if pl else None,
                                            b[f"cls.stats{i}"], self.gn_ws),
                                 (zr, p[gr + ".weight"], p[gr + ".bias"], None if pl else yr, yr if pl else None,
                                  b[f"reg.stats{i}"], self.gn_ws2))
            return yc, yr
        if self.h2:
            K.gn_relu_fwd_pair_q(self.plv, (zc, p[gc + ".weight"], p[gc + ".bias"], yc, None, b[f"cls.stats{i}"], self.gn_ws, None),
                                 (zr, p[gr + ".weight"], p[gr + ".bias"], yr, None, b[f"reg.stats{i}"], self.gn_ws2, None))
            return yc, yr
        K.gn_relu_fwd_pair(self.plv, (zc, p[gc + ".weight"], p[gc + ".bias"], yc, b[f"cls.stats{i}"], self.gn_ws),
                           (zr, p[gr + ".weight"], p[gr + ".bias"], yr, b[f"reg.stats{i}"], self.gn_ws2))
# ... 349 lines not shown
```

radet_amd/kernels.py:

```python
import ctypes as C
import os

import torch

from . import _lib

ID_MASK = 0xFF
SYMBOL = 0x100
BK32 = 0x200
MATH_BF16 = 0x400
STORE_BF16, OUT_F32 = 0x800, 0x10000
SPLITK, SPLITK_MASK = 0x1000, 0xF000
STAGES3 = 0x20000
STAGES4 = 0x40000
ROWPAIRS = 0x80000
STREAMK, STREAMK_MASK = 0x100000, 0x700000
X3 = 0x1000000
P3 = 0x2000000
H2 = 0x8000000
MASKQ = 0x10000000
WG_MATH_BF16, WG_STORE_BF16 = 0x1, 0x2
WG_TILE, WG_TILE_MASK = 0x10, 0x30
WG_ONE_TAP = 0x40
WG_PX32 = 0x80
# ... 452 lines not shown
def autotune(g, need_dgrad=True, reps=None):
    dev = torch.device("cuda", torch.cuda.current_device())
    reps = reps or TUNE_REPS

    def best_of(fn, cands):
        for t in cands:
            fn(t)
        torch.cuda.synchronize()
        best = [float("inf")] * len(cands)
        for _ in range(reps):
            for i, t in enumerate(cands):
                s, e = torch.cuda.Event(enable_timing=True), torch.cuda.Event(enable_timing=True)
                s.record()
                for _b in range(TUNE_BURST):
                    fn(t)
                e.record()
                e.synchronize()
                best[i] = min(best[i], s.elapsed_time(e) / TUNE_BURST)
        return cands[min(range(len(cands)), key=lambda i: (best[i], i))]

    def cands(kdim, n, m, taps):
        tiles = [4] if n <= 32 else [1, 2, 3]
        c = [t for t in tiles]
        if kdim % 32 == 0:
            c += [t | BK32 for t in tiles]
        if getattr(g, "x3", False) and not g.math and not g.h16 and n > 32:
            c += ([7] if kdim % 64 == 0 else []) + ([8] if kdim % 32 == 0 else [])
            if _h2key(g) and kdim % 32 == 0 and KW_DEEP:
                c += [8 | STAGES3, 8 | STAGES4]
        out = list(c)
        for t in c:
            ntiles = _ntiles(t, m, n)
            nk = taps * kdim // (64 if tile_id(t) == 7 else (32 if (t & BK32 or tile_id(t) == 8) else 16))
            out += _splitk_cands(t, m, n, nk)
            if ntiles < 1024 and not g.math and not g.h16 and tile_id(t) in (2, 3, 4) and ntiles % 256:
                out += [t | streamk(w) for w in (1, 2, 3, 4) if ntiles * nk >= 256 * w]
        return out

    global _TUNE_DIRTY, TUNE_RUNS
    key = (g._key, g.cin, g.cout, g.math, g.h16) + (("x3",) if getattr(g, "x3", False) else ()) + _h2key(g)
    if key not in _TUNE_CACHE:
        _TUNE_DIRTY = True
        TUNE_RUNS += 1
        dt = torch.bfloat16 if g.h16 else torch.float32
        x = torch.randn(g.lin.rows, g.cin, device=dev).to(dt)
        w = (torch.randn(g.cout * g.k * g.k * g.cin, device=dev) * 0.05).to(dt)
        y = torch.empty(g.lout.rows, g.cout, device=dev, dtype=dt)
        tmp_keys = _tune_slots(g, x, w, outputs=(y,))
        fc = cands(g.cin, g.cout, g.lout.rows, g.k * g.k)
        if not g.math and not g.h16:
            fc = fc + [t | STAGES3 for t in fc if tile_id(t) < 7 and not t & (STAGES3 | STAGES4)]
        ft = best_of(lambda t: conv_fwd(g, x, w, None, y, relu=True, tile=t), fc)
        bt = 0
        if need_dgrad and g.cout % 16 == 0:
            dx = torch.empty(g.lin.rows, g.cin, device=dev, dtype=dt)
            tmp_keys += _tune_slots(g, outputs=(dx,))
            bt = best_of(lambda t: conv_dgrad(g, y, w, dx, mask=x, tile=t), cands(g.cout, g.cin, g.lin.rows, g.k * g.k))
        _TUNE_CACHE[key] = (ft, bt)
        unregister_amax(tmp_keys)
        if os.environ.get("RADET_TUNE_LOG"):
            print(f"[tune igemm] M={g.lout.rows} {g.cin}->{g.cout} k{g.k}s{g.stride}: fwd tile={ft:#x} dgrad tile={bt:#x}")
    g.fwd_tile, g.bwd_tile = _TUNE_CACHE[key]
    if getattr(g, "pairs", False) and _h2key(g) and g.cin % 32 == 0:
        keyq = key + ("q",)
        if keyq not in _TUNE_CACHE:
            _TUNE_DIRTY = True
            TUNE_RUNS += 1
            x = torch.randn(g.lin.rows, g.cin, device=dev)
            w = torch.randn(g.cout * g.k * g.k, g.cin, device=dev) * 0.05
            xq, wq = Planes.from_float(x, kind="h2"), Planes.from_float(w, kind="h2")
            y = torch.empty(g.lout.rows, g.cout, device=dev)
            cq = [1, 2, 3, 1 | STAGES3, 2 | STAGES3, 3 | STAGES3] + ([7] if g.cin % 64 == 0 else [])
            for t in list(cq):
                cq += _splitk_cands(t, g.lout.rows, g.cout, g.k * g.k * g.cin // (64 if tile_id(t) == 7 else 32))
            ftq = best_of(lambda t: conv_fwd(g, xq, wq, None, y, relu=True, tile=t), cq)
            btq = 0
            if need_dgrad and g.stride == 1 and g.cout % 32 == 0:
                dyq = Planes.from_float(torch.randn(g.lout.rows, g.cout, device=dev), kind="h2")
                wtq = Planes.from_float(torch.randn(g.cin * g.k * g.k, g.cout, device=dev) * 0.05, kind="h2")
                dx = torch.empty(g.lin.rows, g.cin, device=dev)
                tmp_q = _tune_slots(g, outputs=(dx,))
                cb = [1, 2, 3] + ([7] if g.cout % 64 == 0 else [])
                for t in list(cb):
                    cb += _splitk_cands(t, g.lin.rows, g.cin, g.k * g.k * g.cout // (64 if tile_id(t) == 7 else 32))
                btq = best_of(lambda t: conv_dgrad(g, dyq, wtq, dx, mask=xq, tile=t), cb)
                unregister_amax(tmp_q)
            _TUNE_CACHE[keyq] = (ftq, btq)
            if os.environ.get("RADET_TUNE_LOG"):
                print(f"[tune igemm pairs] M={g.lout.rows} {g.cin}->{g.cout} k{g.k}s{g.stride}: fwd tile={ftq:#x} dgrad tile={btq:#x}")
        g.fwd_tile_q, g.bwd_tile_q = _TUNE_CACHE[keyq]


KW_DEEP = os.environ.get("RADET_KW_DEEP", "1") != "0"


def _h2key(g):
    return ("h2",) if (getattr(g, "h2", False) and getattr(g, "x3", False) and not g.math and not g.h16) else ()


def _tune_slots(g, *tensors, outputs=()):
    keys = []
    if _h2key(g):
        for t in tensors:
            s = new_amax(t.device)
            if t.is_floating_point() and t.dtype == torch.float32 and t.is_contiguous() and t.numel() % 4 == 0:
                absmax(t, s)
            elif t.is_floating_point() and t.dtype == torch.float32:
                s.fill_(int(t.abs().max().view(torch.int32)) if t.numel() else 0)
            keys.append(register_amax(t, s))
        for t in outputs:
            t.zero_()
            keys.append(register_amax(t, new_amax(t.device)))
    return keys


AMAX_WORDS = 64
_AMAX_EXACT = {}
_AMAX_STORAGE = {}


def new_amax(device, n=None):
    global AMAX_WORDS
    AMAX_WORDS = _lib.load().radet_amax_slot_words()
    return torch.zeros((AMAX_WORDS,) if n is None else (n, AMAX_WORDS), dtype=torch.int32, device=device)


def amax_value(slot):
    return float(slot.max().view(torch.float32))


def register_amax(t, slot, by_storage=False):
    import weakref
    if by_storage:
        k = ("s", t.untyped_storage().data_ptr())
        _AMAX_STORAGE[k[1]] = (slot, weakref.ref(t))
    else:
        k = ("e", t.data_ptr())
        _AMAX_EXACT[k[1]] = (slot, weakref.ref(t))
    return k


def _live(table, ptr):
    ent = table.get(ptr)
    if ent is None:
        return None
    if ent[1]() is None:
        del table[ptr]
        return None
    return ent


def unregister_amax(keys):
    for kind, ptr in keys:
        (_AMAX_STORAGE if kind == "s" else _AMAX_EXACT).pop(ptr, None)
    _AMAX_MEMO.clear()
    _SCALES.clear()


_AMAX_MEMO = {}


def amax_slot(t, compute=False):
    if t is None:
        return None
    if _isp(t):
        return t.amax
    p = t.data_ptr()
    ent = _live(_AMAX_EXACT, p)
    if ent is None:
        ent = _live(_AMAX_MEMO, p)
        if ent is None and _AMAX_STORAGE:
            ent = _live(_AMAX_STORAGE, t.untyped_storage().data_ptr())
            if ent is not None:
                _AMAX_MEMO[p] = ent
    s = ent[0] if ent is not None else None
    if s is None and compute:
        s = new_amax(t.device)
        absmax(t, s)
    return s


def absmax(t, slot):
    assert t.dtype == torch.float32 and t.is_contiguous()
    _lib.call("radet_absmax", _ptr(t), C.c_size_t(t.numel()), _ptr(slot), _stream())


_SCALES = _LRU(4096)


def _scales(x, w, y, x1=None, w1=None, y1=None, need=True, yq=None, wmeta=None, addend=None):
    sx, sw, sy = amax_slot(x, need), amax_slot(w, need), amax_slot(y)
    if y is None and yq is not None:
        sy = getattr(yq, "true_amax", None)
    sx1, sw1, sy1 = amax_slot(x1, need), amax_slot(w1, need), amax_slot(y1)
    if not need and sy is None and sy1 is None and yq is None:
        return None
    ext = (None,) * 6
    if yq is not None:
        xt = getattr(x, "true_amax", None) if _isp(x) else amax_slot(x, True)
        assert xt is not None and wmeta is not None, "pair copy of a conv output: the true amax slot of x and the conv's L1 slot"
        ext = (yq.t, yq.amax, xt, wmeta[0], wmeta[1], amax_slot(addend, True) if addend is not None else None)
    slots = (sx, sw, sy, sx1, sw1, sy1) + ext
    key = tuple(0 if t is None else t.data_ptr() for t in slots)
    ent = _SCALES.get(key)
    if ent is None:
        sc = _lib.RadetScales(*[None if v == 0 else v for v in key])
        ent = _SCALES[key] = (C.byref(sc), sc, slots)
    return ent[0]


class Planes:

    def __init__(self, rows, C, device=None, t=None, kind="b3", amax=None):
        self.rows, self.C, self.kind = int(rows), int(C), kind
        if t is None:
            t = (torch.empty(self.rows, 2 * self.C, device=device, dtype=torch.float16) if kind == "h2"
                 else torch.empty(self.rows, 3 * self.C, device=device, dtype=torch.bfloat16))
        self.t = t
        self.amax = amax
        if kind == "h2" and amax is None:
            self.amax = new_amax(t.device)

    def __getitem__(self, sl):
        assert isinstance(sl, slice) and sl.step in (None, 1)
        v = self.t[sl]
        return Planes(v.shape[0], self.C, t=v, kind=self.kind, amax=self.amax)

    def data_ptr(self):
        return self.t.data_ptr()

    def to_float(self):
        out = torch.empty(self.rows, self.C, device=self.t.device)
        merge_planes(self, out)
        return out

    @staticmethod
    def from_float(x, kind="b3"):
        p = Planes(x.shape[0], x.shape[1], device=x.device, kind=kind)
        split_planes(x, p)
        return p


def _isp(t):
    return isinstance(t, Planes)


def _ptr_any(t):
    return _ptr(t.t) if _isp(t) else _ptr(t)


def split_planes(src, dst, src_amax=None):
    assert src.dim() == 2 and src.dtype == torch.float32 and src.stride(1) == 1 and dst.C == src.shape[1]
    if dst.kind == "h2":
        sa = src_amax if src_amax is not None else amax_slot(src)
        if sa is None:
            sa = new_amax(src.device)
            absmax(src.contiguous(), sa)
        _lib.call("radet_split_pairs", src.data_ptr(), _ptr(dst.t), C.c_size_t(src.shape[0]), src.shape[1], src.stride(0),
                  _ptr(sa), _ptr(dst.amax), _stream())
        return
    _lib.call("radet_split_planes", C.c_void_p(src.data_ptr()), _ptr(dst.t), C.c_size_t(src.shape[0]), src.shape[1],
              src.stride(0), _stream())


def merge_planes(src, dst):
    assert dst.dim() == 2 and dst.dtype == torch.float32 and dst.stride(1) == 1 and src.C == dst.shape[1]
    if src.kind == "h2":
        _lib.call("radet_merge_pairs", _ptr(src.t), dst.data_ptr(), C.c_size_t(dst.shape[0]), dst.shape[1], dst.stride(0),
                  _ptr(src.amax), _stream())
        return
    _lib.call("radet_merge_planes", _ptr(src.t), C.c_void_p(dst.data_ptr()), C.c_size_t(dst.shape[0]), dst.shape[1],
              dst.stride(0), _stream())


def _is16(t):
    return t is not None and not _isp(t) and t.dtype == torch.bfloat16


def _tile(g, tile, default, x=None, y=None):
    t = (tile or default) | (MATH_BF16 if g.math else 0)
    if _isp(x):
        if tile_id(t) == 8:
            t = with_tile(t, 3)
        return (t & ~(MATH_BF16 | BK32)) | P3 | (H2 if x.kind == "h2" else 0)
    if getattr(g, "x3", False) and not g.math and not _is16(x):
        t |= X3 | (H2 if getattr(g, "h2", False) else 0)
    if _is16(x):
        t = (t & ~MATH_BF16) | STORE_BF16 | (OUT_F32 if (y is not None and y.dtype == torch.float32) else 0)
    return t


def conv_fwd(g, x, wf, bias, y, addend=None, mask=None, relu=False, tile=0, splitk=True, yq=None, wmeta=None):
    assert y is not None or yq is not None
    tile = _tile(g, tile, g.fwd_tile, x, y)
    ws = splitk_ws() if splitk else None
    table = g.fwd_table
    sc = _scales(x, wf, y, need=bool(tile & H2), yq=yq, wmeta=wmeta, addend=addend)

    def launch():
        _lib.call("radet_conv2d_igemm_s", _ptr_any(x), _ptr_any(wf), _ptr(bias), _ptr(addend), _ptr(mask), _ptr(y), _ptr(table),
                  g.lout.rows, g.cin, g.cout, g.k, g.k, int(relu), tile, _ptr(ws), C.c_size_t(ws.numel() if splitk else 0),
                  _stream(), sc)
    _timed(lambda: _igemm_key(tile, x), 2.0 * g.lout.rows * g.cout * g.cin * g.k * g.k, launch, _conv_bytes(g), geom=g)


def _pred_tiles(lv):
    import numpy as np
    t = getattr(lv, "_pred_tiles", None)
    if t is None:
        rows = []
        for (h, w), off in zip(lv.hw, lv.offsets):
            for n in range(lv.B):
                for ty in range(-(-h // 8)):
                    for tx in range(-(-w // 16)):
                        rows.append((off + n * h * w, h, w, (ty << 16) | tx))
        t = torch.from_numpy(np.asarray(rows, np.int32)).cuda()
        if not torch.cuda.is_current_stream_capturing():
            torch.cuda.current_stream().synchronize()
        lv._pred_tiles = t
    return t


def pred_conv_patch(lv, x, a, b=None):
    t = _pred_tiles(lv)
    cin = x.shape[1]
    w1, b1, y1, c1 = b if b is not None else (None, None, None, 0)
    _timed("pred3x3_patch_kernel", 2.0 * lv.rows * (a[3] + c1) * cin * 9,
           lambda: _lib.call("radet_pred3x3_patch", _ptr(x), cin, _ptr(t), t.shape[0], _ptr(a[0]), _ptr(a[1]), _ptr(a[2]), a[3],
                             _ptr(w1), _ptr(b1), _ptr(y1), c1, _stream()))


_WTUNE_CACHE = _LRU(8192)


def autotune_wgrad(g, reps=None):
    dev = torch.device("cuda", torch.cuda.current_device())
    reps = reps or TUNE_REPS
    global _TUNE_DIRTY, TUNE_RUNS
    key = (g._key, g.cin, g.cout, g.math, g.h16, "w") + (("x3",) if getattr(g, "x3", False) else ()) + _h2key(g)
    if key not in _WTUNE_CACHE:
        _TUNE_DIRTY = True
        TUNE_RUNS += 1
        M, kk = g.lout.rows, g.k * g.k
        s0 = g.nsplit
        cands = [(0, s0)]
        if g.cout > 64 and g.cin > 64:
            for tid in (1, 2, 3) if getattr(g, "x3", False) else (1, 2):
                tflag, (t, tn) = tid * WG_TILE, WG_TILE_SHAPE[tid]
                tiles = -(-g.cout // t) * -(-g.cin // tn) * kk
                for blocks in (256, 512, 768, 1024):
                    S = max(1, min(64, round(blocks / tiles), (M + 127) // 128))
                    cands.append((tflag | WG_ONE_TAP, S))
                    if not g.math and not g.h16:
                        cands.append((tflag | WG_ONE_TAP | WG_PX32, S))
                    if getattr(g, "x3", False) and t == 64:
                        cands += [(tflag | WG_ONE_TAP | WG_KDIV4, S), (tflag | WG_ONE_TAP | WG_KDIV2, S)]
        cands = sorted(set(cands))
        dt = torch.bfloat16 if g.h16 else torch.float32
        dy = torch.randn(M, g.cout, device=dev).to(dt)
        x = torch.randn(g.lin.rows, g.cin, device=dev).to(dt)
        tmp_keys = _tune_slots(g, dy, x)
        slabs = torch.empty(max(c[1] for c in cands) * g.cout * kk * g.cin, device=dev)
        for fl, S in cands:
            g.wgrad_flags, g.nsplit = fl, S
            conv_wgrad(g, dy, x, slabs)
        torch.cuda.synchronize()
        tbest = [float("inf")] * len(cands)
        for _ in range(reps):
            for i, (fl, S) in enumerate(cands):
                g.wgrad_flags, g.nsplit = fl, S
                s, e = torch.cuda.Event(enable_timing=True), torch.cuda.Event(enable_timing=True)
                s.record()
                for _b in range(TUNE_BURST):
                    conv_wgrad(g, dy, x, slabs)
                e.record()
                e.synchronize()
                tbest[i] = min(tbest[i], s.elapsed_time(e) / TUNE_BURST)
        best = None
        for (fl, S), t in zip(cands, tbest):
            cost = t + S * g.cout * kk * g.cin * 8 / 3e12 * 1e3
            if best is None or cost < best[0]:
                best = (cost, fl, S)
        _WTUNE_CACHE[key] = best[1:]
        unregister_amax(tmp_keys)
        if os.environ.get("RADET_TUNE_LOG"):
            print(f"[tune wgrad] M={M} {g.cin}->{g.cout} k{g.k}s{g.stride}: heuristic S={s0} -> flags={best[1]:#x} S={best[2]} "
                  f"({best[0] * 1e3:.1f} us incl. slab cost)")
    g.wgrad_flags, g.nsplit = _WTUNE_CACHE[key]


def conv_fwd_pair(g, a, b, relu=False, tile=0):
    ws = splitk_ws()
    q = lambda d: [_ptr_any(d.get(k)) for k in ("x", "w", "bias", "addend", "mask", "y")]
    t, table = _tile(g, tile, g.fwd_tile, a["x"], a["y"]), g.fwd_table
    sc = _scales(a["x"], a["w"], a["y"], b["x"], b["w"], b["y"], need=bool(t & H2))
    _timed(lambda: _igemm_key(t, a["x"]), 4.0 * g.lout.rows * g.cout * g.cin * g.k * g.k,
           lambda: _lib.call("radet_conv2d_igemm_pair_s", *q(a), *q(b), _ptr(table), g.lout.rows, g.cin, g.cout, g.k, g.k,
                             int(relu), t, _ptr(ws), C.c_size_t(ws.numel()), _stream(), sc), _conv_bytes(g, 2))


def conv_dgrad_pair(g, a, b, tile=0):
    assert g.stride == 1
    ws = splitk_ws()
    q = lambda d: [_ptr_any(d.get(k)) for k in ("x", "w", "bias", "addend", "mask", "y")]
    t, table = _tile(g, tile, g.bwd_tile, a["x"], a["y"]), g.bwd_table
    sc = _scales(a["x"], a["w"], a["y"], b["x"], b["w"], b["y"], need=bool(t & H2))
    _timed(lambda: _igemm_key(t, a["x"]), 4.0 * g.lin.rows * g.cout * g.cin * g.k * g.k,
           lambda: _lib.call("radet_conv2d_igemm_pair_s", *q(a), *q(b), _ptr(table), g.lin.rows, g.cout, g.cin, g.k, g.k, 0,
                             t, _ptr(ws), C.c_size_t(ws.numel()), _stream(), sc), _conv_bytes(g, 2), kind="dgrad")


def conv_dgrad(g, dy, wft, dx, addend=None, mask=None, k_channels=None, tile=0, splitk=True, skip_zero_rows=False,
               yq=None, wmeta=None):
    kc = g.cout if k_channels is None else k_channels
    tile = _tile(g, tile, (g.bwd_tile_q if _isp(dy) and getattr(g, "bwd_tile_q", 0) else g.bwd_tile), dy, dx)
    if _isp(mask):
        tile |= MASKQ
    assert dx is not None or (yq is not None and g.stride == 1)
    ws = splitk_ws() if splitk else None
    if EVENTS is not None:
        real_k = min(kc, g.cout)
        _timed(_igemm_key(tile, dy) + (" [strided dgrad, class launch]" if g.stride > 1 else ""),
               2.0 * g.lout.rows * real_k * g.cin * g.k * g.k,
               lambda: _conv_dgrad(g, dy, wft, dx, addend, mask, kc, tile, ws, splitk, skip_zero_rows, yq, wmeta),
               _conv_bytes(g), kind="dgrad", geom=g)
        return
    _conv_dgrad(g, dy, wft, dx, addend, mask, kc, tile, ws, splitk, skip_zero_rows, yq, wmeta)


def _conv_dgrad(g, dy, wft, dx, addend, mask, kc, tile, ws, splitk, skip_zero_rows, yq=None, wmeta=None):
    sc = _scales(dy, wft, dx, need=bool(tile & H2) and (_isp(dy) or kc % 32 == 0), yq=yq, wmeta=wmeta, addend=addend)
    if g.stride > 1 and STRIDED_DGRAD_CLASSES:
        assert yq is None and not _isp(mask) and not _isp(dy), "strided dgrad: fp32 tensors only"
        grp = _strided_dgrad_group(g)
        if grp is not None:
            _lib.call("radet_conv2d_igemm_classes_s", _ptr(dy), _ptr(wft), _ptr(addend), _ptr(mask), _ptr(dx),
                      _ptr(grp["table"]), _ptr(grp["out_rows"]), grp["tap_ids"], grp["ntaps"], grp["start"], grp["ncls"],
                      g.k * g.k, grp["M"], kc, g.cin, tile, _ptr(ws), C.c_size_t(ws.numel() if splitk else 0), _stream(), sc)
        for c in _strided_dgrad_classes(g):
            if grp is not None and not c["zero"]:
                continue
            if c["zero"] and skip_zero_rows:
                assert addend is not None and addend.data_ptr() == dx.data_ptr()
                continue
            ct = with_tile(tile, 3) if (c["zero"] and tile_id(tile) >= 7) else tile
            _lib.call("radet_conv2d_igemm_taps_s", _ptr(dy), _ptr(wft), _ptr(addend), _ptr(mask), _ptr(dx), _ptr(c["table"]),
                      _ptr(c["out_rows"]), c["tap_ids"], c["ntaps"], g.k * g.k, c["rows"],
                      (32 if _is16(dy) else 16) if c["zero"] else kc, g.cin,
                      ct, _ptr(ws), C.c_size_t(ws.numel() if splitk else 0), _stream(), sc)
        return
    _lib.call("radet_conv2d_igemm_s", _ptr_any(dy), _ptr_any(wft), None, _ptr(addend), _ptr_any(mask), _ptr(dx), _ptr(g.bwd_table),
              g.lin.rows, kc, g.cin, g.k, g.k, 0, tile, _ptr(ws), C.c_size_t(ws.numel() if splitk else 0), _stream(), sc)


WGRAD9_WINDOWS = os.environ.get("RADET_WGRAD9_WINDOWS", "0") == "1"
WGRAD9_DEEP = os.environ.get("RADET_WGRAD9_DEEP", "0") == "1"


def _wgrad_key(g, dy, co):
    def onetap(fl):
        tile = ("launcher tile" if not wg_tile(fl) else "%d, %d" % WG_TILE_SHAPE[wg_tile(fl)]) if co > 32 else "32, 128"
        kd = ", 64 px / 4 waves" if fl & WG_KDIV4 else (", 32 px / 2 waves" if fl & WG_KDIV2 else "")
        return tile, (", 32 px" if fl & WG_PX32 else "") + kd

    if _isp(dy):
        if dy.kind == "h2" and (g.k != 3 or g.wgrad_pair_flags & WG_ONE_TAP):
            return f"conv_wgradq_kernel<{'128, 128' if wg_tile(g.wgrad_pair_flags) == 1 else '64, 64'}> (fp16 plane pairs)"
        if dy.kind == "h2":
            if g.stride == 1 and g.pad == 1 and WGRAD9_DEEP and -(-g.lout.rows // (16 * (g.nsplit_pairs or g.nsplit))) * 16 <= 1664:
                return "conv_wgrad9d_kernel"
            return "conv_wgrad9r_kernel" if (g.stride == 1 and g.pad == 1 and WGRAD9_WINDOWS) else "conv_wgrad9q_kernel"
        return "conv_wgrad9p_kernel"
    tile, px = onetap(g.wgrad_flags)
    if getattr(g, "h2", False) and getattr(g, "x3", False) and not g.math and not _is16(dy):
        return f"conv_wgradg_kernel<{tile}> (fp16 hi/lo in registers{px})"
    nine = g.k == 3 and g.cin % 32 == 0 and co >= 256 and g.lout.rows >= 16384 and not (g.wgrad_flags & WG_ONE_TAP)
    mode = "bf16 storage" if _is16(dy) else ("bf16 math" if g.math else ("planes in registers" if getattr(g, "x3", False) else "fp32 MFMA"))
    if nine:
        return f"conv_wgrad9{'h' if _is16(dy) else 'g'}_kernel ({mode})"
    return f"conv_wgrad{'h' if _is16(dy) else 'g'}_kernel<{tile}> ({mode}{px})"


def conv_wgrad(g, dy, x, slabs, dbias_partials=None, cout=None, ld_dy=None):
    if EVENTS is not None:
        co_ = g.cout if cout is None else cout
        _timed(_wgrad_key(g, dy, co_), 2.0 * g.lout.rows * co_ * g.cin * g.k * g.k,
               lambda: _conv_wgrad(g, dy, x, slabs, dbias_partials, cout, ld_dy),
               4.0 * (g.lout.rows * co_ + g.lin.rows * g.cin + g.nsplit * co_ * g.k * g.k * g.cin), kind="wgrad", geom=g)
        return
    _conv_wgrad(g, dy, x, slabs, dbias_partials, cout, ld_dy)


def _conv_wgrad(g, dy, x, slabs, dbias_partials=None, cout=None, ld_dy=None):
    co = g.cout if cout is None else cout
    if _isp(dy):
        assert _isp(x) and x.kind == dy.kind
        if dy.kind == "h2":
            nine = g.k == 3 and not (g.wgrad_pair_flags & WG_ONE_TAP)
            fl = WG_H2 | WG_P3 | (g.wgrad_pair_flags if nine else (WG_ONE_TAP | (g.wgrad_pair_flags & WG_TILE_MASK)))
            if nine and g.stride == 1 and g.pad == 1:
                fl |= (WG_DEEP if WGRAD9_DEEP else 0) | (WG_WINDOWS if WGRAD9_WINDOWS else 0)
            _lib.call("radet_conv2d_wgrad_s", _ptr(dy.t), _ptr(x.t), _ptr(slabs), _ptr(dbias_partials), _ptr(g.fwd_table),
                      g.lout.rows, g.cin, co, co if ld_dy is None else ld_dy, g.k, g.k,
                      g.nsplit_pairs or g.nsplit, fl, _stream(), _scales(dy, x, None))
            return
        _lib.call("radet_conv2d_wgrad", _ptr(dy.t), _ptr(x.t), _ptr(slabs), _ptr(dbias_partials), _ptr(g.fwd_table), g.lout.rows,
                  g.cin, co, co if ld_dy is None else ld_dy, g.k, g.k, g.nsplit, WG_P3 | (g.wgrad_flags & WG_ONE_TAP), _stream())
        return
    if getattr(g, "h2", False) and getattr(g, "x3", False) and not g.math and not _is16(dy):
        _lib.call("radet_conv2d_wgrad_s", _ptr(dy), _ptr(x), _ptr(slabs), _ptr(dbias_partials), _ptr(g.fwd_table), g.lout.rows,
                  g.cin, co, co if ld_dy is None else ld_dy, g.k, g.k, g.nsplit, WG_H2 | WG_ONE_TAP | g.wgrad_flags, _stream(),
                  _scales(dy, x, None))
        return
    _lib.call("radet_conv2d_wgrad", _ptr(dy), _ptr(x), _ptr(slabs), _ptr(dbias_partials), _ptr(g.fwd_table), g.lout.rows,
              g.cin, co, co if ld_dy is None else ld_dy, g.k, g.k, g.nsplit,
              (WG_STORE_BF16 if _is16(dy) else (WG_MATH_BF16 if g.math else (WG_X3 if getattr(g, "x3", False) else 0))) | g.wgrad_flags, _stream())


def conv_wgrad_group(jobs, tile=128, math=0):
    jobs = sorted(jobs, key=lambda j: -(j["g"].lout.rows // j["g"].nsplit))
    for i in range(0, len(jobs), 32):
        part = jobs[i:i + 32]
        arr = (_lib.RadetWgradJob * len(part))()
        for a, j in zip(arr, part):
            g = j["g"]
            a.dy, a.x, a.slabs = _ptr(j["dy"]), _ptr(j["x"]), _ptr(j["slabs"])
            a.dbias_partials, a.gather_table = _ptr(j.get("dbias")), _ptr(g.fwd_table)
            a.M, a.Cin, a.Cout, a.ld_dy, a.KH, a.KW, a.S = g.lout.rows, g.cin, g.cout, g.cout, g.k, g.k, g.nsplit
        _lib.call("radet_conv2d_wgrad_group", arr, len(part), (WG_MATH_BF16 if math else 0) | (1 if tile == 128 else 2) * WG_TILE, _stream())


def group_splits(geoms, tile=128, slots=512):
    best = None
    for px in (6400, 4800, 3200, 2400, 1600, 1200, 800, 600, 400):
        S = [max(1, min(64, round(g.lout.rows / px), (g.lout.rows + 127) // 128)) for g in geoms]
        blocks = sum((g.cout // tile) * (g.cin // tile) * g.k * g.k * s for g, s in zip(geoms, S))
        eff = blocks / (slots * -(-blocks // slots))
        cost = -eff + 0.02 * sum(S) / len(S)
        if best is None or cost < best[0] - 1e-9:
            best = (cost, S)
    return best[1]


def fold_weights(table_dev, n):
    _lib.call("radet_fold_weights", _ptr(table_dev), n, _stream())


def unfold_grads(table_dev, n, max_cout):
    _lib.call("radet_unfold_grads", _ptr(table_dev), n, max_cout, _stream())


def _h(name, t):
    return name + "_h" if _is16(t) else name


def stem(img, wf, bias, y, B, H, W):
    ho, wo = (H + 1) // 2, (W + 1) // 2
    if _is16(y):
        fn = lambda: _lib.call("radet_stem_conv_bn_relu_h", _ptr(img), _ptr(wf), _ptr(bias), _ptr(y), B, H, W, _stream())
    else:
        sl = amax_slot(y)
        fn = lambda: _lib.call("radet_stem_conv_bn_relu_a", _ptr(img), _ptr(wf), _ptr(bias), _ptr(y), B, H, W, _ptr(sl), _stream())
    _timed("stem_kernel", 2.0 * B * ho * wo * 64 * 147, fn, 4.0 * (B * 3 * H * W + 64 * 147 + B * ho * wo * 64))


def convert_rows(src, dst, ncols=None, src_off=0, dst_off=0):
    assert src.dim() == 2 and dst.dim() == 2 and src.shape[0] == dst.shape[0] and src.dtype != dst.dtype
    n = src.shape[1] if ncols is None else ncols
    _lib.call("radet_convert_rows", _ptr(src), _ptr(dst), C.c_size_t(src.shape[0]), n, src.stride(0), src_off,
              dst.stride(0), dst_off, 1 if dst.dtype == torch.bfloat16 else 0, _stream())


def maxpool(x, y, B, H, W, Cch, yq=None):
    if _is16(x):
        _lib.call("radet_maxpool3x3s2_h", _ptr(x), _ptr(y), B, H, W, Cch, _stream())
        return
    if yq is not None:
        _lib.call("radet_maxpool3x3s2_q", _ptr(x), _ptr(y), B, H, W, Cch, _ptr(amax_slot(y)), _ptr(yq.t), _ptr(yq.amax),
                  _ptr(amax_slot(x, True)), _stream())
        return
    _lib.call("radet_maxpool3x3s2_a", _ptr(x), _ptr(y), B, H, W, Cch, _ptr(amax_slot(y)), _stream())


def maxpool_bwd_relu(s, dpool, ds, B, H, W, Cch):
    _lib.call("radet_maxpool3x3s2_bwd_relu", _ptr(s), _ptr(dpool), _ptr(ds), B, H, W, Cch, _stream())


def stem_wgrad_splits(B, H, W):
    return _lib.load().radet_stem_wgrad_splits(B, H, W)


def stem_wgrad(img, ds, slabs, dbias_partials, B, H, W, S):
    _lib.call("radet_stem_wgrad", _ptr(img), _ptr(ds), _ptr(slabs), _ptr(dbias_partials), B, H, W, S, _stream())


def gn_ws_floats(levels):
    d, n = _desc([(h, w, h, w, o, o) for (h, w), o in zip(levels.hw, levels.offsets)])
    return _lib.load().radet_gn_workspace_floats(levels.B, d, n)


def _gn_desc(levels):
    return _desc([(h, w, h, w, o, o) for (h, w), o in zip(levels.hw, levels.offsets)])


def gn_relu_fwd(levels, z, gamma, beta, y, stats, ws, eps=1e-5, relu=True):
    d, n = _gn_desc(levels)
# ... 587 lines not shown
```

Measured before the change: 500.0.

## Fuse frozen layer1 bottleneck conv2+conv3+residual (+next conv1) into one kernel

Adds a HIP kernel that runs the 3x3 conv2, the 1x1 conv3 with bias, the residual add and ReLU for frozen stride-1 64-plane bottleneck blocks in one launch. It keeps the o2 tile in LDS as split fp16 pairs. With RADET_FROZEN_TAIL>=2 it can also compute the next block's conv1 in the same kernel. This removes intermediate global-memory round trips and kernel launches in the frozen prefix forward. In exchange it adds register and LDS pressure, and it requantizes in-block, which may change numerics slightly.

```diff
diff --git a/include/radet_hip.h b/include/radet_hip.h
--- a/include/radet_hip.h
+++ b/include/radet_hip.h
@@ -94,6 +94,10 @@
                                  const int* cls_ntaps, const int* cls_start, int ncls, int kt_w, int M, int Cin, int Cout,
                                  int tile_override, float* splitk_ws, size_t splitk_ws_floats, void* stream,
                                  const RadetScales* sc);
+int radet_bottleneck_tail_s(const float* o1, const float* w2, const float* bias2, float* o2, const float* w3, const float* bias3,
+                            const float* residual, float* out, const int* gather_table, int M, int planes, const void* o1_amax,
+                            const void* w2_amax, void* o2_amax, const void* w3_amax, void* out_amax, const float* w1_next,
+                            const float* bias1_next, float* o1_next, const void* w1_next_amax, void* o1_next_amax, void* stream);
 int radet_conv2d_igemm_pair(const float* x0, const float* w0, const float* bias0, const float* addend0,
                             const float* mask0, float* y0, const float* x1, const float* w1, const float* bias1,
                             const float* addend1, const float* mask1, float* y1, const int* gather_table, int M, int Cin,
diff --git a/radet_amd/_lib.py b/radet_amd/_lib.py
--- a/radet_amd/_lib.py
+++ b/radet_amd/_lib.py
@@ -44,6 +44,7 @@
     "radet_conv2d_igemm_pair_s": (_i, [_p] * 13 + [_i, _i, _i, _i, _i, _i, _i, _p, _sz, _p, _p]),
     "radet_conv2d_igemm_taps_s": (_i, [_p, _p, _p, _p, _p, _p, _p, _p, _i, _i, _i, _i, _i, _i, _p, _sz, _p, _p]),
     "radet_conv2d_igemm_classes_s": (_i, [_p, _p, _p, _p, _p, _p, _p, _p, _p, _p, _i, _i, _i, _i, _i, _i, _p, _sz, _p, _p]),
+    "radet_bottleneck_tail_s": (_i, [_p] * 9 + [_i, _i] + [_p] * 11),
     "radet_conv2d_wgrad_s": (_i, [_p, _p, _p, _p, _p, _i, _i, _i, _i, _i, _i, _i, _i, _p, _p]),
     "radet_split_pairs": (_i, [_p, _p, _sz, _i, _i, _p, _p, _p]),
     "radet_merge_pairs": (_i, [_p, _p, _sz, _i, _i, _p, _p]),
diff --git a/radet_amd/csrc/conv_tail.hip b/radet_amd/csrc/conv_tail.hip
--- /dev/null
+++ b/radet_amd/csrc/conv_tail.hip
@@ -0,0 +1,352 @@
+#include "conv_common.h"
+
+constexpr int T_BM = 64, T_BK = 32, T_NSTG = 3, T_P = 64, T_C3 = 256, T_TAPS = 9;
+constexpr int T_ST2 = T_TAPS * (T_P / T_BK);
+constexpr int T_HALF = T_BM * T_BK * 4;
+constexpr int T_STAGE = 2 * T_HALF;
+constexpr int T_O2 = T_NSTG * T_STAGE;
+constexpr int T_PLANE = T_BM * T_P * 2;
+constexpr int T_QT = T_O2 + 2 * T_PLANE;
+template <bool NEXT> constexpr int T_RED = NEXT ? 0 : T_QT;
+template <bool NEXT> constexpr int T_LDS = NEXT ? T_QT + 2 * T_PLANE : T_QT + 16;
+template <bool NEXT> constexpr int T_ST = T_ST2 + (NEXT ? 16 : 4);
+constexpr int tail_kind(bool next, int S) { return S < T_ST2 ? 0 : (!next || (S - T_ST2) % 4 < 2) ? 1 : 2; }
+constexpr int tail_chunk(bool next, int S) { return (S - T_ST2) / (next ? 4 : 2); }
+constexpr int tail_kh(int S) { return (S - T_ST2) % 2; }
+constexpr int tail_loads(bool next, int S) { return (S < T_ST2 || !next) ? 4 : 2; }
+
+struct TailArgs {
+    const float* o1;
+    const float* w2;
+    const float* b2;
+    const float* w3;
+    const float* b3;
+    const float* res;
+    float* out;
+    const int* rowtab;
+    const unsigned* o1s;
+    const unsigned* w2s;
+    const unsigned* w3s;
+    unsigned* outs;
+    float* o2;
+    unsigned* o2s;
+    const float* w1n;
+    const float* b1n;
+    float* o1n;
+    const unsigned* w1ns;
+    unsigned* o1ns;
+    int M, Mp;
+};
+
+template <bool NEXT>
+__global__ __launch_bounds__(256) void radet_bottleneck_tail_kernel(const TailArgs a) {
+    __shared__ __attribute__((aligned(1024))) unsigned char lds[T_LDS<NEXT>];
+    constexpr int NST = T_ST<NEXT>;
+    radet_kernarg_warm<sizeof(TailArgs)>();
+    const int tid = threadIdx.x;
+    const int lane = tid & 63, wave = __builtin_amdgcn_readfirstlane(tid >> 6);
+    const int wm = wave >> 1, wn = wave & 1;
+    const int li = lane & 31, lh = lane >> 5;
+    const int m0 = xcd_remap(blockIdx.x, gridDim.x) * T_BM;
+    const int M = pin_sgpr(a.M);
+    const float* const pb2 = pin_sgpr(a.b2);
+    const float* const pb3 = pin_sgpr(a.b3);
+    const float* const pres = pin_sgpr(a.res);
+    float* const pout = pin_sgpr(a.out);
+    unsigned* const pouts = pin_sgpr(a.outs);
+    const float* const pb1n = pin_sgpr(a.b1n);
+    float* const po1n = pin_sgpr(a.o1n);
+    unsigned* const po1ns = pin_sgpr(a.o1ns);
+    float* const po2 = pin_sgpr(a.o2);
+    unsigned* const po2s = pin_sgpr(a.o2s);
+
+    const unsigned raw_x = h2_scale_load(a.o1s), raw_w2 = h2_scale_load(a.w2s), raw_w3 = h2_scale_load(a.w3s);
+    const unsigned raw_w1n = NEXT ? h2_scale_load(a.w1ns) : 0u;
+
+    const int lrow = lane >> 3;
+    int trow[2];
+    unsigned kq4[2];
+#pragma unroll
+    for (int k = 0; k < 2; ++k) {
+        trow[k] = (wave + 4 * k) * 8 + lrow;
+        kq4[k] = 16u * (unsigned)((lane & 7) ^ ((trow[k] >> 1) & 7));
+    }
+    int arow[T_TAPS][2];
+#pragma unroll
+    for (int t = 0; t < T_TAPS; ++t)
+#pragma unroll
+        for (int k = 0; k < 2; ++k) arow[t][k] = a.rowtab[(size_t)t * a.Mp + m0 + trow[k]];
+
+    const __amdgpu_buffer_rsrc_t rs_x = radet_rsrc(a.o1), rs_w2 = radet_rsrc(a.w2), rs_w3 = radet_rsrc(a.w3);
+    const __amdgpu_buffer_rsrc_t rs_w1n = radet_rsrc(NEXT ? a.w1n : a.w3);
+    auto issue_stage = [&](auto sc) {
+        constexpr int S = decltype(sc)::value;
+        constexpr int BASE = (S % T_NSTG) * T_STAGE;
+        constexpr int kind = tail_kind(NEXT, S);
+        if constexpr (kind == 0) {
+            constexpr int tap = S / (T_P / T_BK), c0 = (S % (T_P / T_BK)) * T_BK;
+#pragma unroll
+            for (int k = 0; k < 2; ++k) {
+                const unsigned voff = arow[tap][k] >= 0 ? (unsigned)arow[tap][k] * (T_P * 4u) + c0 * 4u + kq4[k] : 0xFFFFFFFFu;
+                __builtin_amdgcn_raw_ptr_buffer_load_lds(rs_x, (lptr_t)(&lds[BASE + (wave + 4 * k) * 1024]), 16, (int)voff, 0, 0, 0);
+            }
+#pragma unroll
+            for (int k = 0; k < 2; ++k) {
+                const unsigned voff = (unsigned)trow[k] * (T_TAPS * T_P * 4u) + (tap * T_P + c0) * 4u + kq4[k];
+                __builtin_amdgcn_raw_ptr_buffer_load_lds(rs_w2, (lptr_t)(&lds[BASE + T_HALF + (wave + 4 * k) * 1024]), 16, (int)voff, 0, 0, 0);
+            }
+        } else if constexpr (!NEXT) {
+            constexpr int chunk = tail_chunk(NEXT, S), c0 = tail_kh(S) * T_BK;
+#pragma unroll
+            for (int h = 0; h < 2; ++h)
+#pragma unroll
+                for (int k = 0; k < 2; ++k) {
+                    const unsigned voff = (unsigned)(chunk * 128 + h * 64 + trow[k]) * (T_P * 4u) + c0 * 4u + kq4[k];
+                    __builtin_amdgcn_raw_ptr_buffer_load_lds(rs_w3, (lptr_t)(&lds[BASE + h * T_HALF + (wave + 4 * k) * 1024]), 16, (int)voff, 0, 0, 0);
+                }
+        } else {
+            constexpr int chunk = tail_chunk(NEXT, S), c0 = tail_kh(S) * T_BK;
+#pragma unroll
+            for (int k = 0; k < 2; ++k) {
+                const unsigned voff = kind == 1 ? (unsigned)(chunk * 64 + trow[k]) * (T_P * 4u) + c0 * 4u + kq4[k]
+                                                : (unsigned)trow[k] * (T_C3 * 4u) + (chunk * 64 + c0) * 4u + kq4[k];
+                __builtin_amdgcn_raw_ptr_buffer_load_lds(kind == 1 ? rs_w3 : rs_w1n, (lptr_t)(&lds[BASE + T_HALF + (wave + 4 * k) * 1024]), 16,
+                                                         (int)voff, 0, 0, 0);
+            }
+        }
+    };
+
+    const unsigned lds0 = (unsigned)(size_t)(lptr_t)(&lds[0]);
+    const unsigned rsw = (unsigned)((li >> 1) & 7);
+    const unsigned fa0 = lds0 + (unsigned)((wm * 32 + li) * 128) + 16u * ((2u * lh) ^ rsw);
+    const unsigned fb0 = lds0 + T_HALF + (unsigned)((wn * 32 + li) * 128) + 16u * ((2u * lh) ^ rsw);
+    const unsigned fw0 = lds0 + (unsigned)((wn * 64 + li) * 128) + 16u * ((2u * lh) ^ rsw);
+    const unsigned fo0 = lds0 + T_O2 + (unsigned)((wm * 32 + li) * 128) + 16u * ((unsigned)lh ^ rsw);
+
+    auto block_to_pairs = [&](const float (&v)[16], int tile) {
+        float mx = 0.f;
+#pragma unroll
+        for (int r = 0; r < 16; ++r) mx = fmaxf(mx, fabsf(v[r]));
+        const unsigned wbits = radet_amax_reduce(__float_as_uint(mx));
+        if (lane == 0) *reinterpret_cast<volatile unsigned*>(&lds[T_RED<NEXT> + 4 * wave]) = wbits;
+        radet_pipe_barrier();
+        unsigned tb = 0u;
+#pragma unroll
+        for (int w = 0; w < 4; ++w) {
+            const unsigned x = *reinterpret_cast<volatile unsigned*>(&lds[T_RED<NEXT> + 4 * w]);
+            tb = x > tb ? x : tb;
+        }
+        const H2Scale sc = h2_scale_bits((unsigned)__builtin_amdgcn_readfirstlane((int)tb));
+        const int c = wn * 32 + li;
+        unsigned short* const ph = reinterpret_cast<unsigned short*>(&lds[tile]) + (c & 7);
+#pragma unroll
+        for (int r = 0; r < 16; r += 2) {
+            unsigned h, l;
+            radet_split2(v[r], v[r + 1], sc.s, sc.s2, h, l);
+            const int t = wm * 32 + (r & 3) + 8 * (r >> 2) + 4 * lh;
+            const int o = t * 64 + 8 * ((c >> 3) ^ ((t >> 1) & 7));
+            ph[o] = (unsigned short)(h & 0xFFFFu);
+            ph[o + 64] = (unsigned short)(h >> 16);
+            ph[o + T_PLANE / 2] = (unsigned short)(l & 0xFFFFu);
+            ph[o + 64 + T_PLANE / 2] = (unsigned short)(l >> 16);
+        }
+        radet_pipe_barrier();
+        return sc;
+    };
+    auto pair_stage = [&](auto boc, auto tnc, unsigned fa, unsigned fb, int kh, const H2Scale& sw, f32x16* d0, f32x16* d1) {
+        constexpr int BO = decltype(boc)::value, TN = decltype(tnc)::value;
+        f32x4 oh[2], ol[2], bf[2][TN][2];
+#pragma unroll
+        for (int g = 0; g < 2; ++g) {
+            lds_read128<0>(oh[g], fa ^ (32u * (unsigned)(2 * kh + g)));
+            lds_read128<T_PLANE>(ol[g], fa ^ (32u * (unsigned)(2 * kh + g)));
+#pragma unroll
+            for (int j = 0; j < TN; ++j) {
+                lds_read128<BO>(bf[g][j][0], (fb + 4096u * j) ^ (64u * g));
+                lds_read128<BO>(bf[g][j][1], (fb + 4096u * j) ^ (64u * g) ^ 16u);
+            }
+        }
+        static_for<0, 2>([&](auto gc) {
+            constexpr int g = decltype(gc)::value;
+            lds_wait<(1 - g) * (2 + 2 * TN)>();
+            asm volatile("" : "+v"(oh[g]), "+v"(ol[g]));
+#pragma unroll
+            for (int j = 0; j < TN; ++j) asm volatile("" : "+v"(bf[g][j][0]), "+v"(bf[g][j][1]));
+            const f16x8 ah = __builtin_bit_cast(f16x8, oh[g]), al = __builtin_bit_cast(f16x8, ol[g]);
+#pragma unroll
+            for (int j = 0; j < TN; ++j) {
+                f16x8 bh, bl;
+                split2_f16(bf[g][j][0], bf[g][j][1], sw, bh, bl);
+                mfma_h2(d0[j], d1[j], ah, al, bh, bl);
+            }
+            __builtin_amdgcn_sched_barrier(0);
+        });
+    };
+
+    f32x16 acc, acc1;
+#pragma unroll
+    for (int r = 0; r < 16; ++r) { acc[r] = 0.f; acc1[r] = 0.f; }
+    constexpr int TN3 = NEXT ? 1 : 2;
+    f32x16 c3[TN3], c31[TN3];
+    f32x16 n0, n1;
+    float o1n[16];
+#pragma unroll
+    for (int r = 0; r < 16; ++r) o1n[r] = 0.f;
+
+    issue_stage(std::integral_constant<int, 0>{});
+    issue_stage(std::integral_constant<int, 1>{});
+    vm_wait<tail_loads(NEXT, 1)>();
+    radet_pipe_barrier();
+    const H2Scale sx = h2_scale_finish(raw_x), sw2 = h2_scale_finish(raw_w2), sw3 = h2_scale_finish(raw_w3);
+    const H2Scale sw1n = h2_scale_finish(raw_w1n);
+    H2Scale so = {1.f, 1.f, 1.f}, sq = {1.f, 1.f, 1.f};
+    float amax = 0.f, amaxn = 0.f;
+    const bool interior = m0 + T_BM <= M;
+
+    static_for<0, NST>([&](auto sc) {
+        constexpr int S = decltype(sc)::value;
+        constexpr int BO = (S % T_NSTG) * T_STAGE;
+        constexpr int kind = tail_kind(NEXT, S);
+        if constexpr (S + T_NSTG - 1 < NST) issue_stage(std::integral_constant<int, S + T_NSTG - 1>{});
+        if constexpr (kind == 0) {
+            f32x4 af[2][2], bf[2][2];
+#pragma unroll
+            for (int g = 0; g < 2; ++g) {
+                lds_read128<BO>(af[g][0], fa0 ^ (64u * g));
+                lds_read128<BO>(af[g][1], fa0 ^ (64u * g) ^ 16u);
+                lds_read128<BO>(bf[g][0], fb0 ^ (64u * g));
+                lds_read128<BO>(bf[g][1], fb0 ^ (64u * g) ^ 16u);
+            }
+            static_for<0, 2>([&](auto gc) {
+                constexpr int g = decltype(gc)::value;
+                lds_wait<(1 - g) * 4>();
+                asm volatile("" : "+v"(af[g][0]), "+v"(af[g][1]), "+v"(bf[g][0]), "+v"(bf[g][1]));
+                f16x8 ah, al, bh, bl;
+                split2_f16(af[g][0], af[g][1], sx, ah, al);
+                split2_f16(bf[g][0], bf[g][1], sw2, bh, bl);
+                mfma_h2(acc, acc1, ah, al, bh, bl);
+                __builtin_amdgcn_sched_barrier(0);
+            });
+        } else if constexpr (kind == 1) {
+            if constexpr (tail_kh(S) == 0) {
+#pragma unroll
+                for (int j = 0; j < TN3; ++j)
+#pragma unroll
+                    for (int r = 0; r < 16; ++r) { c3[j][r] = 0.f; c31[j][r] = 0.f; }
+            }
+            pair_stage(std::integral_constant<int, BO>{}, std::integral_constant<int, TN3>{}, fo0, NEXT ? fb0 : fw0, tail_kh(S), sw3, c3, c31);
+        } else {
+            if constexpr (tail_kh(S) == 0) {
+#pragma unroll
+                for (int r = 0; r < 16; ++r) { n0[r] = 0.f; n1[r] = 0.f; }
+            }
+            pair_stage(std::integral_constant<int, BO>{}, std::integral_constant<int, 1>{}, fo0 + 2u * T_PLANE, fb0, tail_kh(S), sw1n, &n0, &n1);
+        }
+        if constexpr (S + 1 < NST) {
+            if constexpr (S + T_NSTG - 1 < NST) vm_wait<tail_loads(NEXT, S + T_NSTG - 1)>(); else vm_wait<0>();
+            radet_pipe_barrier();
+        }
+        if constexpr (S == T_ST2 - 1) {
+            h2_combine(acc, acc1, sx.inv, sw2.inv);
+            const float bv = pb2[wn * 32 + li];
+            float v[16];
+#pragma unroll
+            for (int r = 0; r < 16; ++r) {
+                const int row = m0 + wm * 32 + (r & 3) + 8 * (r >> 2) + 4 * lh;
+                v[r] = row < M ? fmaxf(acc[r] + bv, 0.f) : 0.f;
+            }
+            if (po2) {
+                float m2 = 0.f;
+#pragma unroll
+                for (int r = 0; r < 16; ++r) {
+                    const int row = m0 + wm * 32 + (r & 3) + 8 * (r >> 2) + 4 * lh;
+                    if (interior || row < M) po2[(size_t)row * T_P + wn * 32 + li] = v[r];
+                    m2 = fmaxf(m2, v[r]);
+                }
+                if (po2s) radet_amax_publish(m2, po2s);
+            }
+            so = block_to_pairs(v, T_O2);
+        }
+        if constexpr (kind == 1 && tail_kh(S) == 1) {
+            constexpr int chunk = tail_chunk(NEXT, S);
+            size_t obase[16];
+            bool rvalid[16];
+#pragma unroll
+            for (int r = 0; r < 16; ++r) {
+                const int row = m0 + wm * 32 + (r & 3) + 8 * (r >> 2) + 4 * lh;
+                rvalid[r] = row < M;
+                obase[r] = (size_t)(rvalid[r] ? row : 0) * T_C3;
+            }
+#pragma unroll
+            for (int j = 0; j < TN3; ++j) {
+                const int col = NEXT ? chunk * 64 + wn * 32 + li : chunk * 128 + wn * 64 + j * 32 + li;
+                const float bv = pb3[col];
+                float av[16], o[16];
+#pragma unroll
+                for (int r = 0; r < 16; ++r) av[r] = pres[obase[r] + col];
+                h2_combine(c3[j], c31[j], so.inv, sw3.inv);
+#pragma unroll
+                for (int r = 0; r < 16; ++r) o[r] = fmaxf(c3[j][r] + bv + av[r], 0.f);
+                if (interior) {
+#pragma unroll
+                    for (int r = 0; r < 16; ++r) { pout[obase[r] + col] = o[r]; amax = fmaxf(amax, fabsf(o[r])); }
+                } else {
+#pragma unroll
+                    for (int r = 0; r < 16; ++r)
+                        if (rvalid[r]) { pout[obase[r] + col] = o[r]; amax = fmaxf(amax, fabsf(o[r])); }
+                }
+                if constexpr (NEXT) {
+#pragma unroll
+                    for (int r = 0; r < 16; ++r) o[r] = rvalid[r] ? o[r] : 0.f;
+                    sq = block_to_pairs(o, T_QT);
+                }
+            }
+        }
+        if constexpr (kind == 2 && tail_kh(S) == 1) {
+            h2_combine(n0, n1, sq.inv, sw1n.inv);
+#pragma unroll
+            for (int r = 0; r < 16; ++r) o1n[r] += n0[r];
+        }
+    });
+    if constexpr (NEXT) {
+        const int col = wn * 32 + li;
+        const float bv = pb1n[col];
+#pragma unroll
+        for (int r = 0; r < 16; ++r) {
+            const int row = m0 + wm * 32 + (r & 3) + 8 * (r >> 2) + 4 * lh;
+            const float v = fmaxf(o1n[r] + bv, 0.f);
+            if (interior || row < M) { po1n[(size_t)row * T_P + col] = v; amaxn = fmaxf(amaxn, v); }
+        }
+        if (po1ns) radet_amax_publish(amaxn, po1ns);
+    }
+    if (pouts) radet_amax_publish(amax, pouts);
+}
+
+static bool tail_aligned(const void* p) { return p != nullptr && ((uintptr_t)p & 15u) == 0; }
+
+extern "C" int radet_bottleneck_tail_s(const float* o1, const float* w2, const float* bias2, float* o2, const float* w3,
+                                       const float* bias3, const float* residual, float* out, const int* gather_table, int M,
+                                       int planes, const void* o1_amax, const void* w2_amax, void* o2_amax, const void* w3_amax,
+                                       void* out_amax, const float* w1_next, const float* bias1_next, float* o1_next, const void* w1_next_amax,
+                                       void* o1_next_amax, void* stream) {
+    if (planes != T_P || M <= 0 || gather_table == nullptr || bias2 == nullptr || bias3 == nullptr) return RADET_ERR_ARG;
+    if (!tail_aligned(o1) || !tail_aligned(w2) || !tail_aligned(w3) || !tail_aligned(residual) || !tail_aligned(out))
+        return RADET_ERR_ARG;
+    if (o1_amax == nullptr || w2_amax == nullptr || w3_amax == nullptr) return RADET_ERR_ARG;
+    if (o2 != nullptr && !tail_aligned(o2)) return RADET_ERR_ARG;
+    const bool next = w1_next != nullptr;
+    if (next && (!tail_aligned(w1_next) || !tail_aligned(o1_next) || bias1_next == nullptr || w1_next_amax == nullptr))
+        return RADET_ERR_ARG;
+    if ((unsigned long long)M * T_C3 * 4ull >= 0xFFFFFF00ull) return RADET_ERR_ARG;
+    TailArgs a;
+    a.o1 = o1; a.w2 = w2; a.b2 = bias2; a.w3 = w3; a.b3 = bias3; a.res = residual; a.out = out; a.rowtab = gather_table;
+    a.o1s = (const unsigned*)o1_amax; a.w2s = (const unsigned*)w2_amax; a.w3s = (const unsigned*)w3_amax;
+    a.outs = (unsigned*)out_amax;
+    a.o2 = o2; a.o2s = o2 ? (unsigned*)o2_amax : nullptr;
+    a.w1n = w1_next; a.b1n = bias1_next; a.o1n = o1_next; a.w1ns = (const unsigned*)w1_next_amax; a.o1ns = (unsigned*)o1_next_amax;
+    a.M = M; a.Mp = radet_gather_table_rows(M);
+    const dim3 grid((M + T_BM - 1) / T_BM);
+    if (next) hipLaunchKernelGGL(radet_bottleneck_tail_kernel<true>, grid, dim3(256), 0, (hipStream_t)stream, a);
+    else hipLaunchKernelGGL(radet_bottleneck_tail_kernel<false>, grid, dim3(256), 0, (hipStream_t)stream, a);
+    return radet_check_launch();
+}
diff --git a/radet_amd/csrc/tape_thunks.c b/radet_amd/csrc/tape_thunks.c
--- a/radet_amd/csrc/tape_thunks.c
+++ b/radet_amd/csrc/tape_thunks.c
@@ -20,6 +20,7 @@
 static int t_radet_bbox_overlaps(const uint64_t* a) { return radet_bbox_overlaps((void*)(uintptr_t)a[0], (void*)(uintptr_t)a[1], (void*)(uintptr_t)a[2], (int)(int64_t)a[3], (int)(int64_t)a[4], (int)(int64_t)a[5], (int)(int64_t)a[6], (int)(int64_t)a[7], f32(a[8]), (void*)(uintptr_t)a[9]); }
 static int t_radet_bce_logits_loss(const uint64_t* a) { return radet_bce_logits_loss((void*)(uintptr_t)a[0], (void*)(uintptr_t)a[1], (void*)(uintptr_t)a[2], (int)(int64_t)a[3], (size_t)a[4], (int)(int64_t)a[5], (void*)(uintptr_t)a[6], f32(a[7]), (void*)(uintptr_t)a[8], (void*)(uintptr_t)a[9]); }
 static int t_radet_bce_logits_loss_bwd(const uint64_t* a) { return radet_bce_logits_loss_bwd((void*)(uintptr_t)a[0], (void*)(uintptr_t)a[1], (void*)(uintptr_t)a[2], (int)(int64_t)a[3], (size_t)a[4], (int)(int64_t)a[5], (void*)(uintptr_t)a[6], (void*)(uintptr_t)a[7], (void*)(uintptr_t)a[8], f32(a[9]), (void*)(uintptr_t)a[10], (void*)(uintptr_t)a[11]); }
+static int t_radet_bottleneck_tail_s(const uint64_t* a) { return radet_bottleneck_tail_s((void*)(uintptr_t)a[0], (void*)(uintptr_t)a[1], (void*)(uintptr_t)a[2], (void*)(uintptr_t)a[3], (void*)(uintptr_t)a[4], (void*)(uintptr_t)a[5], (void*)(uintptr_t)a[6], (void*)(uintptr_t)a[7], (void*)(uintptr_t)a[8], (int)(int64_t)a[9], (int)(int64_t)a[10], (void*)(uintptr_t)a[11], (void*)(uintptr_t)a[12], (void*)(uintptr_t)a[13], (void*)(uintptr_t)a[14], (void*)(uintptr_t)a[15], (void*)(uintptr_t)a[16], (void*)(uintptr_t)a[17], (void*)(uintptr_t)a[18], (void*)(uintptr_t)a[19], (void*)(uintptr_t)a[20], (void*)(uintptr_t)a[21]); }
 static int t_radet_box_loss(const uint64_t* a) { return radet_box_loss((int)(int64_t)a[0], (void*)(uintptr_t)a[1], (void*)(uintptr_t)a[2], (void*)(uintptr_t)a[3], (size_t)a[4], f32(a[5]), f32(a[6]), (void*)(uintptr_t)a[7], f32(a[8]), (void*)(uintptr_t)a[9], (void*)(uintptr_t)a[10]); }
 static int t_radet_box_loss_bwd(const uint64_t* a) { return radet_box_loss_bwd((int)(int64_t)a[0], (void*)(uintptr_t)a[1], (void*)(uintptr_t)a[2], (void*)(uintptr_t)a[3], (size_t)a[4], f32(a[5]), f32(a[6]), (void*)(uintptr_t)a[7], (void*)(uintptr_t)a[8], (void*)(uintptr_t)a[9], f32(a[10]), (void*)(uintptr_t)a[11], (void*)(uintptr_t)a[12]); }
 static int t_radet_build_gather_table(const uint64_t* a) { return radet_build_gather_table((void*)(uintptr_t)a[0], (int)(int64_t)a[1], (int)(int64_t)a[2], (int)(int64_t)a[3], (int)(int64_t)a[4], (int)(int64_t)a[5], (int)(int64_t)a[6], (int)(int64_t)a[7], (void*)(uintptr_t)a[8], (int)(int64_t)a[9], (void*)(uintptr_t)a[10]); }
@@ -137,6 +138,7 @@
     {"radet_bbox_overlaps", t_radet_bbox_overlaps, 10},
     {"radet_bce_logits_loss", t_radet_bce_logits_loss, 10},
     {"radet_bce_logits_loss_bwd", t_radet_bce_logits_loss_bwd, 12},
+    {"radet_bottleneck_tail_s", t_radet_bottleneck_tail_s, 22},
     {"radet_box_loss", t_radet_box_loss, 11},
     {"radet_box_loss_bwd", t_radet_box_loss_bwd, 13},
     {"radet_build_gather_table", t_radet_build_gather_table, 11},
@@ -237,4 +239,4 @@
     {"radet_upsample_add_h", t_radet_upsample_add_h, 9},
     {"radet_warp_affine_u8", t_radet_warp_affine_u8, 9},
 };
-const int radet_tape_nthunks = 114;
+const int radet_tape_nthunks = 115;
diff --git a/radet_amd/engine.py b/radet_amd/engine.py
--- a/radet_amd/engine.py
+++ b/radet_amd/engine.py
@@ -52,6 +52,7 @@
         self.po = self.h2 and not self.pairs and os.environ.get("RADET_PAIRS_ONLY", "0") == "1"
         self.po_max_planes = int(os.environ.get("RADET_PAIRS_ONLY_MAX", "512"))
         self.pairs_from = int(os.environ.get("RADET_PAIRS_FROM", "2"))
+        self.frozen_tail = int(os.environ.get("RADET_FROZEN_TAIL", "1")) if (self.h2 and not self.pairs and not self.po) else 0
         if self.x3 and "RADET_TOWER_MODE" not in os.environ:
             self.tower_mode = "pairbwd"
         self.p3 = self.x3 and self.tower_mode == "pairbwd" and feat % 32 == 0 and os.environ.get("RADET_P3", "1") != "0"
@@ -131,7 +132,8 @@
                     c2=self._add(Conv(pfx + ".conv2", planes, planes, 3, stride, 1, bn=pfx + ".bn2", trainable=train, dgrad=train)),
                     c3=self._add(Conv(pfx + ".conv3", planes, planes * 4, 1, 1, 0, bn=pfx + ".bn3", trainable=train, dgrad=train)),
                     ds=None, stride=stride, train=train,
-                    po=self.po and stride == 1 and planes % 32 == 0 and planes <= self.po_max_planes)
+                    po=self.po and stride == 1 and planes % 32 == 0 and planes <= self.po_max_planes,
+                    tail=self.frozen_tail > 0 and fs >= 0 and not train and stride == 1 and planes == 64)
                 if b == 0:
                     blk["ds"] = self._add(Conv(pfx + ".downsample.0", inpl, planes * 4, 1, stride, 0, bn=pfx + ".downsample.1",
                                                trainable=train, dgrad=in_dgrad))
@@ -600,10 +602,23 @@
     def unfold(self):
         K.unfold_grads(self.table, len(self.convs), self.max_cout)
 
-    def _block_forward(self, blk, pfx, x, b, xq=None):
+    def _block_forward(self, blk, pfx, x, b, xq=None, nxt=None, have_o1=False):
         blk["x"] = x
+        c1, c2, c3, ds = blk["c1"], blk["c2"], blk["c3"], blk["ds"]
+        if blk["tail"]:
+            o1, out = b[pfx + ".o1"], b[pfx + ".out"]
+            if not have_o1:
+                K.conv_fwd(c1.geom, x, c1.wf, c1.bias_f, o1, relu=True)
+            idt = x
+            if ds is not None:
+                idt = b[pfx + ".idt"]
+                K.conv_fwd(ds.geom, x, ds.wf, ds.bias_f, idt)
+            n1 = None
+            if nxt is not None:
+                n1 = (nxt[0]["c1"].geom, nxt[0]["c1"].wf, nxt[0]["c1"].bias_f, b[nxt[1] + ".o1"])
+            K.bottleneck_tail(c2.geom, c3.geom, o1, c2.wf, c2.bias_f, c3.wf, c3.bias_f, idt, out, o2=b[pfx + ".o2"], nxt=n1)
+            return out
         o1, o2, out = b[pfx + ".o1"], b[pfx + ".o2"], b[pfx + ".out"]
-        c1, c2, c3, ds = blk["c1"], blk["c2"], blk["c3"], blk["ds"]
         if xq is not None and c1.wfq is not None and c2.wfq is not None and c3.wfq is not None and (ds is None or ds.wfq is not None):
             o1q, o2q, outq = b[pfx + ".o1@q"], b[pfx + ".o2@q"], b.get(pfx + ".out@q")
             K.conv_fwd(c1.geom, xq, c1.wfq, c1.bias_f, o1, relu=True, tile=c1.geom.fwd_tile_q, yq=o1q, wmeta=c1.wmeta)
@@ -649,8 +664,12 @@
         x, xq = b["pool"], b.get("pool@q")
         for li in range(self._n_frozen_stages()):
             K.STAGE = f"layer{li + 1}"
-            for bi, blk in enumerate(self.stages[li]):
-                x = self._block_forward(blk, f"l{li + 1}.{bi}", x, b, xq)
+            blocks, fused = self.stages[li], False
+            for bi, blk in enumerate(blocks):
+                nxt = (blocks[bi + 1], f"l{li + 1}.{bi + 1}") if (self.frozen_tail >= 2 and blk["tail"] and bi + 1 < len(blocks)
+                                                                  and blocks[bi + 1]["tail"]) else None
+                x = self._block_forward(blk, f"l{li + 1}.{bi}", x, b, xq, nxt=nxt, have_o1=fused)
+                fused = nxt is not None
                 xq = b.get(f"l{li + 1}.{bi}.out@q")
         return b
 
diff --git a/radet_amd/kernels.py b/radet_amd/kernels.py
--- a/radet_amd/kernels.py
+++ b/radet_amd/kernels.py
@@ -778,6 +778,32 @@
                   g.lout.rows, g.cin, g.cout, g.k, g.k, int(relu), tile, _ptr(ws), C.c_size_t(ws.numel() if splitk else 0),
                   _stream(), sc)
     _timed(lambda: _igemm_key(tile, x), 2.0 * g.lout.rows * g.cout * g.cin * g.k * g.k, launch, _conv_bytes(g), geom=g)
+
+
+TAIL_KEY = "radet_bottleneck_tail_kernel"
+
+
+def bottleneck_tail(g2, g3, o1, w2, bias2, w3, bias3, residual, out, o2=None, nxt=None):
+    assert g2.k == 3 and g2.stride == 1 and g2.pad == 1 and g2.cin == g2.cout == g3.cin == 64 and g3.cout == 256 and g3.identity
+    assert not _isp(o1) and o1.dtype == torch.float32 and out.dtype == torch.float32 and residual.dtype == torch.float32
+    table = g2.fwd_table
+    rows = g2.lout.rows
+    flops = 2.0 * rows * (64 * 64 * 9 + 256 * 64)
+    nbytes = 4.0 * (rows * 64 + 2 * rows * 256 + 64 * 9 * 64 + 256 * 64 + (rows * 64 if o2 is not None else 0))
+    g1n = w1n = b1n = o1n = None
+    if nxt is not None:
+        g1n, w1n, b1n, o1n = nxt
+        assert g1n.identity and g1n.cin == 256 and g1n.cout == 64 and g1n.lout.rows == rows and o1n.dtype == torch.float32
+        flops += 2.0 * rows * 256 * 64
+        nbytes += 4.0 * (rows * 64 + 64 * 256)
+    keep = (amax_slot(o1, True), amax_slot(w2, True), amax_slot(o2), amax_slot(w3, True), amax_slot(out),
+            amax_slot(w1n, True), amax_slot(o1n))
+
+    def launch():
+        _lib.call("radet_bottleneck_tail_s", _ptr(o1), _ptr(w2), _ptr(bias2), _ptr(o2), _ptr(w3), _ptr(bias3), _ptr(residual),
+                  _ptr(out), _ptr(table), rows, g2.cout, _ptr(keep[0]), _ptr(keep[1]), _ptr(keep[2]), _ptr(keep[3]), _ptr(keep[4]),
+                  _ptr(w1n), _ptr(b1n), _ptr(o1n), _ptr(keep[5]), _ptr(keep[6]), _stream())
+    _timed(TAIL_KEY + ("<true>" if nxt is not None else "<false>"), flops, launch, nbytes, kind="fwd", geom=g2)
 
 
 def _pred_tiles(lv):
```

After: 501.6 (median of 6 runs). About the same (+0.3%).
